# numericalEFT/MCIntegration.jl

Hardware: AMD Instinct MI355X
Metric: Msamples/sec (whole node), 16-D Gaussian :vegas (higher is better)
Workload: dtype f64

## Files before the change

### mcintegration.jl_amd/_lib.py

```python
import ctypes as C
import os

_PKG = os.path.dirname(os.path.abspath(__file__))
_SO = os.path.join(_PKG, "lib", "libmci_hip.so")

MCI_OK = 0
ERR_NAMES = {1: "INVALID", 2: "HIP", 3: "COMPILE", 4: "NORMALIZATION", 5: "HISTOGRAM", 6: "COMM", 7: "NO_DEVICE"}
CONTINUOUS, DISCRETE, FERMIK = 0, 1, 2
VEGAS, VEGASMC, MCMC = 0, 1, 2
ABI_VERSION = 5
SOLVERS = {"vegas": VEGAS, "vegasmc": VEGASMC, "mcmc": MCMC, VEGAS: VEGAS, VEGASMC: VEGASMC, MCMC: MCMC}

c_double_p = C.POINTER(C.c_double)
c_int32_p = C.POINTER(C.c_int32)


class MCIError(RuntimeError):
    def __init__(self, code, msg):
        super().__init__("[MCI_ERR_%s] %s" % (ERR_NAMES.get(code, code), msg))
        self.code = code


class LeafDesc(C.Structure):
    _fields_ = [("kind", C.c_int32), ("pool", C.c_int32), ("lower", C.c_double), ("upper", C.c_double),
                ("npoints", C.c_int32), ("alpha", C.c_double), ("adapt", C.c_int32), ("init", c_double_p)]


class ProblemDesc(C.Structure):
    _fields_ = [("nleaf", C.c_int32), ("leaves", C.POINTER(LeafDesc)), ("npool", C.c_int32),
                ("nintegrand", C.c_int32), ("dof", c_int32_p), ("obs_nbin", c_int32_p), ("obs_bin_draw", c_int32_p),
                ("neighbor_offsets", c_int32_p), ("neighbor_list", c_int32_p), ("ncomp", C.c_int32)]


class IntegrateArgs(C.Structure):
    _fields_ = [("solver", C.c_int32), ("neval", C.c_int64), ("niter", C.c_int32), ("block", C.c_int64),
                ("ignore", C.c_int32), ("adapt", C.c_int32), ("gamma", C.c_double), ("measurefreq", C.c_int64),
                ("seed", C.c_uint64), ("nchain", C.c_int64), ("first_iteration", C.c_int32),
                ("thermal_ratio", C.c_double), ("reweight_goal", c_double_p)]


HOST_INTEGRAND_FN = C.CFUNCTYPE(C.c_int, c_double_p, c_double_p, C.c_int64, C.c_int32, C.c_int32, C.c_void_p)
HOST_INTEGRAND_IDX_FN = C.CFUNCTYPE(C.c_int, C.POINTER(C.c_int32), c_double_p, c_double_p, C.c_int64, C.c_int32, C.c_int32, C.c_void_p)
HOST_MEASURE_FN = C.CFUNCTYPE(C.c_int, c_double_p, c_double_p, C.c_int64, C.c_int64, C.c_int32, C.c_int32, C.c_int64, c_double_p, C.c_int32, C.c_void_p)
HOST_MEASURE_IDX_FN = C.CFUNCTYPE(C.c_int, C.POINTER(C.c_int32), c_double_p, c_double_p, C.c_int64, C.c_int64, C.c_int32, C.c_int32, C.c_int64, c_double_p,
                                  C.c_int32, C.c_void_p)


class ResultC(C.Structure):
    _fields_ = [("niter", C.c_int32), ("nobs", C.c_int32), ("iter_mean", c_double_p), ("iter_std", c_double_p),
                ("mean", c_double_p), ("stdev", c_double_p), ("chi2", c_double_p), ("neval", C.c_int64),
                ("seconds", C.c_double), ("visited", c_double_p), ("correlated", C.c_int32), ("warmup", C.c_int32)]


_VP = C.c_void_p
SIGNATURES = [
    ("mci_ctx_create", C.c_int, [C.c_int32, C.POINTER(_VP)]),
    ("mci_ctx_destroy", C.c_int, [_VP]),
    ("mci_last_error", C.c_char_p, []),
    ("mci_device_count", C.c_int, [c_int32_p]),
    ("mci_ctx_stream", _VP, [_VP]),
    ("mci_comm_unique_id", C.c_int, [_VP]),
    ("mci_comm_init", C.c_int, [_VP, C.c_int32, C.c_int32, _VP]),
    ("mci_comm_rank", C.c_int, [_VP, c_int32_p, c_int32_p]),
    ("mci_comm_sum", C.c_int, [_VP, c_double_p, C.c_int32]),
    ("mci_problem_create", C.c_int, [_VP, C.POINTER(ProblemDesc), C.POINTER(_VP)]),
    ("mci_problem_destroy", C.c_int, [_VP]),
    ("mci_set_integrand_source", C.c_int, [_VP, C.c_char_p, c_double_p, C.c_int32]),
    ("mci_set_integrand_host", C.c_int, [_VP, _VP, _VP]),
    ("mci_set_integrand_host_indexed", C.c_int, [_VP, _VP, _VP]),
    ("mci_set_measure_source", C.c_int, [_VP, C.c_char_p]),
    ("mci_set_measure_host", C.c_int, [_VP, _VP, _VP]),
    ("mci_set_measure_host_indexed", C.c_int, [_VP, _VP, _VP]),
    ("mci_compile", C.c_int, [_VP]),
    ("mci_compile_solver", C.c_int, [_VP, C.c_int32]),
    ("mci_kernel_code_object", C.c_int, [_VP, C.c_int32, C.c_char_p, C.c_int32]),
    ("mci_check_status", C.c_int, [_VP]),
    ("mci_set_launch", C.c_int, [_VP, C.c_int32, C.c_int32]),
    ("mci_problem_info", C.c_int, [_VP, c_int32_p, c_int32_p, C.POINTER(C.c_int64), c_int32_p, C.POINTER(C.c_int64)]),
    ("mci_get_histogram_copies", C.c_int, [_VP, c_int32_p]),
    ("mci_set_kernel_timing", C.c_int, [_VP, C.c_int32]),
    ("mci_iteration_run", C.c_int, [_VP, C.c_int32, C.c_int64, C.c_int64, C.c_int64, C.c_int32, C.c_uint64, C.c_int64, C.c_int64, C.c_double]),
    ("mci_iteration_reduce", C.c_int, [_VP]),
    ("mci_iteration_finish", C.c_int, [_VP, C.c_int32, C.c_int64, C.c_int32, C.c_double, c_double_p, c_double_p]),
    ("mci_integrate", C.c_int, [_VP, C.POINTER(IntegrateArgs), C.POINTER(ResultC)]),
    ("mci_get_iteration_log", C.c_int, [_VP, C.c_int32, c_double_p]),
    ("mci_reserve_iteration_log", C.c_int, [_VP, C.c_int32]),
    ("mci_get_packed", C.c_int, [_VP, c_double_p, C.c_int64]),
    ("mci_set_packed", C.c_int, [_VP, c_double_p, C.c_int64]),
    ("mci_packed_device_ptr", _VP, [_VP]),
    ("mci_get_grid", C.c_int, [_VP, C.c_int32, c_double_p, C.c_int32]),
    ("mci_set_grid", C.c_int, [_VP, C.c_int32, c_double_p, C.c_int32]),
    ("mci_get_distribution", C.c_int, [_VP, C.c_int32, c_double_p, c_double_p, C.c_int32]),
    ("mci_set_distribution", C.c_int, [_VP, C.c_int32, c_double_p, C.c_int32]),
    ("mci_get_reweight", C.c_int, [_VP, c_double_p, C.c_int32]),
    ("mci_set_reweight", C.c_int, [_VP, c_double_p, C.c_int32]),
    ("mci_set_reweight_goal", C.c_int, [_VP, c_double_p, C.c_int32]),
    ("mci_get_acceptance", C.c_int, [_VP, c_double_p, c_double_p, C.c_int32]),
    ("mci_save_state", C.c_int, [_VP, C.c_char_p]),
    ("mci_load_state", C.c_int, [_VP, C.c_char_p]),
    ("mci_set_train_walk", C.c_int, [_VP, C.c_int32]),
    ("mci_set_rng_bits", C.c_int, [_VP, C.c_int32]),
    ("mci_set_rng_rounds", C.c_int, [_VP, C.c_int32]),
    ("mci_set_deterministic", C.c_int, [_VP, C.c_int32]),
    ("mci_set_chain_carry", C.c_int, [_VP, C.c_int32]),
    ("mci_set_iteration_counted", C.c_int, [_VP, C.c_int32]),
    ("mci_set_persistent", C.c_int, [_VP, C.c_int32]),
    ("mci_last_integrate_persistent", C.c_int, [_VP, C.POINTER(C.c_int32)]),
    ("mci_last_chain_launch", C.c_int, [_VP, C.POINTER(C.c_int64), c_int32_p]),
    ("mci_set_stratification", C.c_int, [_VP, C.c_int32, c_int32_p, C.c_double, C.c_int64]),
    ("mci_set_stratification_off", C.c_int, [_VP]),
    ("mci_get_stratification", C.c_int, [_VP, c_int32_p, C.POINTER(C.c_int64), c_double_p]),
    ("mci_get_strat_counts", C.c_int, [_VP, C.POINTER(C.c_int64), C.c_int64]),
    ("mci_strat_plan", C.c_int, [C.c_int64, C.c_int32, C.c_int64, c_int32_p]),
    ("mci_set_chain_speculation", C.c_int, [_VP, C.c_int32, C.c_double, C.c_int32]),
    ("mci_last_chain_speculation", C.c_int, [_VP, c_int32_p, c_int32_p]),
    ("mci_chain_speculation_status", C.c_int, [_VP, C.c_int32, c_int32_p]),
    ("mci_last_integrate_discarded", C.c_int, [_VP, C.POINTER(C.c_int64), c_int32_p]),
    ("mci_speculation_tree", C.c_int, [C.c_int32, C.c_double, C.c_int32, c_int32_p, c_int32_p, c_int32_p, C.POINTER(C.c_uint64), C.POINTER(C.c_uint64)]),
    ("mci_compile_chain_speculation", C.c_int, [_VP, C.c_int32]),
    ("mci_train", C.c_int, [_VP]),
    ("mci_sample_dump", C.c_int, [_VP, C.c_int32, C.c_uint64, C.c_int64, C.c_int64, C.c_int64, c_double_p, c_double_p, c_double_p]),
    ("mci_kernel_times_ms", C.c_int, [_VP, C.POINTER(C.c_float), C.c_int32, c_int32_p, c_int32_p, c_int32_p]),
    ("mci_kernel_clocks", C.c_int, [_VP, c_double_p, C.c_int32, c_int32_p]),
    ("mci_comm_times_ms", C.c_int, [_VP, C.POINTER(C.c_float), C.c_int32, c_int32_p]),
    ("mci_comm_collectives", C.c_int, [_VP, C.POINTER(C.c_int64), C.POINTER(C.c_int64)]),
    ("mci_reduce_size", C.c_int, [_VP, C.POINTER(C.c_int64)]),
    ("mci_external_reduce_done", C.c_int, [_VP]),
    ("mci_standardize_block", None, [C.c_int64, C.c_int64, C.c_int64, C.POINTER(C.c_int64), C.POINTER(C.c_int64)]),
    ("mci_chain_burnin", C.c_double, [C.c_int64, C.c_int64, C.c_int32]),
    ("mci_mcmc_burnin", C.c_int64, [C.c_int64, C.c_int64, C.c_int32, C.c_int32, C.c_int32, C.c_double]),
    ("mci_mcmc_auto_chains", C.c_int64, [C.c_int64, C.c_int64, C.c_int32, C.c_int32, C.c_int32, C.c_int64, C.c_int64, C.c_int32]),
    ("mci_get_hold_histogram", C.c_int, [_VP, C.POINTER(C.c_uint64)]),
    ("mci_mcmc_launch_valid", C.c_int, [_VP, c_int32_p, c_int32_p, C.POINTER(C.c_int64), C.POINTER(C.c_int64)]),
    ("mci_iteration_discard", C.c_int, [_VP]),
    ("mci_get_block_means", C.c_int, [_VP, C.c_int32, c_double_p, C.POINTER(C.c_int64), c_int32_p]),
    ("mci_reset_block_log", C.c_int, [_VP]),
    ("mci_lineage_sums", None, [c_double_p, C.c_int64, C.c_int64, C.c_int64, c_double_p, C.c_int64, C.c_int64, c_double_p, c_double_p]),
    ("mci_maxdof", None, [c_int32_p, C.c_int32, C.c_int32, c_int32_p]),
    ("mci_mean_std", None, [c_double_p, c_double_p, C.c_int64, C.c_int64, c_double_p, c_double_p]),
    ("mci_average", None, [c_double_p, c_double_p, C.c_int64, C.c_int64, C.c_int64, c_double_p, c_double_p, c_double_p]),
    ("mci_do_reweight", None, [c_double_p, c_double_p, C.c_int64, C.c_double, c_double_p]),
    ("mci_version", C.c_char_p, []),
    ("mci_abi_version", C.c_int32, []),
]
DEBUG_SIGNATURES = [
    ("mci_debug_persist_words", C.c_int, [_VP, C.POINTER(C.c_uint64), C.c_int32]),
    ("mci_debug_walk_counts", C.c_int, [_VP, C.POINTER(C.c_int64)]),
    ("mci_debug_plant_wrong_decision", C.c_int, [_VP, C.c_int32]),
    ("mci_debug_persist_spin_ticks", C.c_int, [_VP, C.c_uint64]),
    ("mci_debug_override", C.c_int, [C.c_char_p, C.c_int64, C.c_int32]),
    ("mci_debug_compiler_id", C.c_int, [C.c_char_p, C.c_char_p, C.c_int32]),
    ("mci_debug_split_chunks", C.c_int, [_VP, C.POINTER(C.c_int64), C.POINTER(C.c_int64)]),
    ("mci_debug_strat_dump", C.c_int, [_VP, C.c_int64, c_double_p, c_double_p, C.POINTER(C.c_int64), c_double_p, c_double_p]),
    ("mci_debug_mcmc_policy", C.c_int, [C.c_int64, C.c_int64, C.c_int64, C.c_int64]),
]

_lib = None


def library_path():
    return _SO


def use_rocm_compiler(rocm=None):
    root = rocm or os.environ.get("ROCM_PATH") or "/opt/rocm"
    mapped = set()
    try:
        with open("/proc/self/maps") as fh:
            for line in fh:
                path = line.split(None, 5)[-1].strip() if line.count(" ") >= 5 else ""
                if "amd_comgr" in path or "hiprtc" in path:
                    mapped.add(os.path.realpath(path))
    except OSError:
        pass

    def installed(names):
        for name in names:
            path = os.path.join(root, "lib", name)
            if os.path.exists(path):
                return path
        return None
    comgr, hiprtc = installed(("libamd_comgr.so.3", "libamd_comgr.so.2", "libamd_comgr.so")), installed(("libhiprtc.so.7", "libhiprtc.so"))
    have_comgr = [p for p in mapped if "amd_comgr" in p]
    if have_comgr and (comgr is None or os.path.realpath(comgr) not in have_comgr):
        return False
    done = False
    for path in (comgr, hiprtc):
        if path is not None:
            C.CDLL(path, mode=C.RTLD_GLOBAL)
            done = True
    return done


def compiler_id():
    buf = C.create_string_buffer(1024)
    lib().mci_debug_compiler_id(None, buf, len(buf))
    return buf.value.decode()


def lib():
    global _lib
    if _lib is None:
        if not os.path.exists(_SO):
            raise ImportError("%s is missing: run `python __graft_entry__.py` (hipcc --offload-arch=gfx950) first; "
                              "the MI355X engine has no Python/CPU fallback" % _SO)
        L = C.CDLL(_SO, mode=C.RTLD_GLOBAL)
        for name, res, args in SIGNATURES + DEBUG_SIGNATURES:
            fn = getattr(L, name)
            fn.restype = res
            fn.argtypes = args
        if L.mci_abi_version() != ABI_VERSION:
            raise ImportError("%s has ABI %d, this package was written against ABI %d: rebuild with `python __graft_entry__.py`" % (_SO, L.mci_abi_version(), ABI_VERSION))
        _lib = L
    return _lib


def check(rc):
    if rc != MCI_OK:
        raise MCIError(rc, lib().mci_last_error().decode(errors="replace"))
```

### mcintegration.jl_amd/csrc/mci_debug.h

```cpp
#ifndef MCI_DEBUG_H
#define MCI_DEBUG_H
#include "../../include/mci.h"
#ifdef __cplusplus
extern "C" {
#endif
int mci_debug_persist_words(mci_problem *prob, unsigned long long *out, int32_t n);
int mci_debug_walk_counts(mci_problem *prob, int64_t *out);
int mci_debug_plant_wrong_decision(mci_problem *prob, int32_t on);
int mci_debug_persist_spin_ticks(mci_problem *prob, unsigned long long ticks);
int mci_debug_override(const char *key, int64_t value, int32_t on);
int mci_debug_split_chunks(const mci_problem *prob, int64_t *chunks, int64_t *bytes);
int mci_debug_strat_dump(mci_problem *prob, int64_t n, double *x, double *y, int64_t *h, double *jac, double *w);
int mci_debug_compiler_id(const char *set, char *out, int32_t n);
int mci_debug_mcmc_policy(int64_t pilot_steps, int64_t grow, int64_t carry_holds, int64_t carry_half_floors);
#ifdef __cplusplus
}
#endif
#endif
```

### mcintegration.jl_amd/csrc/mci_host_integrate.h

```cpp
namespace {
int64_t persist_lds(const mci_problem *p, int *map_off) {
    const int N = p->leaves.empty() ? 1 : p->leaves[0].nbin;
    const int64_t a = (p->lds_bytes + 7) / 8, b = (int64_t)mci::train_lds_doubles(N) + N + 256;
    const int64_t off = ((a > b ? a : b) + 1) & ~(int64_t)1;
    if (map_off) *map_off = (int)off;
    return (off + (N + 2) + 4) * 8;
}
bool persist_layout(const mci_problem *p) {
    const auto &s = p->shape;
    if (p->deterministic || s.table_mode != 0 || s.ntile != 1 || s.host_integrand || s.host_measure || s.nbin <= 0 || s.ec_doubles > 0) return false;
    if (s.nleaf != 1 || p->leaves.size() != 1 || p->leaves[0].kind != 0) return false;
    return persist_lds(p, nullptr) <= 64 * 1024;
}
bool persist_plan(const mci_problem *p, const mci_integrate_args *a, int64_t nevalperblock, int64_t nblocks, int *wpb_out) {
    const auto &s = p->shape;
    if (p->persistent == 0 || p->persist_failed) return false;
    if (a->solver != MCI_VEGAS || a->measurefreq != 1 || a->niter < 1) return false;
    if (p->ctx->nranks != 1) return false;
    if (!persist_layout(p)) return false;
    if (p->wg_per_block > 0 || p->kernel_timing > 0 || p->train_serial >= 1) return false;
    const int64_t work = nevalperblock * nblocks * s.ndraw;
    if (p->persistent < 0 && (work >= ((int64_t)1 << 19) || s.ndraw > 7)) return false;
    const int T = p->threads;
    int64_t target = work < ((int64_t)1 << 19) ? 64 : 128;
// ... 45 lines not shown
    g_orphans.push_back(j);
}
static int compile_persist(mci_problem *p, bool background) {
    if (p->persist_compiled) return MCI_OK;
    Candidate local, *c = &local;
    if (p->persist_job) {
        if (!p->persist_job->done.load(std::memory_order_acquire)) {
            if (background) return MCI_OK;
            p->persist_job->th.join();
        }
        if (p->persist_job->th.joinable()) p->persist_job->th.join();
        local = std::move(p->persist_job->c);
        delete p->persist_job;
        p->persist_job = nullptr;
    } else {
        mcijit::ProblemShape sh = p->shape;
        sh.hcopy = 1;
        sh.det = 0;
        c->src = mcijit::generate_source(sh, MCI_VEGAS, mcijit::kUnitVegasPersist, p->leaves[0].alpha);
        c->threads = p->threads;
        c->rc = mcijit::compile(c->src, c->threads, c->code, c->log, c->cached, &c->path, mcijit::kHdrTrain, background);
        if (c->rc == -1) {
            {
                static const int kPersistAfterCalls = 256;
                static std::mutex mu;
                static std::map<uint64_t, int> asked;
                std::lock_guard<std::mutex> g(mu);
                if (++asked[mcijit::fnv1a(c->src)] < kPersistAfterCalls) return MCI_OK;
            }
            p->persist_job = new mci_problem::PersistJob;
            p->persist_job->c = std::move(local);
            mci_problem::PersistJob *j = p->persist_job;
            j->th = std::thread([j] {
                j->c.rc = mcijit::compile(j->c.src, j->c.threads, j->c.code, j->c.log, j->c.cached, &j->c.path, mcijit::kHdrTrain);
                j->done.store(true, std::memory_order_release);
            });
            return MCI_OK;
        }
    }
    if (c->rc) {
        p->persist_failed = true;
        return fail(MCI_ERR_COMPILE, "integrand failed to compile for gfx950:\n%s", c->log.c_str());
    }
    if (mcijit::max_static_lds_bytes(c->code) != 0 || mcijit::kernel_scratch_bytes(c->code, "mci_vegas_persist") != 0) {
        p->persist_failed = true;
        return fail(MCI_ERR_COMPILE, "the persistent :vegas kernel came out with static LDS or scratch");
    }
    p->persist_code_object = c->path;
    p->persist_threads = c->threads;
    if (p->ctx->offline) {
        p->persist_compiled = true;
        return MCI_OK;
    }
    HIPCHK(hipSetDevice(p->ctx->device));
    if (hipModuleLoadData(&p->module_persist, c->code.data()) != hipSuccess) {
        p->persist_failed = true;
        if (c->cached) unlink(c->path.c_str());
        return fail(MCI_ERR_HIP, "hipModuleLoadData failed for the persistent :vegas code object");
    }
    HIPCHK(hipModuleGetFunction(&p->f_persist, p->module_persist, "mci_vegas_persist"));
    if (!p->d_persist) {
        HIPCHK(hipMalloc((void **)&p->d_persist, kPersistWords * sizeof(unsigned long long)));
        HIPCHK(hipMemsetAsync(p->d_persist, 0, kPersistWords * sizeof(unsigned long long), p->ctx->stream));
        p->persist_arrive = p->persist_done = 0;
    }
    p->persist_compiled = true;
    return MCI_OK;
}

static int persist_launch(mci_problem *p, const mci_integrate_args *ia, int64_t nevalperblock, int64_t lo, int64_t hi, int wpb) {
    const auto &s = p->shape;
    const int64_t nblocks = hi - lo, nrows = nblocks * wpb;
    int rc;
    if ((rc = flush_merge(p))) return rc;
    HIPCHK(hipSetDevice(p->ctx->device));
    if ((rc = ensure_capacity(p, 2 * nrows, nblocks))) return rc;
    if ((rc = grow_iteration_log(p, (int64_t)p->log_row + ia->niter))) return rc;
    const int T = p->persist_threads;
    mci::BatchArgs a{};
    a.edges = p->d_edges;
    a.dacc = p->d_dacc;
    a.ddist = p->d_ddist;
    a.reweight = p->d_reweight;
    a.ud = p->d_ud;
    a.part_cols = p->d_part_cols;
    a.part_hist = p->d_part_hist;
    a.ghist = p->d_ghist;
    a.seed = ia->seed;
    a.iteration = (mci::u32)ia->first_iteration;
    a.neval_per_block = nevalperblock;
    a.block_lo = lo;
    a.wg_per_block = wpb;
    a.measurefreq = 1;
    a.nchain = 1;
    a.hist_atomic = 1;
    a.status = p->d_status;
    a.tile_stride = nblocks * nevalperblock;
    a.nrows = nrows;
    mci::PersistArgs f{};
    mci::MergeArgs &m = f.m;
    m.part_cols = p->d_part_cols;
    m.ncols = s.ncols;
    m.nobs = s.nobs;
    m.ni = s.ni;
    m.nblocks = (int)nblocks;
    m.wg_per_block = wpb;
    m.stage1 = p->d_stage1;
    m.ngroup = (int)mci_problem::kGroups;
    m.ghist = p->d_ghist;
    m.use_ghist = 1;
    m.nbin = s.nbin;
    m.packed = p->d_packed;
    m.status = p->d_status;
    m.scratch = p->d_scratch;
    m.part_pa = nullptr;
    m.npa = p->npa;
    m.nrows = (int)nrows;
    mci::TrainArgs &t = f.t;
    t.leaves = p->d_leaves;
    t.nleaf = s.nleaf;
    t.packed = p->d_packed;
    t.nstat = p->nstat;
    t.edges = p->d_edges;
    t.dacc = p->d_dacc;
    t.ddist = p->d_ddist;
    t.iter_log_row = p->d_iterlog + (size_t)p->log_row * p->nstat;
    t.reweight = p->d_reweight;
    t.goal = nullptr;
    t.nd = s.ni + 1;
    t.do_reweight = 0;
    t.gamma = ia->gamma;
    t.do_train = ia->adapt ? 1 : 0;
    t.serial_walk = 0;
    t.status = p->d_status;
    t.maxn = p->leaves[0].nbin;
    f.niter = ia->niter;
    const int64_t lds = persist_lds(p, &f.map_off);
    f.ctr = p->d_persist;
    if (p->persist_arrive > (1ull << 39)) {
        HIPCHK(hipMemsetAsync(p->d_persist, 0, 3 * sizeof(unsigned long long), p->ctx->stream));
        p->persist_arrive = p->persist_done = 0;
    }
    f.arrive0 = p->persist_arrive;
    f.done0 = p->persist_done;
    f.spin_ticks = p->persist_spin_ticks;
    void *args[] = {&a, &f};
    if (!p->d_edges_backup) HIPCHK(hipMalloc((void **)&p->d_edges_backup, (p->h_edges.size() ? p->h_edges.size() : 1) * sizeof(double)));
    if (p->h_edges.size()) HIPCHK(hipMemcpyAsync(p->d_edges_backup, p->d_edges, p->h_edges.size() * sizeof(double), hipMemcpyDeviceToDevice, p->ctx->stream));
    HIPCHK(hipModuleLaunchKernel(p->f_persist, (unsigned)nrows + 1, 1, 1, (unsigned)T, 1, 1, (unsigned)lds, p->ctx->stream, args, nullptr));
    p->persist_arrive += (unsigned long long)(ia->niter + 1) * (unsigned long long)nrows;
    p->persist_done += (unsigned long long)ia->niter;
    p->launch.time_this_launch = false;
    p->merge_pending = false;
    p->merge = m;
    p->merge.part_cols = p->d_part_cols + (size_t)((ia->niter - 1) & 1) * (size_t)nrows * s.ncols;
    p->launch.last_samples = nblocks * nevalperblock;
    p->launch.last_wg = (int)nrows;
    p->launch.last_threads = T;
    p->launch.last_nblocks = (int)nblocks;
    p->log_row += ia->niter;
    return MCI_OK;
}

static int comm_sum_host(mci_problem *p, double *v, int n) {
    if (!p->ctx->comm) return MCI_OK;
    double *d = nullptr;
    HIPCHK(hipMalloc((void **)&d, (size_t)n * sizeof(double)));
    hipStream_t st = p->ctx->stream;
    hipError_t e = hipMemcpyAsync(d, v, (size_t)n * sizeof(double), hipMemcpyHostToDevice, st);
    int r = e == hipSuccess ? g_rccl.AllReduce(d, d, (size_t)n, kNcclFloat64, kNcclSum, p->ctx->comm, st) : 0;
    p->ctx->collectives += 1;
    p->ctx->last_count = n;
    if (e == hipSuccess && !r) e = hipMemcpyAsync(v, d, (size_t)n * sizeof(double), hipMemcpyDeviceToHost, st);
    if (e == hipSuccess && !r) e = hipStreamSynchronize(st);
    (void)hipFree(d);
    if (r) return fail(MCI_ERR_COMM, "ncclAllReduce (lineage sums): %s", g_rccl.GetErrorString ? g_rccl.GetErrorString(r) : "?");
    if (e != hipSuccess) return fail(MCI_ERR_HIP, "lineage sums: %s", hipGetErrorString(e));
    return MCI_OK;
}

int mci_integrate(mci_problem *p, const mci_integrate_args *a, mci_result *res) {
    if (!p || !a || !res) return fail(MCI_ERR_INVALID, "NULL argument");
    if (p->ctx->offline) return fail(MCI_ERR_NO_DEVICE, "offline context: no device to run on");
    const auto &s = p->shape;
    if (res->niter < a->niter || res->nobs != s.nobs) return fail(MCI_ERR_INVALID, "result buffers too small");
    if (!(a->neval > a->block)) return fail(MCI_ERR_INVALID, "neval=%lld should be larger than nblock = %lld", (long long)a->neval, (long long)a->block);
    int64_t nevalperblock, block;
    mci_standardize_block(a->neval, a->block, p->ctx->nranks, &nevalperblock, &block);
    const int64_t per = block / p->ctx->nranks;
    const int64_t lo = per * p->ctx->rank, hi = lo + per;
    if (a->solver != MCI_VEGAS && a->solver != MCI_VEGASMC && a->solver != MCI_MCMC) return fail(MCI_ERR_INVALID, "Solver %d is not supported!", a->solver);
    int wpb_persist = 0, rc = 0;
    const bool strat = p->strat.on;
    if (strat) {
        if (a->solver != MCI_VEGAS) return fail(MCI_ERR_INVALID, "stratification works with solver = :vegas only (mci_set_stratification_off first)");
        if (a->measurefreq != 1) return fail(MCI_ERR_INVALID, "stratification: measurefreq = %lld is refused (every sample is measured)", (long long)a->measurefreq);
        strat_call_start(p);
    }
    bool persist = !strat && persist_plan(p, a, nevalperblock, hi - lo, &wpb_persist);
    if (persist) (void)compile_persist(p, p->persistent < 0);
    persist = persist && p->persist_compiled;
    if (!persist && !strat && (rc = compile_solver(p, kslot(a->solver, a->measurefreq)))) return rc;
    if ((rc = mci_set_reweight_goal(p, a->reweight_goal, a->reweight_goal ? p->ni + 1 : 0))) return rc;
    const int ignore = a->ignore >= 0 ? a->ignore : (a->adapt ? 1 : 0);
    const size_t nlog = (size_t)a->niter * p->nstat;
    if (nlog + 1 > p->cap_hlog) {
        size_t ncap = p->cap_hlog ? p->cap_hlog : (size_t)64 * p->nstat + 1;
        while (ncap < nlog + 1) ncap *= 2;
        if (p->h_log) (void)hipHostFree(p->h_log);
        p->h_log = nullptr;
        p->cap_hlog = 0;
        HIPCHK(hipHostMalloc((void **)&p->h_log, ncap * sizeof(double), hipHostMallocDefault));
        p->cap_hlog = ncap;
    }
    int64_t blk_row0 = -1;
    if (a->solver != MCI_VEGAS) {
        if ((rc = flush_merge(p))) return rc;
        p->launch.blk_rows = 0;
        p->launch.blk_carried = 0;
        p->launch.blk_stride = (hi - lo) * s.nobs;
        p->launch.blk_lo = lo;
        blk_row0 = 0;
        if ((rc = grow_block_log(p, a->niter))) return rc;
    }
    HIPCHK(hipStreamSynchronize(p->ctx->stream));
    const int row0 = p->log_row;
    auto t0 = std::chrono::steady_clock::now();
    double *h = p->h_log;
    int *hstatus = reinterpret_cast<int *>(p->h_log + nlog);
    int res_warmup = 0;
    p->last_discarded_neval = 0;
    p->last_discarded_launches = 0;
    for (int attempt = 0;; ++attempt) {
        p->last_persistent = persist;
        if (persist && (rc = persist_launch(p, a, nevalperblock, lo, hi, wpb_persist))) return rc;
        for (int it = 0; it < a->niter && !persist; ++it) {
            for (int attempt = 0;; ++attempt) {
                const int32_t iter = a->first_iteration + it + kRepeatStride * attempt;
                p->launch_counted = it >= ignore;
                if ((rc = mci_iteration_run(p, a->solver, nevalperblock, lo, hi, iter, a->seed, a->measurefreq, a->nchain, a->thermal_ratio))) return rc;
                if ((rc = mci_iteration_reduce(p))) return rc;
                if ((rc = mci_iteration_finish(p, a->solver, block, a->adapt, a->gamma, nullptr, nullptr))) return rc;
                if (a->solver != MCI_MCMC || a->nchain > 0 || p->launch.mcmc_warm || (it == 0 && ignore >= 1) || attempt >= kMaxRepeats ||
                    a->first_iteration + it >= kRepeatStride || p->launch.last_nchain <= 1 || !p->launch.hold_inflight)
                    break;
                int32_t valid = 0;
                if ((rc = mci_mcmc_launch_valid(p, &valid, nullptr, nullptr, nullptr))) return rc;
                if (valid) break;
                if ((rc = mci_iteration_discard(p))) return rc;
                res_warmup += 1;
                p->last_discarded_neval += nevalperblock * (hi - lo);
                p->last_discarded_launches += 1;
            }
        }
        p->launch_counted = false;
        HIPCHK(hipMemcpyAsync(h, p->d_iterlog + (size_t)row0 * p->nstat, nlog * sizeof(double), hipMemcpyDeviceToHost, p->ctx->stream));
        HIPCHK(hipMemcpyAsync(hstatus, p->d_status, sizeof(int), hipMemcpyDeviceToHost, p->ctx->stream));
        HIPCHK(hipStreamSynchronize(p->ctx->stream));
        if (persist && attempt == 0 && (*hstatus & mci::ST_PERSIST_STALL)) {
            if (p->d_edges_backup && p->h_edges.size())
                HIPCHK(hipMemcpyAsync(p->d_edges, p->d_edges_backup, p->h_edges.size() * sizeof(double), hipMemcpyDeviceToDevice, p->ctx->stream));
            if ((rc = persist_recover(p))) return rc;
            p->log_row = row0;
            persist = false;
            if ((rc = compile_solver(p, kslot(a->solver, a->measurefreq)))) return rc;
            continue;
        }
        break;
    }
    if (*hstatus && (rc = check_status(p))) return rc;
    auto t1 = std::chrono::steady_clock::now();
    res->seconds = std::chrono::duration<double>(t1 - t0).count();
    res->neval = 0;
    for (int it = 0; it < a->niter; ++it) {
        const double *row = h + (size_t)it * p->nstat;
        if (strat) strat_mean_std(row, s.nobs, res->iter_mean + (size_t)it * s.nobs, res->iter_std + (size_t)it * s.nobs);
        else
        mci_mean_std(row, row + s.nobs, s.nobs, block, res->iter_mean + (size_t)it * s.nobs, res->iter_std + (size_t)it * s.nobs);
        res->neval += (int64_t)row[2 * s.nobs + 1];
        if (res->visited && it == a->niter - 1) memcpy(res->visited, row + 2 * s.nobs + 2, (size_t)(s.ni + 1) * sizeof(double));
    }
    for (int o = 0; o < s.nobs; ++o)
        mci_average(res->iter_mean + o, res->iter_std + o, s.nobs, ignore + 1, a->niter, &res->mean[o], &res->stdev[o], &res->chi2[o]);
    res->correlated = 0;
    res->warmup = res_warmup;
    if (a->solver != MCI_VEGAS && blk_row0 >= 0 && p->launch.blk_rows - blk_row0 == a->niter && p->launch.blk_carried > 0 && a->niter > ignore + 1) {
        const int64_t nb = hi - lo;
        std::vector<double> bm((size_t)a->niter * nb * s.nobs), sums(2 * (size_t)s.nobs);
        HIPCHK(hipMemcpyAsync(bm.data(), p->d_blocklog + (size_t)blk_row0 * p->launch.blk_stride, bm.size() * sizeof(double), hipMemcpyDeviceToHost, p->ctx->stream));
        HIPCHK(hipStreamSynchronize(p->ctx->stream));
        mci_lineage_sums(bm.data(), a->niter, nb, s.nobs, res->iter_std, ignore + 1, a->niter, sums.data(), sums.data() + s.nobs);
        if ((rc = comm_sum_host(p, sums.data(), (int)sums.size()))) return rc;
        std::vector<double> lm(s.nobs), le(s.nobs);
        mci_mean_std(sums.data(), sums.data() + s.nobs, s.nobs, block, lm.data(), le.data());
        for (int o = 0; o < s.nobs; ++o) res->stdev[o] = le[o] > 0.0 ? le[o] : res->stdev[o];
        res->correlated = 1;
    }
    return MCI_OK;
}
```

### mcintegration.jl_amd/csrc/mci_host_iteration.h

```cpp
int mci_iteration_run(mci_problem *p, int32_t solver, int64_t nevalperblock, int64_t block_lo, int64_t block_hi,
                      int32_t iteration, uint64_t seed, int64_t measurefreq, int64_t nchain, double thermal_ratio) {
    if (p->ctx->offline) return fail(MCI_ERR_NO_DEVICE, "offline context: no device to run on");
    if (solver != MCI_VEGAS && solver != MCI_VEGASMC && solver != MCI_MCMC) return fail(MCI_ERR_INVALID, "Solver %d is not supported!", solver);
    const bool auto_chains = nchain <= 0;
    if (measurefreq <= 0) return fail(MCI_ERR_INVALID, "measurefreq must be positive");
    const int64_t nblocks = block_hi - block_lo;
    if (nblocks < 1 || nevalperblock < 1) return fail(MCI_ERR_INVALID, "empty iteration");
    if (p->has_fermik && solver != MCI_MCMC) return fail(MCI_ERR_INVALID, "FermiK variables work with solver=:mcmc only");
    if (p->strat.on) {
        if (solver != MCI_VEGAS) return fail(MCI_ERR_INVALID, "stratification works with solver = :vegas only (mci_set_stratification_off first)");
        return strat_run(p, nevalperblock, block_lo, block_hi, iteration, seed, measurefreq);
    }
    const int kern = kslot(solver, measurefreq);
    int rc = (solver == MCI_VEGAS || p->deterministic || p->shape.host_integrand || p->spec_lanes == 1) ? compile_solver(p, kern) : MCI_OK;
    if (rc) return rc;
    if (solver == MCI_VEGAS && p->shape.host_integrand && (rc = ensure_dump(p))) return rc;
    if ((rc = flush_merge(p))) return rc;
    HIPCHK(hipSetDevice(p->ctx->device));
    const auto &s = p->shape;
    int T = solver_threads(p, solver);
    if (solver == MCI_VEGAS && p->vegas_wide && !p->threads_vegas && p->wg_per_block <= 0 && nblocks * nevalperblock < ((int64_t)1 << 22) &&
        nblocks * nevalperblock * p->shape.ndraw >= ((int64_t)1 << 19))
        T = 512;
    int64_t units = nevalperblock;
// ... 424 lines not shown
            p->d_hstep = nullptr;
            p->cap_hstep = 0;
            HIPCHK(hipMalloc(&p->d_hstep, (size_t)nc * ((3 * nd + nw + 4) * sizeof(double) + (2 * nd + 7) * sizeof(int)) + 16));
            p->cap_hstep = nc;
        }
        if (nc > p->cap_hidx) {
            if (p->h_hidx) (void)hipHostFree(p->h_hidx);
            p->h_hidx = nullptr;
            p->cap_hidx = 0;
            HIPCHK(hipHostMalloc((void **)&p->h_hidx, (size_t)(nc + 1) * sizeof(int32_t), hipHostMallocDefault));
            p->cap_hidx = nc;
        }
        {
            double *dp = (double *)p->d_hstep;
            a.hs.cx = dp; dp += (size_t)nd * nc;
            a.hs.cprob = dp; dp += (size_t)nd * nc;
            a.hs.pprob = dp; dp += (size_t)nd * nc;
            a.hs.cw = dp; dp += (size_t)nw * nc;
            a.hs.cprobability = dp; dp += nc;
            a.hs.pprop = dp; dp += nc;
            a.hs.puacc = dp; dp += nc;
            a.hs.cwabs = dp; dp += nc;
            int *ip = (int *)dp;
            a.hs.cbin = ip; ip += (size_t)nd * nc;
            a.hs.pbin = ip; ip += (size_t)nd * nc;
            a.hs.pvi = ip; ip += nc;
            a.hs.ccurr = ip; ip += nc;
            a.hs.cit = ip; ip += nc;
            a.hs.ctr = ip; ip += nc;
            a.hs.pnew = ip; ip += nc;
            a.hs.put = ip; ip += nc;
            a.hs.hidx = ip; ip += nc;
            a.hs.done = ip;
        }
        a.hs.hx = p->d_hx;
        a.hs.nc = nc;
        a.hs.steps = steps;
        HIPCHK(hipMemsetAsync(p->d_part_cols, 0, (size_t)nrows * s.ncols * sizeof(double), st));
        if (hist_lds && s.nbin > 0) HIPCHK(hipMemsetAsync(p->d_part_hist, 0, (size_t)nrows * s.nbin * sizeof(double), st));
        HIPCHK(hipMemsetAsync(p->d_part_pa, 0, (size_t)nrows * 2 * p->npa * sizeof(double), st));
        HIPCHK(hipMemsetAsync(a.hs.done, 0, sizeof(int), st));
        if (solver == MCI_VEGASMC) {
            for (int64_t ne = 0; ne <= steps + 1; ++ne) {
                a.hs.ne = ne;
                HIPCHK(hipModuleLaunchKernel(f, (unsigned)nwg, 1, 1, (unsigned)T, 1, 1, (unsigned)solver_lds(p, solver), st, args, nullptr));
                if (ne > steps) break;
                HIPCHK(hipMemcpyAsync(p->h_hx, p->d_hx, (size_t)nc * nd * sizeof(double), hipMemcpyDeviceToHost, st));
                HIPCHK(hipStreamSynchronize(st));
                if ((rc = eval_host_integrand(p, nullptr, p->h_hx, p->h_hw, nc))) return rc;
                HIPCHK(hipMemcpyAsync(p->d_hw, p->h_hw, (size_t)nc * nw * sizeof(double), hipMemcpyHostToDevice, st));
            }
        } else {
            const int64_t limit = steps + nburn + 2 + 10000;
            for (int64_t ne = 0;; ++ne) {
                a.hs.ne = ne;
                HIPCHK(hipModuleLaunchKernel(f, (unsigned)nwg, 1, 1, (unsigned)T, 1, 1, (unsigned)solver_lds(p, solver), st, args, nullptr));
                HIPCHK(hipMemcpyAsync(p->h_hidx, a.hs.hidx, (size_t)(nc + 1) * sizeof(int32_t), hipMemcpyDeviceToHost, st));
                HIPCHK(hipMemcpyAsync(p->h_hx, p->d_hx, (size_t)nc * nd * sizeof(double), hipMemcpyDeviceToHost, st));
                HIPCHK(hipStreamSynchronize(st));
                if (p->h_hidx[nc] >= nc) break;
                if (ne > limit) return fail(MCI_ERR_INVALID, "host-closure :mcmc chains did not finish (%d of %lld)", (int)p->h_hidx[nc], (long long)nc);
                if ((rc = eval_host_integrand(p, p->h_hidx, p->h_hx, p->h_hw, nc))) return rc;
                HIPCHK(hipMemcpyAsync(p->d_hw, p->h_hw, (size_t)nc * s.ncomp * sizeof(double), hipMemcpyHostToDevice, st));
            }
        }
    } else
    for (int64_t c = 0; c < nchunks; ++c) {
        if (nchunks > 1) {
            a.chunk_lo = c * chunk_len;
            a.chunk_hi = a.chunk_lo + chunk_len < nevalperblock ? a.chunk_lo + chunk_len : nevalperblock;
            a.accum = c > 0 ? 1 : 0;
        }
        HIPCHK(hipModuleLaunchKernel(f, (unsigned)nwg, 1, 1, (unsigned)T_launch, 1, 1, (unsigned)solver_lds(p, solver), st, args, nullptr));
        if (split && c + 1 < nchunks)
            HIPCHK(hipModuleLaunchKernel(p->f_tiles[kern == kSlotVegasAny ? 1 : 0], (unsigned)(((hist_rows + 7) / 8) * 8 * (s.ntile - (s.split_all ? 0 : 1))), 1, 1, (unsigned)T, 1, 1, (unsigned)p->lds_bytes, st, args, nullptr));
    }
    if (solver == MCI_MCMC) p->launch.hold_measured = a.hold_hist != nullptr;
    if (a.hold_hist && auto_chains && (rc = hold_publish(p, nevalperblock / nchain, solver != MCI_VEGAS && p->launch.last_carried))) return rc;
    if (split)
        HIPCHK(hipModuleLaunchKernel(p->f_tiles[kern == kSlotVegasAny ? 1 : 0], (unsigned)(((hist_rows + 7) / 8) * 8 * (s.ntile - (s.split_all ? 0 : 1))), 1, 1, (unsigned)T, 1, 1, (unsigned)p->lds_bytes, st, args, nullptr));
    if (p->launch.time_this_launch) HIPCHK(hipEventRecord(p->evs[2 * slot + 1], st));
    p->launch.ev_valid[slot] = p->launch.time_this_launch;
    p->launch.clock_valid[slot] = a.clock_out != nullptr && !split && s.ntile == 1;
    p->launch.launches += 1;
    if (s.host_measure) {
        const int64_t n = nblocks * hm_n;
        const int nw = s.ni * s.ncomp, nc = s.ncomp;
        std::vector<double> obs((size_t)nblocks * s.nobs, 0.0);
        if (n > 0 && !p->in_self_check) {
            HIPCHK(hipMemcpyAsync(p->h_mx, p->d_mx, (size_t)n * s.ndraw * sizeof(double), hipMemcpyDeviceToHost, st));
            HIPCHK(hipMemcpyAsync(p->h_mrelw, p->d_mrelw, (size_t)n * hm_rows * sizeof(double), hipMemcpyDeviceToHost, st));
            if (solver == MCI_MCMC) HIPCHK(hipMemcpyAsync(p->h_midx, p->d_midx, (size_t)n * sizeof(int32_t), hipMemcpyDeviceToHost, st));
            HIPCHK(hipStreamSynchronize(st));
            const double *relw = p->h_mrelw;
            if (solver == MCI_MCMC && p->hmeas_fn) {
                p->h_mtmp.assign((size_t)n * nw, 0.0);
                for (int64_t i = 0; i < n; ++i)
                    if (p->h_midx[i] >= 0)
                        for (int q = 0; q < nc; ++q) p->h_mtmp[(size_t)(p->h_midx[i] * nc + q) * n + i] = p->h_mrelw[(size_t)q * n + i];
                relw = p->h_mtmp.data();
            }
            if (solver != MCI_MCMC && p->hmeas_idx_fn) p->h_mitmp.resize((size_t)hm_n);
            const bool squeeze = solver == MCI_VEGAS && measurefreq > 1;
            const int64_t keep = squeeze ? nevalperblock / measurefreq : hm_n;
            std::vector<double> sx, sw;
            if (squeeze) {
                sx.resize((size_t)(keep > 0 ? keep : 1) * s.ndraw);
                sw.resize((size_t)(keep > 0 ? keep : 1) * nw);
            }
            for (int64_t b = 0; b < nblocks; ++b) {
                const int64_t off = b * hm_n;
                double *ob = obs.data() + (size_t)b * s.nobs;
                int hrc = 0;
                if (squeeze) {
                    for (int k = 0; k < s.ndraw; ++k)
                        for (int64_t j = 0; j < keep; ++j) sx[(size_t)k * keep + j] = p->h_mx[(size_t)k * n + off + (j + 1) * measurefreq - 1];
                    for (int q = 0; q < nw; ++q)
                        for (int64_t j = 0; j < keep; ++j) sw[(size_t)q * keep + j] = relw[(size_t)q * n + off + (j + 1) * measurefreq - 1];
                    if (p->hmeas_fn) hrc = p->hmeas_fn(sx.data(), sw.data(), keep, keep, s.ndraw, nw, block_lo + b, ob, s.nobs, p->hmeas_user);
                    else {
                        p->h_mitmp.resize((size_t)(keep > 0 ? keep : 1));
                        for (int j = 0; j < s.ni && !hrc; ++j) {
                            std::fill(p->h_mitmp.begin(), p->h_mitmp.end(), (int32_t)j);
                            hrc = p->hmeas_idx_fn(p->h_mitmp.data(), sx.data(), sw.data() + (size_t)j * nc * keep, keep, keep, s.ndraw, nc, block_lo + b, ob,
                                                  s.nobs, p->hmeas_user);
                        }
                    }
                } else if (p->hmeas_fn) {
                    hrc = p->hmeas_fn(p->h_mx + off, relw + off, hm_n, n, s.ndraw, nw, block_lo + b, ob, s.nobs, p->hmeas_user);
                } else if (solver == MCI_MCMC) {
                    hrc = p->hmeas_idx_fn(p->h_midx + off, p->h_mx + off, relw + off, hm_n, n, s.ndraw, nc, block_lo + b, ob, s.nobs, p->hmeas_user);
                } else {
                    for (int j = 0; j < s.ni && !hrc; ++j) {
                        std::fill(p->h_mitmp.begin(), p->h_mitmp.end(), (int32_t)j);
                        hrc = p->hmeas_idx_fn(p->h_mitmp.data(), p->h_mx + off, relw + (size_t)j * nc * n + off, hm_n, n, s.ndraw, nc, block_lo + b, ob,
                                              s.nobs, p->hmeas_user);
                    }
                }
                if (hrc) return fail(MCI_ERR_INVALID, "the host measure failed (%d)", hrc);
            }
        }
        HIPCHK(hipMemcpyAsync(p->d_mobs, obs.data(), obs.size() * sizeof(double), hipMemcpyHostToDevice, st));
        hipLaunchKernelGGL(mci::k_add_host_obs, dim3((unsigned)((nblocks * s.nobs + 255) / 256)), dim3(256), 0, st, p->d_mobs, (int)nblocks, s.nobs, s.ncols, wpb,
                           p->d_part_cols);
        HIPCHK(hipGetLastError());
        HIPCHK(hipStreamSynchronize(st));
    }
    p->launch.last_samples = nblocks * nevalperblock;
    p->launch.last_wg = (int)nwg;
    p->launch.last_threads = T_launch;
    p->launch.last_nblocks = (int)nblocks;
    if (solver != MCI_VEGAS) p->launch.last_nchain = nchain;
    const int nb256 = (s.nbin + 255) / 256;
    if (hist_lds && s.nbin > 0 && !atomic_flush)
        hipLaunchKernelGGL(mci::k_hist_stage1, dim3(nb256, mci_problem::kGroups), dim3(256), 0, st, p->d_part_hist, (int)hist_rows, s.nbin,
                           (int)mci_problem::kGroups, p->d_stage1);
    HIPCHK(hipGetLastError());
    mci::MergeArgs &m = p->merge;
    m.part_cols = p->d_part_cols;
    m.ncols = s.ncols;
    m.nobs = s.nobs;
    m.ni = s.ni;
    m.nblocks = (int)nblocks;
    m.wg_per_block = wpb;
    m.stage1 = p->d_stage1;
    m.ngroup = (int)mci_problem::kGroups;
    m.ghist = p->d_ghist;
    m.use_ghist = (hist_lds && !atomic_flush) ? 0 : atomic_flush ? ghist_buffers : 1;
    m.nbin = s.nbin;
    m.packed = p->d_packed;
    m.status = p->d_status;
    m.scratch = p->d_scratch;
    m.part_pa = solver != MCI_VEGAS ? p->d_part_pa : nullptr;
    m.npa = p->npa;
    m.nrows = (int)nrows;
    m.block_means = nullptr;
    m.hold = a.hold_hist;
    if (solver != MCI_VEGAS && !p->in_self_check) {
        const int64_t stride = nblocks * s.nobs;
        if (stride != p->launch.blk_stride || block_lo != p->launch.blk_lo) {
            p->launch.blk_rows = 0;
            p->launch.blk_carried = 0;
            p->launch.blk_stride = stride;
            p->launch.blk_lo = block_lo;
        }
        if ((rc = grow_block_log(p, p->launch.blk_rows + 1))) return rc;
        m.block_means = p->d_blocklog + (size_t)p->launch.blk_rows * stride;
        p->launch.blk_rows += 1;
        p->launch.blk_carried += p->launch.last_carried ? 1 : 0;
    }
    p->merge_pending = true;
    return MCI_OK;
}

static int flush_merge(mci_problem *p) {
    if (!p->merge_pending) return MCI_OK;
    p->merge_pending = false;
    HIPCHK(hipSetDevice(p->ctx->device));
    const int nb256 = (p->shape.nbin + 255) / 256;
    hipLaunchKernelGGL(mci::k_finalize, dim3(nb256 + 1 + (2 * p->npa + 3) / 4), dim3(256), 0, p->ctx->stream, p->merge);
    HIPCHK(hipGetLastError());
    return MCI_OK;
}

int mci_iteration_reduce(mci_problem *p) {
    if (p->ctx->offline) return fail(MCI_ERR_NO_DEVICE, "offline context");
    if (!p->ctx->comm) return MCI_OK;
    int rc = flush_merge(p);
    if (rc) return rc;
    const bool timed = p->launch.time_this_launch;
    const int slot = (int)(p->reduces % mci_problem::kCevRing);
    if (timed) {
        if (p->cevs.empty()) {
            p->cevs.resize(2 * mci_problem::kCevRing);
            for (auto &e : p->cevs) HIPCHK(hipEventCreate(&e));
        }
        HIPCHK(hipEventRecord(p->cevs[2 * slot], p->ctx->stream));
    }
    const size_t count = (size_t)p->packed_n + (p->launch.hold_deferred ? 64 : 0);
    int r = g_rccl.AllReduce(p->d_packed, p->d_packed, count, kNcclFloat64, kNcclSum, p->ctx->comm, p->ctx->stream);
    if (r) return fail(MCI_ERR_COMM, "ncclAllReduce: %s", g_rccl.GetErrorString ? g_rccl.GetErrorString(r) : "?");
    p->ctx->collectives += 1;
    p->ctx->last_count = (long long)count;
    if (p->launch.hold_deferred && (rc = hold_publish_reduced(p))) return rc;
    if (timed) HIPCHK(hipEventRecord(p->cevs[2 * slot + 1], p->ctx->stream));
    p->cev_valid[slot] = timed;
    p->reduces += 1;
    return MCI_OK;
}

int mci_comm_collectives(const mci_ctx *c, int64_t *calls, int64_t *last_count) {
    if (!c) return fail(MCI_ERR_INVALID, "NULL argument");
    if (calls) *calls = c->collectives;
    if (last_count) *last_count = c->last_count;
    return MCI_OK;
}

int mci_external_reduce_done(mci_problem *p) {
    if (!p) return fail(MCI_ERR_INVALID, "NULL argument");
    if (p->ctx->offline) return fail(MCI_ERR_NO_DEVICE, "offline context");
    if (!p->launch.hold_ext_pending) return MCI_OK;
    p->launch.hold_ext_pending = false;
    HIPCHK(hipSetDevice(p->ctx->device));
    return hold_publish_reduced(p);
}

int mci_reduce_size(const mci_problem *p, int64_t *n) {
    if (!p || !n) return fail(MCI_ERR_INVALID, "NULL argument");
    *n = p->packed_n + 64;
    return MCI_OK;
}

int mci_comm_times_ms(mci_problem *p, float *ms, int32_t n, int32_t *got) {
    if (!p || !ms || !got) return fail(MCI_ERR_INVALID, "NULL argument");
    if (p->ctx->offline) return fail(MCI_ERR_NO_DEVICE, "offline context");
    HIPCHK(hipStreamSynchronize(p->ctx->stream));
    int64_t have = p->reduces < mci_problem::kCevRing ? p->reduces : mci_problem::kCevRing;
    if (have > n) have = n;
    int32_t k = 0;
    for (int64_t i = 0; i < have; ++i) {
        const int slot = (int)((p->reduces - have + i) % mci_problem::kCevRing);
        if (!p->cev_valid[slot]) continue;
        float t = 0.f;
        HIPCHK(hipEventElapsedTime(&t, p->cevs[2 * slot], p->cevs[2 * slot + 1]));
        ms[k++] = t;
    }
    *got = k;
    return MCI_OK;
}

static int launch_train(mci_problem *p, int do_train, int do_reweight, double gamma, double *log_row) {
    const auto &s = p->shape;
    int maxn = 1;
    for (auto &L : p->leaves) maxn = L.nbin > maxn ? L.nbin : maxn;
    mci::TrainArgs a{};
    a.leaves = p->d_leaves;
    a.nleaf = s.nleaf;
    a.packed = p->d_packed;
    a.nstat = p->nstat;
    a.edges = p->d_edges;
    a.dacc = p->d_dacc;
    a.ddist = p->d_ddist;
    a.iter_log_row = log_row;
    a.reweight = p->d_reweight;
    a.goal = p->h_goal.empty() ? nullptr : p->d_goal;
    a.nd = s.ni + 1;
    a.do_reweight = do_reweight;
    a.gamma = gamma;
    a.do_train = do_train;
    if (do_train) p->ntrain += 1;
    a.serial_walk = p->train_serial >= 0 ? p->train_serial : (p->launch.last_samples == 0 || p->launch.last_samples >= mci_problem::kSerialWalkSamples) ? 1 : 0;
    if (p->debug_wrong_decision && a.serial_walk == 1) a.serial_walk = 3;
    a.status = p->d_status;
    a.maxn = maxn;
    a.spare = (size_t)(mci::train_lds_doubles(maxn) + mci::train_spare_doubles(maxn)) * sizeof(double) <= (size_t)kTrainLdsMax ? 1 : 0;
    const size_t sm = (size_t)(mci::train_lds_doubles(maxn) + (a.spare ? mci::train_spare_doubles(maxn) : maxn)) * sizeof(double);
    const unsigned tt = maxn > 256 ? 512u : 256u;
    if (sm > 64 * 1024 && !p->train_lds_raised) {
        HIPCHK(hipFuncSetAttribute((const void *)mci::k_train, hipFuncAttributeMaxDynamicSharedMemorySize, (int)kTrainLdsMax));
        HIPCHK(hipFuncSetAttribute((const void *)mci::k_finish, hipFuncAttributeMaxDynamicSharedMemorySize, (int)kTrainLdsMax));
        p->train_lds_raised = true;
    }
    if (p->merge_pending) {
        p->merge_pending = false;
        hipLaunchKernelGGL(mci::k_finish, dim3(s.nleaf + 1 + (2 * p->npa + 3) / 4), dim3(tt), sm, p->ctx->stream, p->merge, a);
    } else {
        hipLaunchKernelGGL(mci::k_train, dim3(s.nleaf + 1), dim3(tt), sm, p->ctx->stream, a);
    }
    HIPCHK(hipGetLastError());
    return MCI_OK;
}

static int grow_iteration_log(mci_problem *p, int64_t need) {
    if (need <= p->cap_iter) return MCI_OK;
    int64_t ncap = p->cap_iter ? p->cap_iter : 64;
    while (ncap < need) ncap *= 2;
    double *n = nullptr;
    HIPCHK(hipMalloc((void **)&n, (size_t)ncap * p->nstat * sizeof(double)));
    if (p->d_iterlog) {
        HIPCHK(hipMemcpyAsync(n, p->d_iterlog, (size_t)p->cap_iter * p->nstat * sizeof(double), hipMemcpyDeviceToDevice, p->ctx->stream));
        HIPCHK(hipStreamSynchronize(p->ctx->stream));
        (void)hipFree(p->d_iterlog);
    }
    p->d_iterlog = n;
    p->cap_iter = ncap;
    return MCI_OK;
}

int mci_reserve_iteration_log(mci_problem *p, int32_t rows) {
    if (!p || rows < 0) return fail(MCI_ERR_INVALID, "bad argument");
    if (p->ctx->offline) return fail(MCI_ERR_NO_DEVICE, "offline context");
    HIPCHK(hipSetDevice(p->ctx->device));
    return grow_iteration_log(p, (int64_t)p->log_row + rows);
}

int mci_iteration_finish(mci_problem *p, int32_t solver, int64_t block_total, int32_t adapt, double gamma, double *mean, double *std) {
    if (p->ctx->offline) return fail(MCI_ERR_NO_DEVICE, "offline context");
    HIPCHK(hipSetDevice(p->ctx->device));
    const auto &s = p->shape;
    if (int grc = grow_iteration_log(p, (int64_t)p->log_row + 1)) return grc;
    double *row = p->d_iterlog + (size_t)p->log_row * p->nstat;
    const bool strat = p->strat.last_run;
    int rc = launch_train(p, adapt ? 1 : 0, (solver == MCI_VEGASMC || solver == MCI_MCMC) ? 1 : 0, gamma, row);
    if (rc) return rc;
    if (strat && (rc = strat_finish(p, row, adapt))) return rc;
    p->log_row += 1;
    if (mean || std) {
        std::vector<double> h(p->nstat);
        HIPCHK(hipMemcpyAsync(h.data(), row, (size_t)p->nstat * sizeof(double), hipMemcpyDeviceToHost, p->ctx->stream));
        if ((rc = check_status(p))) return rc;
        std::vector<double> m(s.nobs), e(s.nobs);
        if (strat) strat_mean_std(h.data(), s.nobs, m.data(), e.data());
        else
        mci_mean_std(h.data(), h.data() + s.nobs, s.nobs, block_total, m.data(), e.data());
        if (mean) memcpy(mean, m.data(), s.nobs * sizeof(double));
        if (std) memcpy(std, e.data(), s.nobs * sizeof(double));
    }
    return MCI_OK;
}

int mci_train(mci_problem *p) {
    if (p->ctx->offline) return fail(MCI_ERR_NO_DEVICE, "offline context");
    int rc = flush_merge(p);
    if (rc) return rc;
    rc = launch_train(p, 1, 0, 1.0, nullptr);
    if (rc) return rc;
    return check_status(p);
}
```

### mcintegration.jl_amd/csrc/mci_host_jit.h

```cpp
enum { kSlotVegasAny = 3, kSlotDump = 4, kSlotVegasmcSpec = 5, kSlotMcmcSpec = 6 };
static int kslot(int solver, int64_t measurefreq) { return solver == MCI_VEGAS && measurefreq != 1 ? kSlotVegasAny : solver; }
static int slot_solver(int slot) { return slot == kSlotVegasAny ? MCI_VEGAS : slot == kSlotVegasmcSpec ? MCI_VEGASMC : slot == kSlotMcmcSpec ? MCI_MCMC : slot; }

namespace {
struct Candidate {
    std::string src;
    int threads = 256;
    std::vector<char> code;
    std::string log, path;
    bool cached = false;
    int rc = 0;
    long vgprs() const { return mcijit::kernel_vgprs(code, "mci_vegas_batch"); }
    long scratch() const { return mcijit::kernel_scratch_bytes(code, "mci_vegas_batch"); }
};
void compile_all(std::vector<Candidate *> &cs) {
    std::vector<std::thread> th;
    for (size_t i = 1; i < cs.size(); ++i)
        th.emplace_back([c = cs[i]] { c->rc = mcijit::compile(c->src, c->threads, c->code, c->log, c->cached, &c->path); });
    if (!cs.empty()) cs[0]->rc = mcijit::compile(cs[0]->src, cs[0]->threads, cs[0]->code, cs[0]->log, cs[0]->cached, &cs[0]->path);
    for (auto &t : th) t.join();
}
}

static int load_slot(mci_problem *p, int slot, Candidate &c, int64_t lds) {
// ... 397 lines not shown
    int maxacc = 0;
    spec_build(lanes, accept, max_accepts, tab, &maxacc);
    for (int i = 0; i < lanes; ++i) {
        if (depth) depth[i] = tab[(size_t)i].depth;
        if (anc) anc[i] = tab[(size_t)i].anc;
        if (nacc) nacc[i] = tab[(size_t)i].nacc;
        if (needacc) needacc[i] = tab[(size_t)i].needacc;
        if (needrej) needrej[i] = tab[(size_t)i].needrej;
    }
    return MCI_OK;
}

int mci_compile_chain_speculation(mci_problem *p, int32_t solver) {
    if (!p) return fail(MCI_ERR_INVALID, "NULL argument");
    if (solver != MCI_VEGASMC && solver != MCI_MCMC) return fail(MCI_ERR_INVALID, "several lanes per chain: solver MCI_VEGASMC or MCI_MCMC");
    if (p->shape.host_integrand) return fail(MCI_ERR_INVALID, "a host integrand keeps one lane per chain");
    return compile_spec(p, solver);
}

int mci_compile(mci_problem *p) { return compile_solver(p, MCI_VEGAS); }

int mci_kernel_code_object(mci_problem *p, int32_t solver, char *buf, int32_t n) {
    if (!p || !buf || n < 1) return fail(MCI_ERR_INVALID, "NULL argument");
    if (solver == MCI_VEGAS_PERSISTENT) {
        if (!p->persist_compiled) return fail(MCI_ERR_INVALID, "the persistent :vegas kernel has not been compiled yet");
        snprintf(buf, (size_t)n, "%s", p->persist_code_object.c_str());
        return MCI_OK;
    }
    if (solver == MCI_VEGASMC_LANES || solver == MCI_MCMC_LANES) {
        const int sl = solver == MCI_VEGASMC_LANES ? kSlotVegasmcSpec : kSlotMcmcSpec;
        if (!p->compiled[sl]) return fail(MCI_ERR_INVALID, "the several-lanes-per-chain kernel has not been compiled yet");
        snprintf(buf, (size_t)n, "%s", p->code_object[sl].c_str());
        return MCI_OK;
    }
    if (solver == MCI_VEGAS_STRAT) {
        if (!p->strat.compiled) return fail(MCI_ERR_INVALID, "the stratified :vegas kernel has not been compiled yet");
        snprintf(buf, (size_t)n, "%s", p->strat.code_object.c_str());
        return MCI_OK;
    }
    if (solver < 0 || solver > 2) return fail(MCI_ERR_INVALID, "Solver %d is not supported!", solver);
    const int slot = (solver == MCI_VEGAS && !p->compiled[solver] && p->compiled[kSlotVegasAny]) ? kSlotVegasAny : solver;
    if (!p->compiled[slot]) return fail(MCI_ERR_INVALID, "solver %d has not been compiled yet", solver);
    snprintf(buf, (size_t)n, "%s", p->code_object[slot].c_str());
    return MCI_OK;
}

int mci_set_rng_bits(mci_problem *p, int32_t bits) {
    if (!p) return fail(MCI_ERR_INVALID, "NULL argument");
    if (bits != 52 && bits != 32) return fail(MCI_ERR_INVALID, "rng bits must be 52 (default: the resolution of rand(Float64)) or 32");
    if (p->shape.rng_bits != bits) {
        p->shape.rng_bits = bits;
        drop_modules(p);
    }
    return MCI_OK;
}

int mci_set_rng_rounds(mci_problem *p, int32_t rounds) {
    if (!p) return fail(MCI_ERR_INVALID, "NULL argument");
    if (rounds != 10 && rounds != 7) return fail(MCI_ERR_INVALID, "Philox4x32 rounds must be 10 (default) or 7 (the fewest that pass BigCrush)");
    if (p->shape.rng_rounds != rounds) {
        p->shape.rng_rounds = rounds;
        drop_modules(p);
    }
    return MCI_OK;
}

int mci_set_train_walk(mci_problem *p, int32_t mode) {
    if (!p) return fail(MCI_ERR_INVALID, "NULL argument");
    if (mode < -1 || mode > 2) return fail(MCI_ERR_INVALID, "train walk mode must be -1 (automatic), 0 (prefix scan), 1 (serial recurrence) or 2 (serial recurrence, general form only)");
    p->train_serial = mode;
    return MCI_OK;
}

int mci_debug_plant_wrong_decision(mci_problem *p, int32_t on) {
    if (!p) return fail(MCI_ERR_INVALID, "NULL argument");
    p->debug_wrong_decision = on != 0;
    return MCI_OK;
}

int mci_debug_override(const char *key, int64_t value, int32_t on) {
    Override *o = override_slot(key);
    if (!o) return fail(MCI_ERR_INVALID, "no such override: %s", key ? key : "(null)");
    o->on = on != 0;
    o->v = value;
    return MCI_OK;
}

int mci_debug_split_chunks(const mci_problem *p, int64_t *chunks, int64_t *bytes) {
    if (!p) return fail(MCI_ERR_INVALID, "NULL argument");
    if (chunks) *chunks = p->launch.last_split_chunks;
    if (bytes) *bytes = p->launch.last_split_bytes;
    return MCI_OK;
}

int mci_debug_compiler_id(const char *set, char *out, int32_t n) {
    if (set) mcijit::compiler_id_override() = set;
    if (out && n > 0) snprintf(out, (size_t)n, "%s", mcijit::compiler_id().c_str());
    return MCI_OK;
}

int mci_debug_mcmc_policy(int64_t pilot_steps, int64_t grow, int64_t carry_holds, int64_t carry_half_floors) {
    if (pilot_steps > 0) mci_problem::kMcmcPilotSteps = pilot_steps;
    if (grow > 0) mci_problem::kMcmcGrow = grow;
    if (carry_holds > 0) mci_problem::kMcmcCarryHolds = carry_holds;
    if (carry_half_floors > 0) mci_problem::kMcmcCarryHalfFloors = carry_half_floors;
    return MCI_OK;
}

int mci_debug_persist_spin_ticks(mci_problem *p, unsigned long long ticks) {
    if (!p || ticks == 0) return fail(MCI_ERR_INVALID, "bad argument");
    p->persist_spin_ticks = ticks;
    return MCI_OK;
}

int mci_set_deterministic(mci_problem *p, int32_t on) {
    if (!p) return fail(MCI_ERR_INVALID, "NULL argument");
    const bool want = on != 0;
    if (want != p->deterministic) {
        p->deterministic = want;
        p->shape.det = want ? 1 : 0;
        drop_modules(p);
    }
    return MCI_OK;
}

int mci_set_chain_carry(mci_problem *p, int32_t mode) {
    if (!p) return fail(MCI_ERR_INVALID, "NULL argument");
    if (mode < -1 || mode > 1) return fail(MCI_ERR_INVALID, "chain carry mode must be -1 (automatic) or 1 (many-chain launches of :vegasmc and :mcmc continue the chains of the iteration before) or 0 (every launch starts its chains afresh)");
    p->chain_carry = mode;
    if (mode == 0) p->launch.chain_valid = false;
    return MCI_OK;
}

int mci_set_iteration_counted(mci_problem *p, int32_t counted) {
    if (!p) return fail(MCI_ERR_INVALID, "NULL argument");
    p->launch_counted = counted != 0;
    return MCI_OK;
}

int mci_set_persistent(mci_problem *p, int32_t mode) {
    if (!p) return fail(MCI_ERR_INVALID, "NULL argument");
    if (mode < -1 || mode > 1) return fail(MCI_ERR_INVALID, "persistent mode must be -1 (automatic: launch-bound :vegas calls), 0 (one launch chain per iteration) or 1 (whenever the layout allows)");
    p->persistent = mode;
    return MCI_OK;
}

int mci_debug_persist_words(mci_problem *p, unsigned long long *out, int32_t n) {
    if (!p || !out || !p->d_persist) return fail(MCI_ERR_INVALID, "no persistent launch yet");
    HIPCHK(hipStreamSynchronize(p->ctx->stream));
    HIPCHK(hipMemcpy(out, p->d_persist, (size_t)(n < (int)kPersistWords ? n : (int)kPersistWords) * sizeof(unsigned long long), hipMemcpyDeviceToHost));
    return MCI_OK;
}

int mci_debug_walk_counts(mci_problem *p, int64_t *out) {
    if (!p || !out || !p->d_status) return fail(MCI_ERR_INVALID, "NULL argument");
    int h[2] = {0, 0};
    HIPCHK(hipStreamSynchronize(p->ctx->stream));
    HIPCHK(hipMemcpy(h, p->d_status + 1, sizeof(h), hipMemcpyDeviceToHost));
    out[0] = h[0];
    out[1] = h[1];
    return MCI_OK;
}

int mci_last_integrate_persistent(const mci_problem *p, int32_t *persistent) {
    if (!p || !persistent) return fail(MCI_ERR_INVALID, "NULL argument");
    *persistent = p->last_persistent ? 1 : 0;
    return MCI_OK;
}

int mci_last_chain_launch(const mci_problem *p, int64_t *nchain, int32_t *carried) {
    if (!p) return fail(MCI_ERR_INVALID, "NULL argument");
    if (nchain) *nchain = p->launch.last_nchain;
    if (carried) *carried = p->launch.last_carried ? 1 : 0;
    return MCI_OK;
}

int mci_check_status(mci_problem *p) {
    if (!p) return fail(MCI_ERR_INVALID, "NULL argument");
    if (p->ctx->offline) return fail(MCI_ERR_NO_DEVICE, "offline context");
    return check_status(p);
}
static int compile_persist(mci_problem *p, bool background);
static bool persist_layout_ok(const mci_problem *p);
static int compile_strat(mci_problem *p);
int mci_compile_solver(mci_problem *p, int32_t solver) {
    if (solver == MCI_VEGAS_PERSISTENT) {
        if (!persist_layout_ok(p)) return fail(MCI_ERR_INVALID, "this layout has no persistent :vegas kernel (mci_set_persistent)");
        return compile_persist(p, false);
    }
    if (solver == MCI_VEGASMC_LANES || solver == MCI_MCMC_LANES) return mci_compile_chain_speculation(p, solver == MCI_VEGASMC_LANES ? MCI_VEGASMC : MCI_MCMC);
    if (solver == MCI_VEGAS_STRAT) {
        if (!p->strat.on) return fail(MCI_ERR_INVALID, "the problem is not stratified (mci_set_stratification)");
        return compile_strat(p);
    }
    if (solver < 0 || solver > 2) return fail(MCI_ERR_INVALID, "Solver %d is not supported!", solver);
    return compile_solver(p, solver);
}

int mci_get_histogram_copies(const mci_problem *p, int32_t *copies) {
    if (!p || !copies) return fail(MCI_ERR_INVALID, "NULL argument");
    *copies = (p->compiled[MCI_VEGAS] || p->compiled[kSlotVegasAny]) ? p->shape.hcopy : planned_hcopy(p, nullptr);
    return MCI_OK;
}

int mci_problem_info(const mci_problem *p, int32_t *ndraw, int32_t *nobs, int64_t *packed_size, int32_t *table_mode, int64_t *lds_bytes) {
    if (ndraw) *ndraw = p->shape.ndraw;
    if (nobs) *nobs = p->shape.nobs;
    if (packed_size) *packed_size = p->packed_n;
    if (table_mode) *table_mode = p->shape.table_mode;
    if (lds_bytes) *lds_bytes = p->lds_bytes;
    return MCI_OK;
}
```

### mcintegration.jl_amd/csrc/mci_host_problem.h

```cpp
int mci_problem_create(mci_ctx *ctx, const mci_problem_desc *d, mci_problem **out) {
    if (!ctx || !d || !out) return fail(MCI_ERR_INVALID, "NULL argument");
    if (d->nleaf < 1 || d->npool < 1 || d->nintegrand < 1) return fail(MCI_ERR_INVALID, "At least one integrand is required.");
    if (d->nintegrand > 31) return fail(MCI_ERR_INVALID, "at most 31 integrands are supported");
    mci_problem *p = new mci_problem();
    p->ctx = ctx;
    p->npool = d->npool;
    p->ni = d->nintegrand;
    const int Nd = p->ni + 1;
    p->dof.assign((size_t)Nd * p->npool, 0);
    for (int i = 0; i < p->ni * p->npool; ++i) {
        if (d->dof[i] < 0) { delete p; return fail(MCI_ERR_INVALID, "dof must be non-negative"); }
        p->dof[i] = d->dof[i];
    }
    p->maxdof.assign(p->npool, 0);
    mci_maxdof(p->dof.data(), Nd, p->npool, p->maxdof.data());
    p->pool_leaf0.assign(p->npool, -1);
    p->pool_nleaf.assign(p->npool, 0);
    auto &s = p->shape;
    int eoff = 0, aoff = 0, doff = 0, boff = 0;
    for (int l = 0; l < d->nleaf; ++l) {
        const mci_leaf_desc &ld = d->leaves[l];
        if (ld.pool < 0 || ld.pool >= p->npool) { delete p; return fail(MCI_ERR_INVALID, "leaf %d: pool out of range", l); }
        if (p->pool_leaf0[ld.pool] < 0) p->pool_leaf0[ld.pool] = l;
        else if (p->pool_leaf0[ld.pool] + p->pool_nleaf[ld.pool] != l) { delete p; return fail(MCI_ERR_INVALID, "leaves of pool %d are not contiguous", ld.pool); }
// ... 154 lines not shown
    for (auto &L : p->leaves) {
        s.leaf_kind.push_back(L.kind);
        s.leaf_nbin.push_back(L.nbin);
        s.leaf_eoff.push_back(L.eoff);
        s.leaf_doff.push_back(L.doff);
        s.leaf_boff.push_back(L.boff);
        s.leaf_adapt.push_back(L.adapt);
        s.leaf_lower.push_back(L.kind == MCI_CONTINUOUS ? 0.0 : L.lower);
        s.leaf_upper.push_back(L.kind == MCI_CONTINUOUS ? 0.0 : L.upper);
    }
    {
        int npair = 0;
        for (auto &L : p->leaves) {
            s.leaf_poff.push_back(npair);
            if (L.kind == MCI_CONTINUOUS) npair += 2 * L.nbin;
        }
        s.npair = npair;
        const int64_t fixed = (int64_t)(s.ndacc + s.nddist + s.nobs + 16 * s.ncols + 2 * p->npa) * 8;
        const int64_t e1 = (int64_t)s.nedge * 8, e2 = (int64_t)npair * 8, hb = (int64_t)s.nbin * 8;
        const int64_t lim0 = 80 * 1024, lim1 = 160 * 1024 - 1024;
        int mode = 3, pair = 0;
        if (fixed + e2 + hb <= lim0) { mode = 0; pair = 1; }
        else if (fixed + e1 + hb <= lim0) { mode = 0; pair = 0; }
        else if (fixed + e2 + hb <= lim1) { mode = 0; pair = 1; }
        else if (fixed + e1 + hb <= lim1) { mode = 0; pair = 0; }
        if (g_over.table_mode.on) {
            const int m = (int)g_over.table_mode.v;
            if (m == 1 && fixed + e1 <= lim1) { mode = 1; pair = (fixed + e2 <= lim1) ? 1 : 0; }
            if (m == 2) { mode = 2; pair = 0; }
            if (m == 3) { mode = 3; pair = 0; }
        }
        if (g_over.train_walk.on) p->train_serial = g_over.train_walk.v == 2 ? 2 : g_over.train_walk.v != 0 ? 1 : 0;
        s.leaf_tile.assign(p->leaves.size(), 0);
        s.tile_boff.assign(1, 0);
        s.tile_nbin.assign(1, s.nbin);
        if (mode == 3) {
            int64_t budget = (lim1 - fixed) / 8;
            if (g_over.hist_tile_bins.on) budget = g_over.hist_tile_bins.v;
            s.tile_boff.clear();
            s.tile_nbin.clear();
            int64_t fill = budget;
            {
                int64_t ntile_min = 1, acc = 0;
                for (const Leaf &L : p->leaves) {
                    if (acc + L.nbin > budget) { ntile_min += 1; acc = 0; }
                    acc += L.nbin;
                }
                const int64_t even = ((int64_t)s.nbin + ntile_min - 1) / ntile_min;
                int64_t mx = 0;
                for (const Leaf &L : p->leaves) mx = L.nbin > mx ? L.nbin : mx;
                fill = even + mx - 1 < budget ? even + mx - 1 : budget;
                if (g_over.hist_tile_bins.on) fill = budget;
            }
            int cur = -1;
            for (size_t l = 0; l < p->leaves.size(); ++l) {
                const Leaf &L = p->leaves[l];
                if (L.nbin > budget) { delete p; return fail(MCI_ERR_INVALID, "leaf %zu: %d bins do not fit the LDS histogram", l, L.nbin); }
                if (cur < 0 || s.tile_nbin[cur] + L.nbin > fill) {
                    s.tile_boff.push_back(L.boff);
                    s.tile_nbin.push_back(0);
                    cur += 1;
                }
                s.leaf_tile[l] = cur;
                s.tile_nbin[cur] += L.nbin;
            }
        }
        s.ntile = (int)s.tile_nbin.size();
        s.split_all = (s.ntile > 1 && !(g_over.no_split_all.on && g_over.no_split_all.v != 0)) ? 1 : 0;
        s.leaf_ecoff.assign(p->leaves.size(), -1);
        s.ec_doubles = 0;
        if (s.split_all) {
            int64_t budget = (lim1 - fixed) / 8;
            for (size_t l = 0; l < p->leaves.size(); ++l) {
                const Leaf &L = p->leaves[l];
                if (L.kind != MCI_CONTINUOUS || s.ec_doubles + L.nbin + 1 > budget) continue;
                s.leaf_ecoff[l] = s.ec_doubles;
                s.ec_doubles += L.nbin + 1;
            }
        }
        p->lds_bytes_k1 = fixed + (int64_t)s.ec_doubles * 8;
        p->ntdraw = 0;
        int tdraw_maxbin = 2;
        if (s.ntile > 1)
            for (int k = 0; k < s.ndraw; ++k) {
                const Leaf &L = p->leaves[s.draw_leaf[k]];
                if (L.adapt && s.cover_mask[k] && s.leaf_tile[s.draw_leaf[k]] >= (s.split_all ? 0 : 1)) {
                    p->ntdraw += 1;
                    if (L.nbin > 65536) { delete p; return fail(MCI_ERR_INVALID, "leaf %d: more than 65536 bins with tiled histograms", s.draw_leaf[k]); }
                    if (s.leaf_nbin[s.draw_leaf[k]] > tdraw_maxbin) tdraw_maxbin = s.leaf_nbin[s.draw_leaf[k]];
                }
            }
        {
            int bits = 1;
            while ((1 << bits) < tdraw_maxbin) ++bits;
            p->tdraw_words = (p->ntdraw * bits + 31) / 32;
        }
        s.htile = 0;
        for (int v : s.tile_nbin) s.htile = v > s.htile ? v : s.htile;
        s.table_mode = mode;
        s.pair_table = pair;
        const bool hist_lds = (mode == 0 || mode == 3);
        p->lds_bytes = fixed + (mode <= 1 ? (pair ? e2 : e1) : 0) + (hist_lds ? (int64_t)s.htile * 8 : 0);
        s.hcopy = 1;
        {
            int hc = 1;
            const int64_t one = (int64_t)s.htile * 8;
            int nadd = 0;
            for (int k = 0; k < s.ndraw; ++k) nadd += (p->leaves[s.draw_leaf[k]].adapt && s.cover_mask[k]) ? 1 : 0;
            if (mode == 0 && s.ntile == 1 && p->lds_bytes <= lim0 && nadd >= 4)
                while (hc < 8 && p->lds_bytes + one * (2 * hc - 1) <= lim0) hc *= 2;
            if (g_over.hist_copies.on) {
                hc = (int)g_over.hist_copies.v;
                while (hc > 1 && (!hist_lds || s.ntile != 1 || (hc & (hc - 1)) || p->lds_bytes + one * (hc - 1) > lim1)) hc >>= 1;
                if (hc < 1) hc = 1;
            }
            s.hcopy = p->hcopy_auto = p->hcopy_rule = hc;
        }
        const int64_t hcopy_bytes = (int64_t)s.htile * 8 * (s.hcopy - 1);
        if (mode == 3 && s.ntile == 1) {
            const int64_t budget = (lim1 - p->lds_bytes - hcopy_bytes) / 8;
            for (size_t l = 0; l < p->leaves.size(); ++l) {
                const Leaf &L = p->leaves[l];
                if (L.kind != MCI_CONTINUOUS || s.ec_doubles + L.nbin + 1 > budget) continue;
                s.leaf_ecoff[l] = s.ec_doubles;
                s.ec_doubles += L.nbin + 1;
            }
            p->lds_bytes_k1 = p->lds_bytes + (int64_t)s.ec_doubles * 8;
        }
        s.l1_phase = (mode == 3 && s.split_all) ? 1 : 0;
        if (g_over.l1_phase.on) s.l1_phase = (mode >= 2 && g_over.l1_phase.v > 0) ? 1 : 0;
        if (p->lds_bytes > lim0) p->threads = 512;
        if (p->lds_bytes > lim0) {
            p->vegas_plan_a = true;
            p->threads_vegas = 1024;
        }
        if (s.hcopy > 1 && !p->vegas_plan_a) {
            p->hcopy_plan = true;
            p->threads_vegas = 512;
        }
    }
    p->nstat = 2 * s.nobs + 2 + Nd;
    p->packed_n = p->nstat + s.nbin + 2 * p->npa;
    p->h_reweight.assign(Nd, 1.0 / Nd);
    s.body = "w[0] = 1.0;";
    if (!ctx->offline) {
        HIPCHK(hipSetDevice(ctx->device));
        int rc = upload(p);
        if (rc) { delete p; return rc; }
        HIPCHK(hipMalloc((void **)&p->d_packed, (size_t)(p->packed_n + 64) * sizeof(double)));
        HIPCHK(hipMemset(p->d_packed, 0, (size_t)(p->packed_n + 64) * sizeof(double)));
        HIPCHK(hipMalloc((void **)&p->d_ghist, 3 * (size_t)(s.nbin ? s.nbin : 1) * sizeof(double)));
        HIPCHK(hipMemset(p->d_ghist, 0, 3 * (size_t)(s.nbin ? s.nbin : 1) * sizeof(double)));
        HIPCHK(hipMalloc((void **)&p->d_stage1, (size_t)mci_problem::kGroups * (s.nbin ? s.nbin : 1) * sizeof(double)));
        HIPCHK(hipMalloc((void **)&p->d_status, 4 * sizeof(int)));
        HIPCHK(hipMemset(p->d_status, 0, 4 * sizeof(int)));
        std::vector<mci::LeafDev> ld;
        for (auto &L : p->leaves) ld.push_back({L.kind, L.nbin, L.eoff, L.doff, L.boff, L.adapt, L.alpha});
        HIPCHK(hipMalloc((void **)&p->d_leaves, ld.size() * sizeof(mci::LeafDev)));
        HIPCHK(hipMemcpy(p->d_leaves, ld.data(), ld.size() * sizeof(mci::LeafDev), hipMemcpyHostToDevice));
        p->evs.resize(2 * mci_problem::kEvRing);
        for (auto &e : p->evs) HIPCHK(hipEventCreate(&e));
    }
    *out = p;
    return MCI_OK;
}

static void strat_free_buffers(mci_problem *p);
int mci_problem_destroy(mci_problem *p) {
    if (!p) return MCI_OK;
    if (!p->ctx->offline) {
        (void)hipStreamSynchronize(p->ctx->stream);
        for (void *q : {(void *)p->d_edges, (void *)p->d_dacc, (void *)p->d_ddist, (void *)p->d_reweight, (void *)p->d_ud,
                        (void *)p->d_part_cols, (void *)p->d_part_hist, (void *)p->d_ghist, (void *)p->d_stage1,
                        (void *)p->d_packed, (void *)p->d_scratch, (void *)p->d_iterlog, (void *)p->d_dump,
                        (void *)p->d_status, (void *)p->d_leaves})
            if (q) (void)hipFree(q);
        for (int k = 0; k < mci_problem::kSlots; ++k)
            if (p->module[k]) (void)hipModuleUnload(p->module[k]);
        if (p->module_persist) (void)hipModuleUnload(p->module_persist);
        if (p->strat.module) (void)hipModuleUnload(p->strat.module);
        strat_free_buffers(p);
        if (p->d_persist) (void)hipFree(p->d_persist);
    }
    persist_job_drop(p);
    if (!p->ctx->offline) {
        if (p->d_goal) (void)hipFree(p->d_goal);
        if (p->d_part_pa) (void)hipFree(p->d_part_pa);
        if (p->d_hold) (void)hipFree(p->d_hold);
        for (int b = 0; b < 2; ++b) {
            if (p->d_chain_x[b]) (void)hipFree(p->d_chain_x[b]);
            if (p->d_chain_curr[b]) (void)hipFree(p->d_chain_curr[b]);
        }
        if (p->d_reweight_used) (void)hipFree(p->d_reweight_used);
        if (p->d_carry_W) (void)hipFree(p->d_carry_W);
        if (p->d_carry_src) (void)hipFree(p->d_carry_src);
        if (p->d_spec_tab) (void)hipFree(p->d_spec_tab);
        for (int b = 0; b < 2; ++b)
            if (p->d_chain_P[b]) (void)hipFree(p->d_chain_P[b]);
        if (p->d_carry_w) (void)hipFree(p->d_carry_w);
        if (p->d_clocks) (void)hipFree(p->d_clocks);
        if (p->d_edges_backup) (void)hipFree(p->d_edges_backup);
        if (p->h_hold) (void)hipHostFree(p->h_hold);
        if (p->h_hold_d) (void)hipHostFree(p->h_hold_d);
        if (p->h_log) (void)hipHostFree(p->h_log);
        if (p->hold_ev) (void)hipEventDestroy(p->hold_ev);
        if (p->d_blocklog) (void)hipFree(p->d_blocklog);
        for (auto &e : p->cevs) (void)hipEventDestroy(e);
        if (p->d_hx) (void)hipFree(p->d_hx);
        if (p->d_hstep) (void)hipFree(p->d_hstep);
        if (p->h_hidx) (void)hipHostFree(p->h_hidx);
        if (p->d_hw) (void)hipFree(p->d_hw);
        if (p->h_hx) (void)hipHostFree(p->h_hx);
        if (p->h_hw) (void)hipHostFree(p->h_hw);
        tile_release(p);
        if (p->d_mx) (void)hipFree(p->d_mx);
        if (p->d_mrelw) (void)hipFree(p->d_mrelw);
        if (p->d_mobs) (void)hipFree(p->d_mobs);
        if (p->h_mx) (void)hipHostFree(p->h_mx);
        if (p->h_mrelw) (void)hipHostFree(p->h_mrelw);
        if (p->d_midx) (void)hipFree(p->d_midx);
        if (p->h_midx) (void)hipHostFree(p->h_midx);
        for (auto &e : p->evs) (void)hipEventDestroy(e);
    }
    delete p;
    return MCI_OK;
}

int mci_set_integrand_source(mci_problem *p, const char *body, const double *ud, int32_t nud) {
    if (!p || !body) return fail(MCI_ERR_INVALID, "NULL argument");
    p->shape.body = body;
    p->shape.host_integrand = 0;
    p->host_fn = nullptr;
    p->h_ud.assign(ud, ud + (nud > 0 ? nud : 0));
    drop_modules(p);
    if (!p->ctx->offline) {
        if (p->d_ud) (void)hipFree(p->d_ud);
        p->d_ud = nullptr;
        HIPCHK(hipMalloc((void **)&p->d_ud, (p->h_ud.size() ? p->h_ud.size() : 1) * sizeof(double)));
        if (p->h_ud.size()) HIPCHK(hipMemcpy(p->d_ud, p->h_ud.data(), p->h_ud.size() * sizeof(double), hipMemcpyHostToDevice));
    }
    return MCI_OK;
}

int mci_set_integrand_host(mci_problem *p, mci_host_integrand_fn fn, void *user) {
    if (!p || !fn) return fail(MCI_ERR_INVALID, "NULL argument");
    p->host_fn = fn;
    p->host_user = user;
    p->host_idx_fn = nullptr;
    p->shape.host_integrand = 1;
    p->shape.body = "";
    p->h_ud.clear();
    drop_modules(p);
    if (!p->ctx->offline && !p->d_ud) HIPCHK(hipMalloc((void **)&p->d_ud, sizeof(double)));
    return MCI_OK;
}

int mci_set_integrand_host_indexed(mci_problem *p, mci_host_integrand_idx_fn fn, void *user) {
    if (!p || !fn) return fail(MCI_ERR_INVALID, "NULL argument");
    p->host_idx_fn = fn;
    p->host_fn = nullptr;
    p->host_user = user;
    p->shape.host_integrand = 1;
    p->shape.body = "";
    p->h_ud.clear();
    drop_modules(p);
    if (!p->ctx->offline && !p->d_ud) HIPCHK(hipMalloc((void **)&p->d_ud, sizeof(double)));
    return MCI_OK;
}

static int eval_host_integrand(mci_problem *p, const int32_t *idx, const double *x, double *w, int64_t n) {
    const auto &s = p->shape;
    const int nw = s.ni * s.ncomp, nc = s.ncomp;
    int hrc = 0;
    if (!idx) {
        memset(w, 0, (size_t)n * nw * sizeof(double));
        if (p->host_fn) hrc = p->host_fn(x, w, n, s.ndraw, nw, p->host_user);
        else {
            std::vector<int32_t> which((size_t)n);
            for (int j = 0; j < s.ni && !hrc; ++j) {
                std::fill(which.begin(), which.end(), j);
                hrc = p->host_idx_fn(which.data(), x, w + (size_t)j * nc * n, n, s.ndraw, nc, p->host_user);
            }
        }
    } else if (p->host_idx_fn) {
        memset(w, 0, (size_t)n * nc * sizeof(double));
        hrc = p->host_idx_fn(idx, x, w, n, s.ndraw, nc, p->host_user);
    } else {
        p->h_tmp.assign((size_t)n * nw, 0.0);
        hrc = p->host_fn(x, p->h_tmp.data(), n, s.ndraw, nw, p->host_user);
        for (int q = 0; q < nc; ++q)
            for (int64_t i = 0; i < n; ++i) w[(size_t)q * n + i] = idx[i] >= 0 ? p->h_tmp[((size_t)idx[i] * nc + q) * n + i] : 0.0;
    }
    if (hrc) return fail(MCI_ERR_INVALID, "the host integrand failed (%d)", hrc);
    return MCI_OK;
}

int mci_set_measure_source(mci_problem *p, const char *body) {
    if (!p) return fail(MCI_ERR_INVALID, "NULL argument");
    p->shape.measure_body = body ? body : "";
    p->shape.host_measure = 0;
    p->hmeas_fn = nullptr;
    p->hmeas_idx_fn = nullptr;
    drop_modules(p);
    return MCI_OK;
}

int mci_set_measure_host(mci_problem *p, mci_host_measure_fn fn, void *user) {
    if (!p) return fail(MCI_ERR_INVALID, "NULL argument");
    p->hmeas_fn = fn;
    p->hmeas_idx_fn = nullptr;
    p->hmeas_user = user;
    p->shape.host_measure = fn ? 1 : 0;
    if (fn) p->shape.measure_body = "";
    drop_modules(p);
    return MCI_OK;
}

int mci_set_measure_host_indexed(mci_problem *p, mci_host_measure_idx_fn fn, void *user) {
    if (!p) return fail(MCI_ERR_INVALID, "NULL argument");
    p->hmeas_idx_fn = fn;
    p->hmeas_fn = nullptr;
    p->hmeas_user = user;
    p->shape.host_measure = fn ? 1 : 0;
    if (fn) p->shape.measure_body = "";
    drop_modules(p);
    return MCI_OK;
}

int mci_set_launch(mci_problem *p, int32_t threads, int32_t wg_per_block) {
    if (threads > 0) {
        if (threads % 64 || threads > 1024) return fail(MCI_ERR_INVALID, "threads per workgroup must be a multiple of 64, <= 1024");
        p->threads_explicit = true;
        if (threads != p->threads || p->threads_vegas) {
            p->threads = threads;
            p->vegas_plan_a = false;
// ... 43 lines not shown
```

### mcintegration.jl_amd/csrc/mci_host_strat.h

```cpp
static_assert(mci::kStratMaxCols == mci::kStratReduceCols, "k_strat_reduce keeps the columns the sample kernel writes");
static int flush_merge(mci_problem *p);

static const int64_t kStratSamplesPerCube = 8;

int mci_strat_plan(int64_t neval, int32_t ndim, int64_t max_nhcube, int32_t *nstrat) {
    if (!nstrat || ndim < 1) return fail(MCI_ERR_INVALID, "stratification: ndim must be positive");
    if (max_nhcube < 1) return fail(MCI_ERR_INVALID, "stratification: max_nhcube must be positive");
    const int64_t per = neval / kStratSamplesPerCube, cap = per < max_nhcube ? per : max_nhcube;
    if (cap < 1) return fail(MCI_ERR_INVALID, "stratification: neval = %lld is too small for %lld samples per hypercube", (long long)neval,
                             (long long)kStratSamplesPerCube);
    auto power_le = [cap](int64_t v, int n) {
        int64_t r = 1;
        for (int i = 0; i < n; ++i) {
            if (r > cap / v) return cap + 1;
            r *= v;
        }
        return r;
    };
    int64_t s = (int64_t)floor(pow((double)cap, 1.0 / ndim));
    if (s < 1) s = 1;
    while (s > 1 && power_le(s, ndim) > cap) --s;
    while (power_le(s + 1, ndim) <= cap) ++s;
    int64_t ncube = power_le(s, ndim);
    for (int d = 0; d < ndim; ++d) nstrat[d] = (int32_t)s;
// ... 214 lines not shown
    if ((rc = compile_strat(p))) return rc;
    HIPCHK(hipSetDevice(p->ctx->device));
    const int64_t N = (block_hi - block_lo) * nevalperblock;
    if ((rc = strat_prepare(p, N))) return rc;
    const int T = 256, NW = s.ni * s.ncomp;
    const int64_t base = p->deterministic ? det_lds(p, T) : p->lds_bytes;
    int trips = 0;
    int64_t lds = 0;
    for (int64_t lim : {(int64_t)64 * 1024, (int64_t)159 * 1024}) {
        for (int k = 8; k >= 1 && !trips; k >>= 1) {
            const int nloc = k * T / 2 + 1;
            const int64_t need = base + (int64_t)((nloc + 1) + nloc * 2 * NW + T + T * 2 * NW) * 8;
            if (need <= lim) {
                trips = k;
                lds = need;
            }
        }
        if (trips) break;
    }
    if (!trips) return fail(MCI_ERR_INVALID, "stratification: the tables and the chunk's hypercubes do not fit one CU's LDS");
    const int64_t S = (int64_t)trips * T, nchunk = (N + S - 1) / S;
    const int64_t nblocks = block_hi - block_lo;
    int64_t nwg = nchunk < 2048 ? nchunk : 2048;
    const int64_t mblocks = nwg >= nblocks ? nblocks : 1;
    nwg -= nwg % mblocks;
    if ((rc = ensure_capacity(p, nwg, 1))) return rc;
    if (nchunk > st.cap_chunk) {
        for (void *q : {(void *)st.d_part, (void *)st.d_rec_s, (void *)st.d_rec_h})
            if (q) (void)hipFree(q);
        st.d_part = st.d_rec_s = nullptr;
        st.d_rec_h = nullptr;
        st.cap_chunk = 0;
        HIPCHK(hipMalloc((void **)&st.d_part, (size_t)nchunk * 2 * NW * sizeof(double)));
        HIPCHK(hipMalloc((void **)&st.d_rec_s, (size_t)nchunk * 2 * 2 * NW * sizeof(double)));
        HIPCHK(hipMalloc((void **)&st.d_rec_h, (size_t)nchunk * 2 * sizeof(long long)));
        st.cap_chunk = nchunk;
    }
    if (!st.d_stat) HIPCHK(hipMalloc((void **)&st.d_stat, 2 * mci::kStratMaxCols * sizeof(double)));
    st.ran = true;
    st.last_nchunk = nchunk;

    mci::BatchArgs a{};
    a.edges = p->d_edges;
    a.dacc = p->d_dacc;
    a.ddist = p->d_ddist;
    a.reweight = p->d_reweight;
    a.ud = p->d_ud;
    a.part_cols = p->d_part_cols;
    a.part_hist = p->d_part_hist;
    a.ghist = p->d_ghist;
    a.seed = seed;
    a.iteration = (mci::u32)iteration;
    a.neval_per_block = nevalperblock;
    a.block_lo = block_lo;
    a.wg_per_block = (int)nwg;
    a.measurefreq = 1;
    a.nchain = 1;
    a.status = p->d_status;
    a.hist_atomic = 0;
    a.nrows = nwg;
    mci::StratArgs sa{};
    sa.off = st.d_off;
    sa.dnext = st.d_d;
    sa.part = st.d_part;
    sa.rec_h = st.d_rec_h;
    sa.rec_s = st.d_rec_s;
    sa.ncube = st.ncube;
    sa.nsamp = N;
    sa.chunk = S;
    sa.nchunk = nchunk;
    sa.first_index = block_lo * nevalperblock;
    sa.nloc = (int)(S / 2 + 1);
    sa.beta = st.beta;
    for (int d = 0; d < s.ndraw; ++d) {
        const uint32_t n = (uint32_t)st.nstrat[d];
        int l = 0;
        while (((uint64_t)1 << l) < n) ++l;
        const uint64_t m = (((uint64_t)1 << (31 + l)) + n - 1) / n;
        sa.magic[d] = (uint32_t)(m > 0xFFFFFFFFull ? 0xFFFFFFFFull : m);
        sa.shift[d] = 31 + l;
        sa.nstrat[d] = (int)n;
        sa.inv[d] = 1.0 / (double)n;
        if (n == 1) {
            sa.magic[d] = 0x80000000u;
            sa.shift[d] = 31;
        }
    }
    struct Scratch {
        void *q[5] = {nullptr, nullptr, nullptr, nullptr, nullptr};
        ~Scratch() {
            for (void *v : q)
                if (v) (void)hipFree(v);
        }
    } dump;
    const bool dumping = st.hn > 0;
    if (dumping) {
        if (st.hn != N) return fail(MCI_ERR_INVALID, "mci_debug_strat_dump: %lld samples asked for, the iteration has %lld", (long long)st.hn, (long long)N);
        HIPCHK(hipMalloc(&dump.q[0], (size_t)N * s.ndraw * sizeof(double)));
        HIPCHK(hipMalloc(&dump.q[1], (size_t)N * s.ndraw * sizeof(double)));
        HIPCHK(hipMalloc(&dump.q[2], (size_t)N * sizeof(long long)));
        HIPCHK(hipMalloc(&dump.q[3], (size_t)N * sizeof(double)));
        HIPCHK(hipMalloc(&dump.q[4], (size_t)N * NW * sizeof(double)));
        sa.dump_x = (double *)dump.q[0];
        sa.dump_y = (double *)dump.q[1];
        sa.dump_h = (long long *)dump.q[2];
        sa.dump_jac = (double *)dump.q[3];
        sa.dump_w = (double *)dump.q[4];
    }
    void *args[] = {&a, &sa};
    const int slot = (int)(p->launch.launches % mci_problem::kEvRing);
    p->launch.time_this_launch = p->kernel_timing > 0 || (p->kernel_timing < 0 && N >= ((int64_t)1 << 20));
    if (p->launch.time_this_launch) HIPCHK(hipEventRecord(p->evs[2 * slot], p->ctx->stream));
    HIPCHK(hipModuleLaunchKernel(st.f, (unsigned)nwg, 1, 1, (unsigned)T, 1, 1, (unsigned)lds, p->ctx->stream, args, nullptr));
    if (p->launch.time_this_launch) HIPCHK(hipEventRecord(p->evs[2 * slot + 1], p->ctx->stream));
    p->launch.ev_valid[slot] = p->launch.time_this_launch;
    p->launch.clock_valid[slot] = false;
    p->launch.launches += 1;
    if (dumping) {
        hipStream_t hs = p->ctx->stream;
        HIPCHK(hipMemcpyAsync(st.hx, dump.q[0], (size_t)N * s.ndraw * sizeof(double), hipMemcpyDeviceToHost, hs));
        HIPCHK(hipMemcpyAsync(st.hy, dump.q[1], (size_t)N * s.ndraw * sizeof(double), hipMemcpyDeviceToHost, hs));
        HIPCHK(hipMemcpyAsync(st.hh, dump.q[2], (size_t)N * sizeof(long long), hipMemcpyDeviceToHost, hs));
        HIPCHK(hipMemcpyAsync(st.hjac, dump.q[3], (size_t)N * sizeof(double), hipMemcpyDeviceToHost, hs));
        HIPCHK(hipMemcpyAsync(st.hw, dump.q[4], (size_t)N * NW * sizeof(double), hipMemcpyDeviceToHost, hs));
        HIPCHK(hipStreamSynchronize(hs));
        st.hn = 0;
    }
    const int nb256 = (s.nbin + 255) / 256;
    if (s.nbin > 0)
        hipLaunchKernelGGL(mci::k_hist_stage1, dim3(nb256, mci_problem::kGroups), dim3(256), 0, p->ctx->stream, p->d_part_hist, (int)nwg, s.nbin,
                           (int)mci_problem::kGroups, p->d_stage1);
    HIPCHK(hipGetLastError());
    mci::MergeArgs &m = p->merge;
    m.part_cols = p->d_part_cols;
    m.ncols = s.ncols;
    m.nobs = s.nobs;
    m.ni = s.ni;
    m.nblocks = (int)mblocks;
    m.wg_per_block = (int)(nwg / mblocks);
    m.stage1 = p->d_stage1;
    m.ngroup = (int)mci_problem::kGroups;
    m.ghist = p->d_ghist;
    m.use_ghist = 0;
    m.nbin = s.nbin;
    m.packed = p->d_packed;
    m.status = p->d_status;
    m.scratch = p->d_scratch;
    m.part_pa = nullptr;
    m.npa = p->npa;
    m.nrows = (int)nwg;
    m.block_means = nullptr;
    m.hold = nullptr;
    p->merge_pending = true;
    p->launch.last_samples = N;
    p->launch.last_wg = (int)nwg;
    p->launch.last_threads = T;
    p->launch.last_nblocks = (int)mblocks;
    st.last_run = true;
    return MCI_OK;
}

static int strat_finish(mci_problem *p, double *row, int32_t adapt) {
    auto &st = p->strat;
    st.last_run = false;
    mci::StratReduceArgs r{};
    r.off = st.d_off;
    r.part = st.d_part;
    r.rec_h = st.d_rec_h;
    r.rec_s = st.d_rec_s;
    r.ncube = st.ncube;
    r.nchunk = st.last_nchunk;
    r.nw = p->shape.ni * p->shape.ncomp;
    r.beta = st.beta;
    r.dnext = st.d_d;
    r.out = st.d_stat;
    r.log_row = row;
    hipLaunchKernelGGL(mci::k_strat_reduce, dim3(1), dim3(mci::kStratReduceThreads), 0, p->ctx->stream, r);
    HIPCHK(hipGetLastError());
    st.alloc_pending = adapt != 0;
    return MCI_OK;
}

static void strat_mean_std(const double *row, int nobs, double *mean, double *std) {
    for (int o = 0; o < nobs; ++o) {
        mean[o] = row[o];
        std[o] = row[nobs + o] > 0.0 ? sqrt(row[nobs + o]) : 0.0;
    }
}
```

### mcintegration.jl_amd/csrc/mci_host_types.h

```cpp
namespace {

struct Id128 { char b[128]; };
struct Rccl {
    void *h = nullptr;
    int (*GetUniqueId)(void *) = nullptr;
    int (*CommInitRank)(void **, int, Id128 , int) = nullptr;
    int (*AllReduce)(const void *, void *, size_t, int, int, void *, hipStream_t) = nullptr;
    int (*CommDestroy)(void *) = nullptr;
    const char *(*GetErrorString)(int) = nullptr;
};
Rccl g_rccl;
const int kNcclFloat64 = 8, kNcclSum = 0;

int find_loaded_rccl(struct dl_phdr_info *info, size_t, void *out) {
    const char *n = info->dlpi_name;
    if (n && strstr(n, "librccl.so")) {
        *(std::string *)out = n;
        return 1;
    }
    return 0;
}

int rccl_load() {
    if (g_rccl.h) return MCI_OK;
    void *h = nullptr;
    std::string loaded;
    dl_iterate_phdr(find_loaded_rccl, &loaded);
    if (!loaded.empty()) h = dlopen(loaded.c_str(), RTLD_NOW | RTLD_GLOBAL);
    if (!h) h = dlopen("librccl.so", RTLD_NOW | RTLD_GLOBAL);
    if (!h) h = dlopen("librccl.so.1", RTLD_NOW | RTLD_GLOBAL);
    if (!h) return fail(MCI_ERR_COMM, "cannot load librccl.so: %s", dlerror());
    g_rccl.GetUniqueId = (int (*)(void *))dlsym(h, "ncclGetUniqueId");
    g_rccl.CommInitRank = (int (*)(void **, int, Id128, int))dlsym(h, "ncclCommInitRank");
    g_rccl.AllReduce = (int (*)(const void *, void *, size_t, int, int, void *, hipStream_t))dlsym(h, "ncclAllReduce");
    g_rccl.CommDestroy = (int (*)(void *))dlsym(h, "ncclCommDestroy");
    g_rccl.GetErrorString = (const char *(*)(int))dlsym(h, "ncclGetErrorString");
    if (!g_rccl.GetUniqueId || !g_rccl.CommInitRank || !g_rccl.AllReduce || !g_rccl.CommDestroy)
        return fail(MCI_ERR_COMM, "librccl.so lacks the nccl* entry points");
    g_rccl.h = h;
    return MCI_OK;
}

}

struct mci_ctx {
    int device = -1;
    bool offline = false;
    hipStream_t stream = nullptr;
    void *comm = nullptr;
    int rank = 0, nranks = 1;
    long long collectives = 0, last_count = 0;
    std::mutex spare_mu;
    void *spare = nullptr;
    size_t spare_bytes = 0;
};

namespace {
const int64_t kTrainLdsMax = 160 * 1024 - 4096;
const int kMaxLeafBins = 4400;
struct Leaf {
    int kind, pool, npts, nbin, adapt, eoff, doff, boff;
    double lower, upper, alpha;
    int width = 1;
};
}

struct mci_problem {
    mci_ctx *ctx = nullptr;
    std::vector<Leaf> leaves;
    int npool = 0, ni = 0;
    std::vector<int> dof, maxdof, pool_leaf0, pool_nleaf;
    mcijit::ProblemShape shape;
    int nstat = 0;
    int64_t packed_n = 0;
    int64_t lds_bytes = 0;
    int64_t lds_bytes_k1 = 0;
    std::vector<double> h_edges, h_dacc, h_ddist, h_reweight, h_ud;
    double *d_edges = nullptr, *d_dacc = nullptr, *d_ddist = nullptr, *d_reweight = nullptr, *d_ud = nullptr;
    double *d_part_cols = nullptr, *d_part_hist = nullptr, *d_ghist = nullptr, *d_stage1 = nullptr, *d_packed = nullptr;
    double *d_scratch = nullptr, *d_iterlog = nullptr, *d_dump = nullptr;
    int *d_status = nullptr;
    mci::LeafDev *d_leaves = nullptr;
    int64_t cap_wg = 0, cap_blocks = 0, cap_iter = 0, cap_dump = 0;
    static const int kSlots = 7;
    hipModule_t module[kSlots] = {};
    hipFunction_t f_solver[kSlots] = {}, f_dump = nullptr;
    bool compiled[kSlots] = {};
    std::string code_object[kSlots];
    int spec_lanes = -1, spec_maxacc = -1;
    double spec_accept = 0.0;
    mci::SpecNode *d_spec_tab = nullptr;
    int spec_tab_lanes = 0, spec_tab_limit = -2, spec_tab_maxacc = 0;
    int spec_ntree = 0, spec_first = 0;
    float spec_accepts[8] = {};
    double spec_tab_accept = -1.0;
    int spec_state[2] = {0, 0};
    bool spec_need_check[2] = {false, false};
    bool in_self_check = false;
    int64_t last_discarded_neval = 0;
    int32_t last_discarded_launches = 0;
    static const int64_t kSpecFill = 65536;
    bool vegas_planned = false, vegas_keys = false;
    std::vector<double> h_goal;
    double *d_goal = nullptr;
    int npa = 0;
    double *d_part_pa = nullptr;
    int64_t cap_pa = 0;
    unsigned long long *d_hold = nullptr;
    double *d_tile_w = nullptr;
    uint32_t *d_tile_bins = nullptr;
    size_t tile_bytes = 0;
    int64_t cap_tile = 0;
    int ntdraw = 0;
    int tdraw_words = 0;
    hipFunction_t f_tiles[2] = {nullptr, nullptr};
    mci::MergeArgs merge{};
    bool merge_pending = false;
    bool has_fermik = false;
    mci_host_integrand_fn host_fn = nullptr;
    mci_host_integrand_idx_fn host_idx_fn = nullptr;
    int32_t *h_hidx = nullptr;
    int64_t cap_hidx = 0;
    std::vector<double> h_tmp;
    void *host_user = nullptr;
    double *d_hx = nullptr, *d_hw = nullptr, *h_hx = nullptr, *h_hw = nullptr;
    int64_t cap_host = 0;
    void *d_hstep = nullptr;
    int64_t cap_hstep = 0;
    mci_host_measure_fn hmeas_fn = nullptr;
    mci_host_measure_idx_fn hmeas_idx_fn = nullptr;
    void *hmeas_user = nullptr;
    double *d_mx = nullptr, *d_mrelw = nullptr, *h_mx = nullptr, *h_mrelw = nullptr, *d_mobs = nullptr;
    int32_t *d_midx = nullptr, *h_midx = nullptr;
    int64_t cap_hmeas = 0, cap_mobs = 0;
    std::vector<double> h_mtmp;
    std::vector<int32_t> h_mitmp;
    int threads = 256, wg_per_block = 0;
    bool threads_explicit = false;
    bool vegas_wide = false;
    int threads_vegas = 0;
    bool vegas_plan_a = false;
    int kernel_timing = -1;
    int hcopy_auto = 1, hcopy_rule = 1;
    bool deterministic = false;
    int threads_det[3] = {0, 0, 0};
    bool hcopy_plan = false;
    int train_serial = -1;
    bool debug_wrong_decision = false;
    static const int64_t kSerialWalkSamples = (int64_t)1 << 26;
    bool train_lds_raised = false;
    std::vector<hipEvent_t> cevs;
    bool cev_valid[64] = {};
    int64_t reduces = 0;
    static const int kCevRing = 64;
    unsigned long long *h_hold = nullptr;
    double *h_hold_d = nullptr;
    hipEvent_t hold_ev = nullptr;
    double *d_blocklog = nullptr;
    int64_t cap_blocklog = 0;
    double *d_chain_x[2] = {nullptr, nullptr};
    double *d_chain_P[2] = {nullptr, nullptr};
    double *d_carry_w = nullptr;
    int64_t cap_carry_w = 0;
    hipFunction_t f_carryw[2] = {nullptr, nullptr};
    int *d_chain_curr[2] = {nullptr, nullptr};
    int64_t chain_cap[2] = {0, 0};
    int chain_carry = -1;
    int64_t ntrain = 0;
    bool launch_counted = false;
    double *d_reweight_used = nullptr, *d_carry_W = nullptr;
    int *d_carry_src = nullptr;
    int64_t cap_carry_src = 0, cap_carry_W = 0;
    unsigned long long *d_clocks = nullptr;
    std::vector<hipEvent_t> evs;
    static const int kEvRing = 512;
    int log_row = 0;
    double *h_log = nullptr;
    size_t cap_hlog = 0;
    hipModule_t module_persist = nullptr;
    hipFunction_t f_persist = nullptr;
    bool persist_compiled = false, persist_failed = false;
    std::string persist_code_object;
    int persist_threads = 256;
    struct PersistJob;
    PersistJob *persist_job = nullptr;
    unsigned long long *d_persist = nullptr;
    double *d_edges_backup = nullptr;
    unsigned long long persist_arrive = 0, persist_done = 0;
    unsigned long long persist_spin_ticks = 200000000ull;
    int persistent = -1;
    bool last_persistent = false;
    static const int kGroups = mci::kMergeGroups;
    static const int64_t kChainFill = 131072;
    static int64_t kMcmcPilotSteps, kMcmcGrow;
    static int64_t kMcmcCarryHolds, kMcmcCarryHalfFloors;
    struct LaunchState {
        int last_wg = 0, last_threads = 0, last_nblocks = 0;
        int64_t last_samples = 0;
        int64_t last_nchain = 0;
        int last_spec_lanes = 1, last_spec_maxacc = 0;
        bool last_carried = false;
        int64_t last_split_chunks = 0, last_split_bytes = 0;
        int64_t launches = 0;
        bool time_this_launch = true;
        bool ev_valid[kEvRing] = {};
        bool clock_valid[kEvRing] = {};
        int chain_cur = 0;
        bool chain_valid = false;
        int chain_solver = -1, chain_iteration = -1;
        int64_t chain_lo = 0, chain_hi = 0, chain_nchain = 0;
        int64_t chain_ntrain = 0;
        int64_t blk_rows = 0, blk_stride = 0, blk_lo = -1;
        int blk_carried = 0;
        int64_t hold_max = 0;
        int64_t hold_len = 0;
        int64_t hold_prev = 0;
        bool hold_valid = false;
        bool hold_measured = false;
        bool mcmc_warm = false;
        bool hold_inflight = false;
        bool hold_from_packed = false;
        bool hold_deferred = false;
        bool hold_ext_pending = false;
        int64_t hold_launches = 0;
        int64_t hold_len_inflight = 0;
        bool hold_carried_inflight = false;
    } launch;
    static_assert(std::is_trivially_copyable<LaunchState>::value, "the launch record holds values only");
    struct Strat {
        bool on = false;
        std::vector<int> want;
        double beta = 0.75;
        int64_t max_nhcube = (int64_t)1 << 24;
        std::vector<int> nstrat;
        int64_t ncube = 0, nsamp = 0;
        long long *d_off = nullptr;
        bool ran = false;
        bool alloc_valid = false;
        bool alloc_pending = false;
        double *d_d = nullptr;
        double *d_tsum = nullptr;
        int64_t cap_cube = 0;
        double *d_part = nullptr, *d_rec_s = nullptr, *d_stat = nullptr;
        long long *d_rec_h = nullptr;
        int64_t cap_chunk = 0, last_nchunk = 0;
        bool last_run = false;
        bool compiled = false;
        int compiled_det = -1;
        hipModule_t module = nullptr;
        hipFunction_t f = nullptr;
        std::string code_object;
        double *hx = nullptr, *hy = nullptr, *hjac = nullptr, *hw = nullptr;
        long long *hh = nullptr;
        int64_t hn = 0;
    } strat;
};

static const int kRepeatStride = 16384, kMaxRepeats = 7;

int64_t mci_problem::kMcmcPilotSteps = 4096;
int64_t mci_problem::kMcmcGrow = 2;
int64_t mci_problem::kMcmcCarryHolds = 4;
int64_t mci_problem::kMcmcCarryHalfFloors = 2;

namespace {
struct Override { bool on = false; int64_t v = 0; };
struct Overrides { Override table_mode, hist_tile_bins, no_split_all, l1_phase, train_walk, hist_copies, fresh_floors, fresh_burnin_pct, spec_self_check, split_chunk; } g_over;
Override *override_slot(const char *key) {
    if (!key) return nullptr;
    if (!strcmp(key, "table_mode")) return &g_over.table_mode;
    if (!strcmp(key, "hist_tile_bins")) return &g_over.hist_tile_bins;
    if (!strcmp(key, "no_split_all")) return &g_over.no_split_all;
    if (!strcmp(key, "l1_phase")) return &g_over.l1_phase;
    if (!strcmp(key, "train_walk")) return &g_over.train_walk;
    if (!strcmp(key, "hist_copies")) return &g_over.hist_copies;
    if (!strcmp(key, "fresh_floors")) return &g_over.fresh_floors;
    if (!strcmp(key, "fresh_burnin_pct")) return &g_over.fresh_burnin_pct;
    if (!strcmp(key, "spec_self_check")) return &g_over.spec_self_check;
    if (!strcmp(key, "split_chunk")) return &g_over.split_chunk;
    return nullptr;
}
}

static void persist_job_drop(mci_problem *p);
namespace { void persist_orphans_join(); }
static const size_t kPersistWords = 8 + 3 * 8 * 8 + 16;

namespace {

int tile_alloc(mci_problem *p, size_t bytes) {
    mci_ctx *c = p->ctx;
    void *base = nullptr;
    {
        std::lock_guard<std::mutex> g(c->spare_mu);
        if (c->spare && c->spare_bytes >= bytes && c->spare_bytes <= 2 * bytes + ((size_t)64 << 20)) {
            base = c->spare;
            p->tile_bytes = c->spare_bytes;
            c->spare = nullptr;
            c->spare_bytes = 0;
        }
    }
    if (!base) {
        HIPCHK(hipMalloc(&base, bytes));
        p->tile_bytes = bytes;
    }
    p->d_tile_w = (double *)base;
    return MCI_OK;
}
void tile_release(mci_problem *p) {
    if (!p->d_tile_w) return;
    mci_ctx *c = p->ctx;
    void *drop = p->d_tile_w;
    {
        std::lock_guard<std::mutex> g(c->spare_mu);
        if (p->tile_bytes > c->spare_bytes) {
            drop = c->spare;
            c->spare = p->d_tile_w;
            c->spare_bytes = p->tile_bytes;
        }
    }
    if (drop) (void)hipFree(drop);
    p->d_tile_w = nullptr;
    p->d_tile_bins = nullptr;
    p->tile_bytes = 0;
    p->cap_tile = 0;
}

int upload(mci_problem *p) {
    if (p->ctx->offline) return MCI_OK;
    auto up = [&](double *&d, const std::vector<double> &h) -> int {
        size_t n = h.size() ? h.size() : 1;
        if (!d) HIPCHK(hipMalloc((void **)&d, n * sizeof(double)));
        if (h.size()) HIPCHK(hipMemcpyAsync(d, h.data(), h.size() * sizeof(double), hipMemcpyHostToDevice, p->ctx->stream));
        return MCI_OK;
    };
    int rc;
    if ((rc = up(p->d_edges, p->h_edges))) return rc;
    if ((rc = up(p->d_dacc, p->h_dacc))) return rc;
    if ((rc = up(p->d_ddist, p->h_ddist))) return rc;
    if ((rc = up(p->d_reweight, p->h_reweight))) return rc;
    HIPCHK(hipStreamSynchronize(p->ctx->stream));
    return MCI_OK;
}

int ensure_capacity(mci_problem *p, int64_t nwg, int64_t nblocks) {
    const auto &s = p->shape;
    if (nwg > p->cap_wg) {
        if (p->d_part_cols) (void)hipFree(p->d_part_cols);
        if (p->d_part_hist) (void)hipFree(p->d_part_hist);
        p->d_part_cols = p->d_part_hist = nullptr;
        HIPCHK(hipMalloc((void **)&p->d_part_cols, (size_t)nwg * s.ncols * sizeof(double)));
        if (s.table_mode == 0 || s.table_mode == 3) HIPCHK(hipMalloc((void **)&p->d_part_hist, (size_t)nwg * (s.nbin ? s.nbin : 1) * sizeof(double)));
        p->cap_wg = nwg;
    }
    if (nblocks > p->cap_blocks) {
        if (p->d_scratch) (void)hipFree(p->d_scratch);
        p->d_scratch = nullptr;
        HIPCHK(hipMalloc((void **)&p->d_scratch, (size_t)nblocks * s.ncols * sizeof(double)));
        p->cap_blocks = nblocks;
    }
    return MCI_OK;
}

int check_status(mci_problem *p) {
    int st = 0;
    HIPCHK(hipMemcpyAsync(&st, p->d_status, sizeof(int), hipMemcpyDeviceToHost, p->ctx->stream));
    HIPCHK(hipStreamSynchronize(p->ctx->stream));
    if (!st) return MCI_OK;
    HIPCHK(hipMemsetAsync(p->d_status, 0, sizeof(int), p->ctx->stream));
    if (st & mci::ST_PERSIST_STALL) {
        HIPCHK(hipMemsetAsync(p->d_persist, 0, 3 * sizeof(unsigned long long), p->ctx->stream));
        HIPCHK(hipMemsetAsync(p->d_ghist, 0, 3 * (size_t)(p->shape.nbin ? p->shape.nbin : 1) * sizeof(double), p->ctx->stream));
        p->persist_arrive = p->persist_done = 0;
        p->persist_failed = true;
        return fail(MCI_ERR_HIP, "the persistent :vegas launch stalled (is the device shared with other long-running kernels?); "
                                 "the iterations of this call are void -- later calls launch per iteration (mci_set_persistent(prob, 0))");
    }
    if (st & mci::ST_MCMC_INIT) return fail(MCI_ERR_INVALID, "Cannot find the variables that makes the integrand nonzero!");
    if (st & mci::ST_NORMALIZATION) return fail(MCI_ERR_NORMALIZATION, "Block normalization is not positively defined!");
    if (st & mci::ST_HIST_NONFINITE) return fail(MCI_ERR_HISTOGRAM, "histogram should be all finite");
    if (st & mci::ST_HIST_NONPOSITIVE) return fail(MCI_ERR_HISTOGRAM, "histogram should be all positive and non-zero");
    return fail(MCI_ERR_HISTOGRAM, "distribution is not all finite");
}

int persist_recover(mci_problem *p) {
    hipStream_t st = p->ctx->stream;
    HIPCHK(hipMemsetAsync(p->d_status, 0, sizeof(int), st));
    HIPCHK(hipMemsetAsync(p->d_persist, 0, 3 * sizeof(unsigned long long), st));
    HIPCHK(hipMemsetAsync(p->d_ghist, 0, 3 * (size_t)(p->shape.nbin ? p->shape.nbin : 1) * sizeof(double), st));
    p->persist_arrive = p->persist_done = 0;
    p->persist_failed = true;
    p->merge_pending = false;
    return MCI_OK;
}

int hold_publish(mci_problem *p, int64_t chain_len, bool carried) {
    hipStream_t st = p->ctx->stream;
    if (!p->h_hold) {
        HIPCHK(hipHostMalloc((void **)&p->h_hold, 64 * sizeof(unsigned long long), hipHostMallocDefault));
        HIPCHK(hipHostMalloc((void **)&p->h_hold_d, 64 * sizeof(double), hipHostMallocDefault));
        HIPCHK(hipEventCreateWithFlags(&p->hold_ev, hipEventDisableTiming));
    }
    p->launch.hold_len_inflight = chain_len;
    p->launch.hold_carried_inflight = carried;
    p->launch.hold_launches += 1;
    if (p->ctx->comm) {
        p->launch.hold_deferred = true;
        return MCI_OK;
    }
    if (p->launch.hold_inflight) HIPCHK(hipEventSynchronize(p->hold_ev));
    HIPCHK(hipMemcpyAsync(p->h_hold, p->d_hold, 64 * sizeof(unsigned long long), hipMemcpyDeviceToHost, st));
    HIPCHK(hipEventRecord(p->hold_ev, st));
    p->launch.hold_inflight = true;
    p->launch.hold_from_packed = false;
    p->launch.hold_ext_pending = true;
    return MCI_OK;
}

int hold_publish_reduced(mci_problem *p) {
    hipStream_t st = p->ctx->stream;
    HIPCHK(hipMemcpyAsync(p->h_hold_d, p->d_packed + p->packed_n, 64 * sizeof(double), hipMemcpyDeviceToHost, st));
    HIPCHK(hipEventRecord(p->hold_ev, st));
    p->launch.hold_inflight = true;
    p->launch.hold_from_packed = true;
    p->launch.hold_deferred = false;
    return MCI_OK;
}

int hold_consume(mci_problem *p) {
    if (!p->launch.hold_inflight) return MCI_OK;
    HIPCHK(hipEventSynchronize(p->hold_ev));
    p->launch.hold_inflight = false;
    int top = -1;
    for (int b = 0; b < 64; ++b)
        if (p->launch.hold_from_packed ? p->h_hold_d[b] > 0.5 : p->h_hold[b] != 0ull) top = b;
    if (top >= 0) {
        p->launch.hold_prev = p->launch.mcmc_warm ? p->launch.hold_max : 0;
        p->launch.hold_max = (int64_t)1 << top;
        p->launch.hold_len = p->launch.hold_len_inflight;
        p->launch.hold_valid = p->launch.hold_len >= (p->launch.hold_carried_inflight ? mci_problem::kMcmcCarryHolds : 16) * p->launch.hold_max;
        if (p->launch.hold_valid) p->launch.mcmc_warm = true;
    }
    return MCI_OK;
}

void drop_modules(mci_problem *p) {
    p->vegas_planned = p->vegas_keys = p->vegas_wide = false;
    p->f_dump = nullptr;
    for (int k = 0; k < mci_problem::kSlots; ++k) {
        p->compiled[k] = false;
        if (p->module[k]) {
            (void)hipModuleUnload(p->module[k]);
            p->module[k] = nullptr;
        }
    }
    p->persist_compiled = p->persist_failed = false;
    persist_job_drop(p);
    p->f_persist = nullptr;
    if (p->module_persist) {
        (void)hipModuleUnload(p->module_persist);
        p->module_persist = nullptr;
    }
    p->strat.compiled = false;
    p->strat.f = nullptr;
    if (p->strat.module) {
        (void)hipModuleUnload(p->strat.module);
        p->strat.module = nullptr;
    }
}

}

static int flush_merge(mci_problem *p);
static int comm_sum_host(mci_problem *p, double *v, int n);

static int grow_block_log(mci_problem *p, int64_t rows) {
    const int64_t need = rows * p->launch.blk_stride;
    if (need <= p->cap_blocklog) return MCI_OK;
    int64_t ncap = p->cap_blocklog ? p->cap_blocklog : 4096;
    while (ncap < need) ncap *= 2;
    double *n = nullptr;
    HIPCHK(hipMalloc((void **)&n, (size_t)ncap * sizeof(double)));
    if (p->d_blocklog) {
        HIPCHK(hipMemcpyAsync(n, p->d_blocklog, (size_t)p->cap_blocklog * sizeof(double), hipMemcpyDeviceToDevice, p->ctx->stream));
        HIPCHK(hipStreamSynchronize(p->ctx->stream));
        (void)hipFree(p->d_blocklog);
    }
    p->d_blocklog = n;
    p->cap_blocklog = ncap;
    return MCI_OK;
}
```

### mcintegration.jl_amd/csrc/mci_static_kernels.h

```cpp
#pragma once
#include <hip/hip_runtime.h>

#include "mci_train.h"

namespace mci {

__global__ void __launch_bounds__(256) k_hist_stage1(const double *__restrict__ part_hist, int nwg, int nbin, int ngroup,
                                                     double *__restrict__ out) {
    const int bin = blockIdx.x * 256 + threadIdx.x;
    const int g = blockIdx.y;
    if (bin >= nbin) return;
    const int per = (nwg + ngroup - 1) / ngroup;
    const int w0 = g * per, w1 = min(nwg, w0 + per);
    double s0 = 0.0, s1 = 0.0, s2 = 0.0, s3 = 0.0;
    int w = w0;
    for (; w + 3 < w1; w += 4) {
        s0 += part_hist[(size_t)(w + 0) * nbin + bin];
        s1 += part_hist[(size_t)(w + 1) * nbin + bin];
        s2 += part_hist[(size_t)(w + 2) * nbin + bin];
        s3 += part_hist[(size_t)(w + 3) * nbin + bin];
    }
    for (; w < w1; ++w) s0 += part_hist[(size_t)w * nbin + bin];
    out[(size_t)g * nbin + bin] = (s0 + s1) + (s2 + s3);
}

__global__ void __launch_bounds__(256) k_add_host_obs(const double *__restrict__ obs, int nblocks, int nobs, int ncols, int wg_per_block,
                                                      double *__restrict__ part_cols) {
    const int i = blockIdx.x * 256 + threadIdx.x;
    if (i >= nblocks * nobs) return;
    const int b = i / nobs, o = i % nobs;
    part_cols[(size_t)b * wg_per_block * ncols + o] += obs[i];
}

__global__ void __launch_bounds__(256) k_finalize(MergeArgs m) {
    const int nhb = (m.nbin + 255) / 256;
    const int hoff = 2 * m.nobs + 2 + m.ni + 1;
    if ((int)blockIdx.x < nhb) {
        const int bin = blockIdx.x * 256 + threadIdx.x;
        if (bin < m.nbin) m.packed[hoff + bin] = merge_hist_bin(m, bin);
        return;
    }
    if ((int)blockIdx.x > nhb) {
        merge_pa(m, (int)blockIdx.x - nhb - 1);
        return;
    }
    merge_stats(m);
}

struct ResampleArgs {
    const int *curr_old;
    long long n_old, n_new;
    int nd;
    const double *rw_now, *rw_used;
    int *src;
    double *W;
    const double *w_chain;
};
__global__ void __launch_bounds__(256) k_resample_chains(ResampleArgs a) {
    constexpr int kLdsW = 8192;
    __shared__ double sW[kLdsW];
    __shared__ long long part[256];
    const int tid = threadIdx.x, T = 256;
    const int *co = a.curr_old + (size_t)blockIdx.x * a.n_old;
    double *W = a.W + (size_t)blockIdx.x * a.n_old;
    int *src = a.src + (size_t)blockIdx.x * a.n_new;
    const long long per = (a.n_old + T - 1) / T, j0 = tid * per < a.n_old ? tid * per : a.n_old, j1 = j0 + per < a.n_old ? j0 + per : a.n_old;
    constexpr int kNd = 16;
    if (a.w_chain) {
        __shared__ double dpart[256];
        const double *wc = a.w_chain + (size_t)blockIdx.x * a.n_old;
        double mine = 0.0;
        for (long long j = j0; j < j1; ++j) mine += wc[j];
        dpart[tid] = mine;
        __syncthreads();
        double below = 0.0;
        for (int t = 0; t < tid; ++t) below += dpart[t];
        double run = 0.0;
        for (long long j = j0; j < j1; ++j) {
            run += wc[j];
            const double v = below + run;
            W[j] = v;
            if (a.n_old <= kLdsW) sW[j] = v;
        }
    } else
    if (a.nd <= kNd) {
        long long cnt[kNd];
        double w[kNd];
#pragma unroll
        for (int i = 0; i < kNd; ++i) {
            cnt[i] = 0;
            w[i] = i < a.nd ? a.rw_now[i] / a.rw_used[i] : 0.0;
        }
        for (long long j = j0; j < j1; ++j) {
            const int c = co[j];
#pragma unroll
            for (int i = 0; i < kNd; ++i) cnt[i] += c == i ? 1 : 0;
        }
        for (int i = 0; i < a.nd; ++i) {
            long long mine = 0;
#pragma unroll
            for (int q = 0; q < kNd; ++q) mine = q == i ? cnt[q] : mine;
            __syncthreads();
            part[tid] = mine;
            __syncthreads();
            long long below = 0;
            for (int t = 0; t < tid; ++t) below += part[t];
#pragma unroll
            for (int q = 0; q < kNd; ++q) cnt[q] = q == i ? below : cnt[q];
        }
        for (long long j = j0; j < j1; ++j) {
            const int c = co[j];
            double acc = 0.0;
#pragma unroll
            for (int i = 0; i < kNd; ++i) {
                cnt[i] += c == i ? 1 : 0;
                if (i < a.nd) {
                    const double term = w[i] * (double)cnt[i];
                    acc = i == 0 ? term : acc + term;
                }
            }
            W[j] = acc;
            if (a.n_old <= kLdsW) sW[j] = acc;
        }
    } else
    for (int i = 0; i < a.nd; ++i) {
        const double w = a.rw_now[i] / a.rw_used[i];
        long long mine = 0;
        for (long long j = j0; j < j1; ++j) mine += co[j] == i ? 1 : 0;
        __syncthreads();
        part[tid] = mine;
        __syncthreads();
        long long cnt = 0;
        for (int t = 0; t < tid; ++t) cnt += part[t];
        for (long long j = j0; j < j1; ++j) {
            cnt += co[j] == i ? 1 : 0;
            const double term = w * (double)cnt;
            W[j] = i == 0 ? term : W[j] + term;
        }
    }
    __threadfence_block();
    __syncthreads();
    const bool in_lds = (a.w_chain != nullptr || a.nd <= kNd) && a.n_old <= kLdsW;
    const double step = W[a.n_old - 1] / (double)a.n_new;
    if (!(W[a.n_old - 1] > 0.0)) {
        for (long long c = tid; c < a.n_new; c += T) src[c] = (int)(c % a.n_old);
        return;
    }
    for (long long c = tid; c < a.n_new; c += T) {
        const double target = ((double)c + 0.6180339887498949) * step;
        long long lo = 0, hi = a.n_old - 1;
        while (lo < hi) {
            const long long mid = (lo + hi) >> 1;
            if ((in_lds ? sW[mid] : W[mid]) > target) hi = mid;
            else lo = mid + 1;
        }
        src[c] = (int)lo;
    }
}

__global__ void __launch_bounds__(512) k_train(TrainArgs a) {
    extern __shared__ __attribute__((aligned(16))) double sm[];
    __shared__ double ps[256];
    __shared__ int bad;
    __shared__ double ssum;
    if ((int)blockIdx.x == a.nleaf) {
        iteration_bookkeeping(a);
        return;
    }
    if (!a.do_train) return;
    const LeafDev L = a.leaves[blockIdx.x];
    if (!L.adapt) return;
    double *h = a.packed + a.nstat + L.boff;
    train_leaf(L, h, h, sm, ps, bad, ssum, a.edges, a.dacc, a.ddist, a.serial_walk, a.status, false, nullptr, false, a.spare ? sm + train_lds_doubles(a.maxn) : nullptr);
}

__global__ void __launch_bounds__(512) k_finish(MergeArgs m, TrainArgs a) {
    extern __shared__ __attribute__((aligned(16))) double sm[];
    __shared__ double ps[256];
    __shared__ int bad;
    __shared__ double ssum;
    const int tid = threadIdx.x, T = blockDim.x;
    if ((int)blockIdx.x == a.nleaf) {
        merge_stats(m);
        __syncthreads();
        iteration_bookkeeping(a);
        return;
    }
    if ((int)blockIdx.x > a.nleaf) {
        merge_pa(m, (int)blockIdx.x - a.nleaf - 1);
        return;
    }
    const LeafDev L = a.leaves[blockIdx.x];
    double *hl = sm + train_lds_doubles(a.maxn);
    double *hp = a.packed + a.nstat + L.boff;
    const bool train = a.do_train && L.adapt;
    if (train) train_stage_grid(L, sm, a.edges);
    for (int i = tid; i < L.nbin; i += T) {
        const double v = merge_hist_bin(m, L.boff + i);
        hl[i] = v;
        hp[i] = v;
    }
    __syncthreads();
    if (!train) return;
    train_leaf(L, hl, hp, sm, ps, bad, ssum, a.edges, a.dacc, a.ddist, a.serial_walk, a.status, true, nullptr, false, a.spare ? hl : nullptr);
}

struct StratAllocArgs {
    const double *d;
    long long *off;
    double *tsum;
    long long ncube, nsamp;
    int ntile;
    int uniform;
};
__device__ inline void strat_stretch(const StratAllocArgs &a, long long &lo, long long &hi) {
    const long long tl = (a.ncube + a.ntile - 1) / a.ntile, t0 = (long long)blockIdx.x * tl, t1 = t0 + tl < a.ncube ? t0 + tl : a.ncube;
    const long long per = (t1 - t0 + 255) / 256;
    lo = t0 + (long long)threadIdx.x * per;
    if (lo > t1) lo = t1;
    hi = lo + per < t1 ? lo + per : t1;
}
__global__ void __launch_bounds__(256) k_strat_alloc(StratAllocArgs a, int phase) {
    __shared__ double part[256];
    const int tid = threadIdx.x;
    const long long M = a.nsamp - 2 * a.ncube;
    if (phase == 1) {
        if (tid != 0) return;
        double base = 0.0;
        for (int g = 0; g < a.ntile; ++g) {
            a.tsum[a.ntile + g] = base;
            base += a.tsum[g];
        }
        a.tsum[2 * a.ntile] = base;
        a.tsum[2 * a.ntile + 1] = (a.uniform || !(base > 0.0) || !isfinite(base)) ? 1.0 : 0.0;
        return;
    }
    long long lo, hi;
    strat_stretch(a, lo, hi);
    double mine = 0.0;
    if (!(phase == 2 && a.tsum[2 * a.ntile + 1] != 0.0))
        for (long long h = lo; h < hi; ++h) mine += a.d[h];
    part[tid] = mine;
    __syncthreads();
    if (phase == 0) {
        if (tid == 0) {
            double s = 0.0;
            for (int t = 0; t < 256; ++t) s += part[t];
            a.tsum[blockIdx.x] = s;
        }
        return;
    }
    if (blockIdx.x == 0 && tid == 0) a.off[0] = 0;
    if (a.tsum[2 * a.ntile + 1] != 0.0) {
        for (long long h = lo; h < hi; ++h) {
            double C = (double)M * (double)(h + 1) / (double)a.ncube;
            if (h == a.ncube - 1 || C > (double)M) C = (double)M;
            a.off[h + 1] = 2 * (h + 1) + (long long)floor(C);
        }
        return;
    }
    double sbase = 0.0;
    for (int t = 0; t < tid; ++t) sbase += part[t];
    const double tbase = a.tsum[a.ntile + blockIdx.x], total = a.tsum[2 * a.ntile];
    double run = 0.0;
    for (long long h = lo; h < hi; ++h) {
        run += a.d[h];
        double C = (double)M * (tbase + (sbase + run)) / total;
        if (h == a.ncube - 1 || C > (double)M) C = (double)M;
        a.off[h + 1] = 2 * (h + 1) + (long long)floor(C);
    }
}

enum { kStratReduceCols = 8, kStratReduceThreads = 1024 };
struct StratReduceArgs {
    const long long *off;
    const double *part;
    const long long *rec_h;
    const double *rec_s;
    long long ncube, nchunk;
    int nw;
    double beta;
    double *dnext;
    double *out;
    double *log_row;
};
__global__ void __launch_bounds__(kStratReduceThreads) k_strat_reduce(StratReduceArgs a) {
    __shared__ double red[kStratReduceThreads];
    const int tid = threadIdx.x, T = blockDim.x, nw = a.nw;
    double acc[2 * kStratReduceCols];
    for (int q = 0; q < 2 * kStratReduceCols; ++q) acc[q] = 0.0;
    const double V = 1.0 / (double)a.ncube;
    const long long per = (a.nchunk + T - 1) / T;
    long long c0 = (long long)tid * per;
    if (c0 > a.nchunk) c0 = a.nchunk;
    const long long c1 = c0 + per < a.nchunk ? c0 + per : a.nchunk;
    for (long long c = c0; c < c1; ++c) {
        for (int q = 0; q < 2 * nw; ++q) acc[q] += a.part[c * 2 * nw + q];
        for (int rr = 0; rr < 2; ++rr) {
            const long long h = a.rec_h[2 * c + rr];
            if (h < 0) continue;
            if (rr == 0 && c > 0) {
                const long long ph = a.rec_h[2 * c - 1] >= 0 ? a.rec_h[2 * c - 1] : a.rec_h[2 * c - 2];
                if (ph == h) continue;
            }
            double S[2 * kStratReduceCols];
            for (int q = 0; q < 2 * nw; ++q) S[q] = a.rec_s[(2 * c + rr) * 2 * nw + q];
            for (long long d = c + 1; d < a.nchunk && a.rec_h[2 * d] == h; ++d)
                for (int q = 0; q < 2 * nw; ++q) S[q] += a.rec_s[(2 * d) * 2 * nw + q];
            const double n = (double)(a.off[h + 1] - a.off[h]);
            double ssum = 0.0;
            for (int q = 0; q < nw; ++q) {
                double v2 = (S[nw + q] - S[q] * S[q] / n) / (n - 1.0);
                v2 = v2 > 0.0 ? v2 : 0.0;
                acc[q] += V / n * S[q];
                acc[nw + q] += V * V * v2 / n;
                ssum += v2;
            }
            a.dnext[h] = pow(ssum, 0.5 * a.beta);
        }
    }
    for (int q = 0; q < 2 * nw; ++q) {
        red[tid] = acc[q];
        __syncthreads();
        for (int s = T / 2; s > 0; s >>= 1) {
            if (tid < s) red[tid] += red[tid + s];
            __syncthreads();
        }
        if (tid == 0) {
            a.out[q] = red[0];
            if (a.log_row) a.log_row[q] = red[0];
        }
        __syncthreads();
    }
}

}
```

### mcintegration.jl_amd/csrc/mci_train.h

```cpp
#pragma once
#include "mci_device.h"

namespace mci {


struct LeafDev {
    int kind;
    int nbin;
    int eoff;
    int doff;
    int boff;
    int adapt;
    double alpha;
};


enum { kMergeGroups = 32 };

struct MergeArgs {
    const double *part_cols;
    int ncols, nobs, ni, nblocks, wg_per_block;
    const double *stage1;
    int ngroup;
    double *ghist;
// ... 145 lines not shown
#pragma unroll
        for (int k = 0; k < 32; ++k) s += t[k];
    }
    for (; i + 112 < n; i += 128) {
        double t[8];
#pragma unroll
        for (int k = 0; k < 8; ++k) t[k] = v[i + 16 * k];
#pragma unroll
        for (int k = 0; k < 8; ++k) s += t[k];
    }
    for (; i < n; i += 16) s += v[i];
    s += dpp_read<0x108, 0xf>(s);
    s += dpp_read<0x104, 0xf>(s);
    s += dpp_read<0x102, 0xf>(s);
    s += dpp_read<0x101, 0xf>(s);
    return __shfl(s, 0, 16);
}

#ifdef MCI_TRAIN_SHORT_SUMS
template <int DEPTH = 3> __device__ inline double sum_julia(const double *v, int n) { return sum16(v, n); }
#else
template <int DEPTH = 3> __device__ inline double sum_julia(const double *v, int n) {
    if constexpr (DEPTH == 0) return sum16(v, n);
    else {
        if (n <= 1024) return sum16(v, n);
        const int h = ((n - 1) >> 1) + 1;
        return sum_julia<DEPTH - 1>(v, h) + sum_julia<DEPTH - 1>(v + h, n - h);
    }
}
#endif

__device__ inline double rescale_pow(double b, double alpha) {
    if (alpha == 2.0) return b * b;
    if (alpha == 1.0) return b;
    if (alpha == 3.0) return b * b * b;
    return pow(b, alpha);
}

struct TrainArgs {
    const LeafDev *leaves;
    int nleaf;
    double *packed;
    int nstat;
    double *edges, *dacc, *ddist;
    double *iter_log_row;
    double *reweight;
    const double *goal;
    int nd, do_reweight;
    double gamma;
    int do_train, serial_walk;
    int *status;
    int maxn;
    int spare;
};

#ifndef MCI_TRAIN_SCAN_ONLY
#define MCI_WALK_BIN(K, OFF, DN)                                                                                                       \
    "ds_write_b64 %4, %0 offset:" OFF "\n\tv_cmp_ge_f64 vcc, %0, %3\n\tv_add_f64 %1, %0, -%3\n\tv_cmp_ge_f64_e64 %2, %1, %3\n\t"          \
    "v_add_f64 %0, %0, " DN "\n\ts_cbranch_vccz .Lwd" K "_%=\n\tv_add_f64 %0, %1, " DN "\n\ts_cmp_lg_u64 %2, 0\n\t"                      \
    "s_cbranch_scc1 .Lwr" K "_%=\n.Lwd" K "_%=:\n\t"
#define MCI_WALK_MORE(K, DN)                                                                                                           \
    ".Lwr" K "_%=:\n\tv_add_f64 %1, %1, -%3\n\tv_cmp_ge_f64 vcc, %1, %3\n\ts_cbranch_vccnz .Lwr" K "_%=\n\tv_add_f64 %0, %1, " DN "\n\t"   \
    "s_branch .Lwd" K "_%=\n\t"
__device__ __forceinline__ void walk_bins16(double &acc, const double (&v)[16], const double vnext, const double f, const unsigned rec_addr) {
    double a1;
    unsigned long long c2;
    asm volatile(
                 MCI_WALK_BIN("0", "0", "%6")
                 MCI_WALK_BIN("1", "8", "%7")
                 MCI_WALK_BIN("2", "16", "%8")
                 MCI_WALK_BIN("3", "24", "%9")
                 MCI_WALK_BIN("4", "32", "%10")
                 MCI_WALK_BIN("5", "40", "%11")
                 MCI_WALK_BIN("6", "48", "%12")
                 MCI_WALK_BIN("7", "56", "%13")
                 MCI_WALK_BIN("8", "64", "%14")
                 MCI_WALK_BIN("9", "72", "%15")
                 MCI_WALK_BIN("10", "80", "%16")
                 MCI_WALK_BIN("11", "88", "%17")
                 MCI_WALK_BIN("12", "96", "%18")
                 MCI_WALK_BIN("13", "104", "%19")
                 MCI_WALK_BIN("14", "112", "%20")
                 MCI_WALK_BIN("15", "120", "%21")
                 "s_branch .Lwend_%=\n\t"
                 MCI_WALK_MORE("0", "%6")
                 MCI_WALK_MORE("1", "%7")
                 MCI_WALK_MORE("2", "%8")
                 MCI_WALK_MORE("3", "%9")
                 MCI_WALK_MORE("4", "%10")
                 MCI_WALK_MORE("5", "%11")
                 MCI_WALK_MORE("6", "%12")
                 MCI_WALK_MORE("7", "%13")
                 MCI_WALK_MORE("8", "%14")
                 MCI_WALK_MORE("9", "%15")
                 MCI_WALK_MORE("10", "%16")
                 MCI_WALK_MORE("11", "%17")
                 MCI_WALK_MORE("12", "%18")
                 MCI_WALK_MORE("13", "%19")
                 MCI_WALK_MORE("14", "%20")
                 MCI_WALK_MORE("15", "%21")
                 ".Lwend_%=:"
                 : "+v"(acc), "=&v"(a1), "=&s"(c2)
                 : "v"(f), "v"(rec_addr), "v"(v[0]), "v"(v[1]), "v"(v[2]), "v"(v[3]), "v"(v[4]), "v"(v[5]), "v"(v[6]), "v"(v[7]), "v"(v[8]),
                   "v"(v[9]), "v"(v[10]), "v"(v[11]), "v"(v[12]), "v"(v[13]), "v"(v[14]), "v"(v[15]), "v"(vnext)
                 : "vcc", "scc", "memory");
}

#undef MCI_WALK_BIN
#undef MCI_WALK_MORE

template <bool RECORD> __device__ __forceinline__ void walk_slots16(double &acc, const double (&e)[16], double *__restrict__ rec) {
    if (!RECORD) rec[0] = acc;
#pragma unroll
    for (int k = 0; k < 16; ++k) {
        if (RECORD) rec[k] = acc;
        acc = acc + e[k];
    }
}

__device__ __forceinline__ void walk_trip(double &acc, const double (&v)[16], const double vnext, const double f, const unsigned rec_addr) {
    walk_bins16(acc, v, vnext, f, rec_addr);
}
#endif

enum { kTrainQ = 4 };

__device__ inline void train_stage_grid(const LeafDev &L, double *sm, const double *__restrict__ edges) {
    if (L.kind != 0) return;
    const int tid = threadIdx.x, T = blockDim.x, N = L.nbin;
    double *d = sm, *sg = sm + N + kWalkPad;
    const double *g = edges + L.eoff;
    for (int base = 0; base <= N; base += kTrainQ * T) {
        double v[kTrainQ];
#pragma unroll
        for (int q = 0; q < kTrainQ; ++q) {
            const int i = base + q * T + tid;
            v[q] = i <= N ? g[i] : 0.0;
        }
#pragma unroll
        for (int q = 0; q < kTrainQ; ++q) {
            const int i = base + q * T + tid;
            if (i <= N) sg[i] = v[q];
        }
    }
    if (tid < kWalkPad) d[N + tid] = 0.0;
}

__device__ inline void train_leaf(const LeafDev &L, const double *h, double *hclear, double *sm, double *ps, int &bad, double &ssum,
                                  double *__restrict__ edges, double *__restrict__ dacc, double *__restrict__ ddist, int serial_walk,
                                  int *__restrict__ status, bool staged = false, unsigned long long *tt = nullptr, bool checked = false,
                                  double *spare = nullptr) {
#ifdef MCI_PERSIST_TRACE
#define MCI_TT(k) if (tt && threadIdx.x == 0) tt[k] = wall_clock64();
#else
#define MCI_TT(k)
    (void)tt;
#endif
    const int tid = threadIdx.x, T = blockDim.x;
    const int N = L.nbin;
    double *d = sm;
    double *sg = sm + N + kWalkPad;
    double *wa = sg + N + 2;
    MCI_TT(0)
    if (!checked) {
        if (tid == 0) bad = 0;
        __syncthreads();
        for (int i = tid; i < N; i += T) {
            const double v = h[i];
            if (!isfinite(v)) atomicOr(&bad, ST_HIST_NONFINITE);
            else if (!(v > 0.0)) atomicOr(&bad, ST_HIST_NONPOSITIVE);
        }
        __syncthreads();
    }
    if (bad) {
        if (tid == 0) atomicOr(status, bad);
        return;
    }
    if (L.kind == 0) {
        double *g = edges + L.eoff;
        MCI_TT(1)
        if (!staged) train_stage_grid(L, sm, edges);
        double mine = 0.0;
        for (int i = tid; i < N; i += T) {
            double v;
            if (N <= 1) v = h[i];
            else if (i == 0) v = (h[0] * 7.0 + h[1]) / 8.0;
            else if (i == N - 1) v = (h[N - 1] * 7.0 + h[N - 2]) / 8.0;
            else v = (h[i - 1] + h[i] * 6.0 + h[i + 1]) / 8.0;
            d[i] = v;
            mine += v;
        }
        if (!serial_walk) {
            const double w = wave_sum(mine);
            if ((tid & 63) == 0) ps[32 + (tid >> 6)] = w;
        }
        __syncthreads();
        MCI_TT(2)
        if (N > 1) {
            double s;
            if (serial_walk) {
                s = sum_julia(d, N);
                __syncthreads();
            } else {
                s = 0.0;
                for (int w = 0; w < (T >> 6); ++w) s += ps[32 + w];
            }
            MCI_TT(3)
            int anybad = 0;
            auto rescale_q = [&](auto power, auto QC) {
                constexpr int Q = decltype(QC)::value;
                for (int base = 0; base < N; base += Q * T) {
                    double v[Q];
#pragma unroll
                    for (int q = 0; q < Q; ++q) {
                        const int i = base + q * T + tid;
                        v[q] = i < N ? d[i] / s : 1.0;
                    }
#pragma unroll
                    for (int q = 0; q < Q; ++q) {
                        const double r = power(-(1 - v[q]) / log(v[q]));
                        v[q] = (v[q] > 0 && v[q] <= 0.99999999) ? r : v[q];
                    }
#pragma unroll
                    for (int q = 0; q < Q; ++q) {
                        const int i = base + q * T + tid;
                        if (!isfinite(v[q])) anybad = 1;
                        if (i < N) d[i] = v[q];
                    }
                }
            };
            auto rescale_bins = [&](auto power) {
#ifdef MCI_TRAIN_SCAN_ONLY
                rescale_q(power, IC<(MCI_THREADS >= 512 ? 2 : kTrainQ)>{});
#else
                if (2 * T >= N) rescale_q(power, IC<2>{});
                else rescale_q(power, IC<kTrainQ>{});
#endif
            };
            const double alpha = L.alpha;
#if defined(MCI_TRAIN_POWER) && MCI_TRAIN_POWER == 2
            rescale_bins([](double b) { return b * b; });
#elif defined(MCI_TRAIN_POWER) && MCI_TRAIN_POWER == 3
            rescale_bins([](double b) { return b * b * b; });
#elif defined(MCI_TRAIN_POWER) && MCI_TRAIN_POWER == 1
            rescale_bins([](double b) { return b; });
#elif defined(MCI_TRAIN_POWER) && MCI_TRAIN_POWER == 4
            rescale_bins([alpha](double b) { return pow(b, alpha); });
#else
            if (alpha == 2.0) rescale_bins([](double b) { return b * b; });
            else if (alpha == 3.0) rescale_bins([](double b) { return b * b * b; });
            else if (alpha == 1.0) rescale_bins([](double b) { return b; });
            else rescale_bins([alpha](double b) { return pow(b, alpha); });
#endif
            if (anybad) atomicOr(&bad, ST_RESCALE_NONFINITE);
            __syncthreads();
            MCI_TT(4)
            if (bad) {
                if (tid == 0) atomicOr(status, bad);
                return;
            }
        }
        if (!serial_walk) {
            const double total = block_prefix(d, wa, N, ps);
            const double f_ninc = total / (double)N;
            MCI_TT(5)
            auto place_points = [&](auto QC) {
                constexpr int Q = decltype(QC)::value;
                for (int base = 0; base <= N; base += Q * T) {
                    int lo[Q];
                    double target[Q];
#pragma unroll
                    for (int q = 0; q < Q; ++q) {
                        lo[q] = 0;
                        target[q] = (double)(base + q * T + tid) * f_ninc;
                    }
                    for (int len = N; len > 1;) {
                        const int half = len >> 1;
#pragma unroll
                        for (int q = 0; q < Q; ++q) lo[q] += wa[lo[q] + half - 1] < target[q] ? half : 0;
                        len -= half;
                    }
#pragma unroll
                    for (int q = 0; q < Q; ++q) {
                        lo[q] += wa[lo[q]] < target[q] ? 1 : 0;
                        lo[q] = lo[q] > N - 1 ? N - 1 : lo[q];
                    }
                    double vnew[Q];
#pragma unroll
                    for (int q = 0; q < Q; ++q) {
                        const int i = base + q * T + tid, j = lo[q];
                        const double acc_f = wa[j] - target[q];
                        const double v = sg[j + 1] - (acc_f / d[j]) * (sg[j + 1] - sg[j]);
                        vnew[q] = (i == 0 || i >= N) ? sg[i < N ? 0 : N] : v;
                    }
#pragma unroll
                    for (int q = 0; q < Q; ++q) {
                        const int i = base + q * T + tid;
                        if (i <= N) g[i] = vnew[q];
                    }
                }
            };
#ifdef MCI_TRAIN_SCAN_ONLY
            place_points(IC<(MCI_THREADS >= 512 ? 2 : kTrainQ)>{});
#else
            if (2 * T > N) place_points(IC<2>{});
            else place_points(IC<kTrainQ>{});
#endif
            __syncthreads();
            MCI_TT(6)
            if (hclear)
                for (int i = tid; i < N; i += T) hclear[i] = 1.0e-10;
            MCI_TT(7)
            return;
        }
#ifndef MCI_TRAIN_SCAN_ONLY
        const double f_ninc = sum_julia(d, N) / (double)N;
        if (!(f_ninc > 0.0 && isfinite(f_ninc))) {
            if (tid == 0) atomicOr(status, ST_RESCALE_NONFINITE);
            return;
        }
        int *flag = (int *)(ps + 64);
        int *pw = (int *)ps;
        const int lane = tid & 63, wave = tid >> 6;
        const int per = (N + T - 1) / T, b = min(N, tid * per), e = min(N, b + per);
        bool given = spare != nullptr && serial_walk != 2 && N > 1;
        double *es = spare, *rs = spare + 2 * N + kWalkPad, *heads = rs + 2 * N + kWalkPad;
        const double f_inv = 1.0 / f_ninc, f_lo = 0.5 * f_ninc, f_hi = 2.0 * f_ninc;
        auto points = [&](int j) {
            if (j >= N - 1) return 0;
            const double c = floor(wa[j] * f_inv) - (j > 0 ? floor(wa[j - 1] * f_inv) : 0.0);
            if (serial_walk == 3 && j == N / 2) return c > 0.0 ? (int)c + 1 : 1;
            return c > 0.0 ? (int)c : 0;
        };
        auto slots = [&](int j, int c) { return c + ((c >= 1 && d[j + 1] >= f_lo && d[j + 1] <= f_hi) ? 0 : 1); };
        int sbase = 0, nslot = 0;
        if (given) {
            if (tid == 0) *flag = 0;
            block_prefix(d, wa, N, ps);
            int mine = 0;
            for (int j = b; j < e; ++j) mine += slots(j, points(j));
            int x = mine;
#pragma unroll
            for (int off = 1; off < 64; off <<= 1) {
                const int y = __shfl_up(x, off, 64);
                if (lane >= off) x += y;
            }
            if (lane == 63) pw[wave] = x;
            __syncthreads();
            for (int w = 0; w < (T >> 6); ++w) {
                if (w < wave) sbase += pw[w];
                nslot += pw[w];
            }
            sbase += x - mine;
            int sl = sbase;
            for (int j = b; j < e; ++j) {
                const int c = points(j);
                for (int k = 0; k < c - 1; ++k) es[sl++] = -f_ninc;
                if (c >= 1 && slots(j, c) == c) es[sl++] = d[j + 1] - f_ninc;
                else {
                    if (c >= 1) es[sl++] = -f_ninc;
                    es[sl++] = d[j + 1];
                }
            }
            for (int k = nslot + tid; k < nslot + kWalkPad; k += T) es[k] = 0.0;
            __syncthreads();
        }
        int cnt;
        for (;;) {
            if (tid == 0) {
                double va[16], vb[16];
                double acc_f = 0.0 + d[0];
                if (given) {
#pragma unroll
                    for (int k = 0; k < 16; ++k) va[k] = es[k];
                    for (int sb = 0; sb < nslot; sb += 32) {
#pragma unroll
                        for (int k = 0; k < 16; ++k) vb[k] = es[sb + 16 + k];
                        walk_slots16<false>(acc_f, va, heads + (sb >> 4));
#pragma unroll
                        for (int k = 0; k < 16; ++k) va[k] = es[sb + 32 + k];
                        walk_slots16<false>(acc_f, vb, heads + (sb >> 4) + 1);
                    }
                } else {
                    const unsigned rec = (unsigned)(size_t)wa;
#pragma unroll
                    for (int k = 0; k < 16; ++k) va[k] = d[k];
                    for (int jb = 0; jb < N; jb += 32) {
#pragma unroll
                        for (int k = 0; k < 16; ++k) vb[k] = d[jb + 16 + k];
                        walk_trip(acc_f, va, vb[0], f_ninc, rec + 8u * (unsigned)jb);
#pragma unroll
                        for (int k = 0; k < 16; ++k) va[k] = d[jb + 32 + k];
                        walk_trip(acc_f, vb, va[0], f_ninc, rec + 8u * (unsigned)(jb + 16));
                    }
                }
            }
            __syncthreads();
            if (given) {
                for (int t = tid; t * 16 < nslot; t += T) {
                    double ev[16];
#pragma unroll
                    for (int k = 0; k < 16; ++k) ev[k] = es[t * 16 + k];
                    double acc_f = heads[t];
                    walk_slots16<true>(acc_f, ev, rs + t * 16);
                }
                __syncthreads();
            }
            cnt = 0;
            int wrong = 0, sl = sbase;
            for (int j = b; j < e; ++j) {
                int c = 0;
                for (double a = given ? rs[sl] : wa[j]; a >= f_ninc; a -= f_ninc) c += 1;
                cnt += c;
                if (given) {
                    const int cp = points(j);
                    wrong |= (j < N - 1 && c != cp) ? 1 : 0;
                    sl += slots(j, cp);
                }
            }
            if (!given) break;
            if (wrong) atomicOr(flag, 1);
            __syncthreads();
            if (*flag == 0) break;
            given = false;
        }
        if (tid == 0) atomicAdd(status + (given ? 1 : 2), 1);
        {
            int x = cnt;
#pragma unroll
            for (int off = 1; off < 64; off <<= 1) {
                const int y = __shfl_up(x, off, 64);
                if (lane >= off) x += y;
            }
            if (lane == 63) pw[wave] = x;
            __syncthreads();
            int base = 0, total = 0;
            for (int w = 0; w < (T >> 6); ++w) {
                if (w < wave) base += pw[w];
                total += pw[w];
            }
            int i = 1 + base + x - cnt;
            int sl = sbase;
            for (int j = b; j < e; ++j) {
                for (double a = given ? rs[sl] : wa[j]; a >= f_ninc;) {
                    a -= f_ninc;
                    if (i < N) g[i] = sg[j + 1] - (a / d[j]) * (sg[j + 1] - sg[j]);
                    i += 1;
                }
                if (given) sl += slots(j, points(j));
            }
            for (int k = 1 + total + tid; k < N; k += T) g[k] = sg[N];
            if (tid == 0) {
                g[0] = sg[0];
                g[N] = sg[N];
            }
        }
#endif
    }
#ifndef MCI_TRAIN_CONTINUOUS_ONLY
    else {
        double *acc = dacc + L.eoff, *dist = ddist + L.doff;
        const double s = N > 1 ? sum_julia(h, N) : 1.0;
        if (tid == 0) {
            int lbad = 0;
            if (N > 1) {
                for (int i = 0; i < N; ++i) {
                    double v = h[i] / s;
                    if (v > 0 && v <= 0.99999999) v = rescale_pow(-(1 - v) / log(v), L.alpha);
                    if (!isfinite(v)) lbad = ST_RESCALE_NONFINITE;
                    d[i] = v;
                }
            } else {
                d[0] = h[0];
            }
            if (lbad) {
                atomicOr(status, lbad);
            } else {
                double s = 0.0;
                for (int i = 0; i < N; ++i) s += d[i];
                double run = 0.0;
                acc[0] = 0.0;
                for (int i = 0; i < N; ++i) {
                    const double v = d[i] / s;
                    dist[i] = v;
                    run += v;
                    acc[i + 1] = run;
                }
            }
        }
    }
#endif
    __syncthreads();
    if (hclear)
        for (int i = tid; i < N; i += T) hclear[i] = 1.0e-10;
#undef MCI_TT
}

__device__ inline void iteration_bookkeeping(const TrainArgs &a) {
    const int tid = threadIdx.x, T = blockDim.x;
    double *row = a.iter_log_row;
    if (row)
        for (int i = tid; i < a.nstat; i += T) row[i] = a.packed[i];
#ifndef MCI_TRAIN_CONTINUOUS_ONLY
    if (a.do_reweight && tid == 0) do_reweight_dev(a.reweight, a.packed + (a.nstat - a.nd), a.nd, a.gamma, a.goal);
#endif
}

struct PersistArgs {
    MergeArgs m;
    TrainArgs t;
    int niter;
    int map_off;
    u64 *ctr;
    u64 arrive0, done0;
    u64 spin_ticks;
};

enum : u64 { kPersistDoneShift = 40, kPersistArriveMask = (1ull << 40) - 1 };
__device__ __forceinline__ bool persist_wait(const PersistArgs &f, u64 t0, u64 t1, int *verdict) {
    if (threadIdx.x == 0) {
        int ok = 1;
        const u64 start = wall_clock64();
        unsigned n = 0;
        for (;;) {
            const u64 w = __hip_atomic_load(&f.ctr[0], __ATOMIC_RELAXED, __HIP_MEMORY_SCOPE_AGENT);
            if ((w & kPersistArriveMask) >= t0 && (long long)(((w >> kPersistDoneShift) - t1) << kPersistDoneShift) >= 0) break;
            __builtin_amdgcn_s_sleep(1);
            if (((++n & 255u) == 0u || f.spin_ticks < 256ull) &&
                (__hip_atomic_load(&f.ctr[2], __ATOMIC_RELAXED, __HIP_MEMORY_SCOPE_AGENT) != 0ull || wall_clock64() - start > f.spin_ticks)) {
                ok = 0;
                break;
            }
        }
        if (!ok) {
            __hip_atomic_store(&f.ctr[2], 1ull, __ATOMIC_RELAXED, __HIP_MEMORY_SCOPE_AGENT);
            atomicOr(f.m.status, ST_PERSIST_STALL);
        }
        __builtin_amdgcn_fence(__ATOMIC_ACQUIRE, "agent");
        *verdict = ok;
    }
    __syncthreads();
    return *verdict != 0;
}
__device__ __forceinline__ void persist_signal(u64 *ctr, u64 inc) {
    __builtin_amdgcn_s_waitcnt(0x0F70);
    __syncthreads();
    if (threadIdx.x == 0) {
        __builtin_amdgcn_fence(__ATOMIC_RELEASE, "agent");
        __hip_atomic_fetch_add(ctr, inc, __ATOMIC_RELAXED, __HIP_MEMORY_SCOPE_AGENT);
    }
}

template <class Cfg> __device__ __forceinline__ void vegas_persist(const BatchArgs &a0, const PersistArgs &f) {
    static_assert(Cfg::NLEAF == 1 && Cfg::leaf_kind(0) == 0, "the persistent kernel refines ONE Continuous grid (the host checks)");
    extern __shared__ __attribute__((aligned(16))) double smem[];
    const int tid = threadIdx.x, T = blockDim.x;
    constexpr int N = Cfg::leaf_nbin(0);
    double *sm = smem, *hl = sm + train_lds_doubles(N), *ps = hl + N, *gcur = smem + f.map_off, *flags = gcur + N + 2;
    int *verdict = reinterpret_cast<int *>(flags + 2);
    const u64 G = gridDim.x - 1;
    const int wg = (int)blockIdx.x;
    const size_t rows = (size_t)G * f.m.ncols;
#ifdef MCI_PERSIST_TRACE
#define MCI_PT(k)                                                                                                                      \
    if (tid == 0 && it < 8 && (wg == 0 || wg == (int)G - 1 || wg == (int)G)) {                                                          \
        f.ctr[8 + ((wg == 0 ? 0 : wg == (int)G ? 1 : 2) * 8 + it) * 8 + (k)] = wall_clock64();                                          \
        if (wg == 0 && (k) == 0 && (it == 0 || it == 7)) f.ctr[8 + 3 * 8 * 8 + 8 + (it == 0 ? 0 : 1)] = clock64();   \
    }
#else
#define MCI_PT(k)
#endif
    const LeafDev L = f.t.leaves[0];
    const bool train = f.t.do_train && L.adapt;
    if (wg == (int)G) {
        for (int it = 0; it < f.niter; ++it) {
            MCI_PT(0)
            if (!persist_wait(f, f.arrive0 + (u64)(it + 1) * G, f.done0 + (u64)it, verdict)) return;
            MCI_PT(3)
            MergeArgs m = f.m;
            m.part_cols = f.m.part_cols + (size_t)(it & 1) * rows;
            merge_stats(m);
            for (int e = tid; e < 2 * m.npa; e += T)
                m.packed[2 * m.nobs + 2 + m.ni + 1 + m.nbin + e] = (double)(m.nblocks + 1) * (e < m.npa ? 1.0e-8 : 1.0e-10);
            if (it > 0) {
                double *gz = a0.ghist + (size_t)((it + 2) % 3) * Cfg::NBIN + L.boff;
                for (int i = tid; i < N; i += T) gz[i] = 0.0;
            }
            if (it == f.niter - 1) {
                const double *gh = a0.ghist + (size_t)(it % 3) * Cfg::NBIN + L.boff;
                double *hp = f.t.packed + f.t.nstat + L.boff;
                for (int i = tid; i < N; i += T)
                    hp[i] = train ? 1.0e-10 : (double)(m.nblocks + 1) * 1.0e-10 + __hip_atomic_load(&gh[i], __ATOMIC_RELAXED, __HIP_MEMORY_SCOPE_AGENT);
            }
            __syncthreads();
            TrainArgs t = f.t;
            if (t.iter_log_row) t.iter_log_row += (size_t)it * t.nstat;
            iteration_bookkeeping(t);
            __syncthreads();
            MCI_PT(4)
            persist_signal(&f.ctr[0], 1ull << kPersistDoneShift);
            MCI_PT(5)
        }
        if (!persist_wait(f, f.arrive0 + (u64)(f.niter + 1) * G, f.done0, verdict)) return;
        double *gz = a0.ghist + (size_t)((f.niter - 1) % 3) * Cfg::NBIN + L.boff;
        for (int i = tid; i < N; i += T) gz[i] = 0.0;
        return;
    }
    for (int i = tid; i <= N; i += T) gcur[i] = f.t.edges[L.eoff + i];
    for (int it = 0; it < f.niter; ++it) {
        BatchArgs a = a0;
        a.iteration = a0.iteration + (u32)it;
        a.edges = gcur - L.eoff;
        a.part_cols = a0.part_cols + (size_t)(it & 1) * rows;
        a.ghist = a0.ghist + (size_t)(it % 3) * Cfg::NBIN;
        MCI_PT(0)
        if (tid == 0) *reinterpret_cast<int *>(flags) = 0;
        __syncthreads();
        vegas_batch<Cfg, false>(a);
        __syncthreads();
        MCI_PT(1)
        persist_signal(&f.ctr[0], 1ull);
        MCI_PT(2)
        if (!persist_wait(f, f.arrive0 + (u64)(it + 1) * G, f.done0 + (u64)it, verdict)) return;
        MCI_PT(3)
        const double *gh = a.ghist + L.boff;
        int hbad = 0;
        for (int base = 0; base < N; base += kTrainQ * T) {
            double v[kTrainQ];
#pragma unroll
            for (int q = 0; q < kTrainQ; ++q) {
                const int i = base + q * T + tid;
                v[q] = i < N ? __hip_atomic_load(&gh[i], __ATOMIC_RELAXED, __HIP_MEMORY_SCOPE_AGENT) : 0.0;
            }
#pragma unroll
            for (int q = 0; q < kTrainQ; ++q) {
                const int i = base + q * T + tid;
                if (i < N) {
                    const double h = (double)(f.m.nblocks + 1) * 1.0e-10 + v[q];
                    hl[i] = h;
                    if (!isfinite(h)) hbad |= ST_HIST_NONFINITE;
                    else if (!(h > 0.0)) hbad |= ST_HIST_NONPOSITIVE;
                }
            }
        }
        if (hbad) atomicOr(reinterpret_cast<int *>(flags), hbad);
        __syncthreads();
#ifdef MCI_PERSIST_TRACE
// ... 20 lines not shown
```

### mcintegration.jl_amd/engine.py

```python
import atexit
import ctypes as C
import weakref

import numpy as np

from . import _lib
from ._lib import LeafDesc, ProblemDesc, c_double_p, c_int32_p, check, lib
from .integrand import HostIntegrand, HostMeasure, Integrand, Measure
from .variables import ContinuousVar, FermiK

_ctx_cache = {}


def _dp(a):
    return a.ctypes.data_as(c_double_p)


def context(device=0):
    if device not in _ctx_cache:
        p = C.c_void_p()
        check(lib().mci_ctx_create(device, C.byref(p)))
        _ctx_cache[device] = p
    return _ctx_cache[device]

# ... 370 lines not shown
        try:
            self.close()
        except Exception:
            pass

    @staticmethod
    def _kernel_code(solver):
        return {"vegas_persistent": 3, "vegasmc_lanes": 5, "mcmc_lanes": 6, "vegas_strat": 7}.get(solver) or _lib.SOLVERS[solver]

    def compile(self, solver="vegas"):
        check(lib().mci_compile_solver(self.p, self._kernel_code(solver)))

    def code_object(self, solver="vegas"):
        buf = C.create_string_buffer(4096)
        check(lib().mci_kernel_code_object(self.p, self._kernel_code(solver), buf, len(buf)))
        return buf.value.decode()

    def set_kernel_timing(self, mode=-1):
        check(lib().mci_set_kernel_timing(self.p, int(mode)))

    def histogram_copies(self):
        n = C.c_int32()
        check(lib().mci_get_histogram_copies(self.p, C.byref(n)))
        return n.value

    def check_status(self):
        check(lib().mci_check_status(self.p))

    def set_launch(self, threads=0, wg_per_block=-1):
        check(lib().mci_set_launch(self.p, threads, wg_per_block))

    def run(self, solver, nevalperblock, block_lo, block_hi, iteration, seed, measurefreq=1, nchain=0, thermal_ratio=0.1):
        check(lib().mci_iteration_run(self.p, _lib.SOLVERS[solver], int(nevalperblock), int(block_lo), int(block_hi),
                                      int(iteration), int(seed), int(measurefreq), int(nchain), float(thermal_ratio)))

    def reduce(self):
        check(lib().mci_iteration_reduce(self.p))

    def finish(self, solver, block_total, adapt=True, gamma=1.0, want_stats=True):
        if not want_stats:
            check(lib().mci_iteration_finish(self.p, _lib.SOLVERS[solver], int(block_total), 1 if adapt else 0, gamma, None, None))
            return None, None
        m, e = np.empty(self.nobs), np.empty(self.nobs)
        check(lib().mci_iteration_finish(self.p, _lib.SOLVERS[solver], int(block_total), 1 if adapt else 0, gamma, _dp(m), _dp(e)))
        return m, e

    def iteration(self, solver, nevalperblock, block_lo, block_hi, iteration, seed, measurefreq=1, nchain=0, thermal_ratio=0.1):
        self.run(solver, nevalperblock, block_lo, block_hi, iteration, seed, measurefreq, nchain, thermal_ratio)
        return self.get_packed()

    def iteration_log(self, nrows):
        nstat = 2 * self.nobs + 2 + self.config.N + 1
        out = np.empty((nrows, nstat))
        check(lib().mci_get_iteration_log(self.p, int(nrows), _dp(out)))
        return out

    def reserve_iterations(self, rows):
        check(lib().mci_reserve_iteration_log(self.p, int(rows)))

    def get_packed(self, reduce_size=False):
        out = np.empty(self.reduce_size if reduce_size else self.packed_size)
        check(lib().mci_get_packed(self.p, _dp(out), len(out)))
        return out

    @property
    def reduce_size(self):
        return self.packed_size + 64

    def external_reduce_done(self):
        check(lib().mci_external_reduce_done(self.p))

    def comm_collectives(self):
        n, c = C.c_int64(), C.c_int64()
        check(lib().mci_comm_collectives(context(self.device), C.byref(n), C.byref(c)))
        return int(n.value), int(c.value)

    def set_packed(self, a):
        a = np.ascontiguousarray(a, dtype=np.float64)
        check(lib().mci_set_packed(self.p, _dp(a), len(a)))

    def packed_device_ptr(self):
        return lib().mci_packed_device_ptr(self.p)

    def hold_histogram(self):
        out = (C.c_uint64 * 64)()
        check(lib().mci_get_hold_histogram(self.p, out))
        return np.array(list(out), dtype=np.uint64)

    def stream(self):
        return lib().mci_ctx_stream(context(self.device)) or 0

    def save_state(self, path):
        check(lib().mci_save_state(self.p, str(path).encode()))

    def load_state(self, path):
        check(lib().mci_load_state(self.p, str(path).encode()))

    def train(self):
        check(lib().mci_train(self.p))

    def set_rng_rounds(self, rounds):
        check(lib().mci_set_rng_rounds(self.p, int(rounds)))

    def set_rng_bits(self, bits):
        check(lib().mci_set_rng_bits(self.p, int(bits)))

    def set_deterministic(self, on=True):
        check(lib().mci_set_deterministic(self.p, 1 if on else 0))

    def set_chain_carry(self, mode):
        check(lib().mci_set_chain_carry(self.p, {"auto": -1, "off": 0, "on": 1, -1: -1, 0: 0, 1: 1}[mode]))

    def set_iteration_counted(self, counted):
        check(lib().mci_set_iteration_counted(self.p, 1 if counted else 0))

    def set_persistent(self, mode):
        check(lib().mci_set_persistent(self.p, {"auto": -1, "off": 0, "on": 1, -1: -1, 0: 0, 1: 1}[mode]))

    def last_integrate_persistent(self):
        v = C.c_int32()
        check(lib().mci_last_integrate_persistent(self.p, C.byref(v)))
        return bool(v.value)

    def last_chain_launch(self):
        n, c = C.c_int64(), C.c_int32()
        check(lib().mci_last_chain_launch(self.p, C.byref(n), C.byref(c)))
        return int(n.value), bool(c.value)

    def set_chain_speculation(self, lanes=-1, accept=0.0, max_accepts=-1):
        check(lib().mci_set_chain_speculation(self.p, int(lanes), float(accept), int(max_accepts)))

    def last_chain_speculation(self):
        g, m = C.c_int32(), C.c_int32()
        check(lib().mci_last_chain_speculation(self.p, C.byref(g), C.byref(m)))
        return int(g.value), int(m.value)

    def chain_speculation_status(self, solver):
        st = C.c_int32()
        check(lib().mci_chain_speculation_status(self.p, _lib.SOLVERS[solver], C.byref(st)))
        return int(st.value)

    def compile_chain_speculation(self, solver):
        check(lib().mci_compile_chain_speculation(self.p, _lib.SOLVERS[solver]))

    def set_train_walk(self, mode):
        check(lib().mci_debug_plant_wrong_decision(self.p, 1 if mode in ("serial_wrong_decision", 3) else 0))
        check(lib().mci_set_train_walk(self.p, {"auto": -1, "scan": 0, "serial": 1, "serial_general": 2, "serial_wrong_decision": 1, -1: -1, 0: 0, 1: 1, 2: 2, 3: 1}[mode]))

    def walk_counts(self):
        out = (C.c_int64 * 2)()
        check(lib().mci_debug_walk_counts(self.p, out))
        return int(out[0]), int(out[1])

    def split_chunks(self):
        n, b = C.c_int64(), C.c_int64()
        check(lib().mci_debug_split_chunks(self.p, C.byref(n), C.byref(b)))
        return int(n.value), int(b.value)

    def integrate(self, solver, neval, niter=10, block=16, ignore=-1, adapt=True, gamma=1.0, measurefreq=1, seed=1234,
                  nchain=0, first_iteration=0, thermal_ratio=0.1, reweight_goal=None):
        goal = None
        if reweight_goal is not None:
            self._goal = np.ascontiguousarray(reweight_goal, dtype=np.float64)
            goal = _dp(self._goal)
        a = _lib.IntegrateArgs(_lib.SOLVERS[solver], int(neval), int(niter), int(block), int(ignore), 1 if adapt else 0,
                               float(gamma), int(measurefreq), int(seed), int(nchain), int(first_iteration),
                               float(thermal_ratio), goal)
        n = self.nobs
        im, ie = np.zeros((niter, n)), np.zeros((niter, n))
        m, s, c2 = np.zeros(n), np.zeros(n), np.zeros(n)
        vis = np.zeros(self.config.N + 1)
        r = _lib.ResultC(niter, n, _dp(im), _dp(ie), _dp(m), _dp(s), _dp(c2), 0, 0.0, _dp(vis), 0, 0)
        check(lib().mci_integrate(self.p, C.byref(a), C.byref(r)))
        dn, dl = C.c_int64(), C.c_int32()
        check(lib().mci_last_integrate_discarded(self.p, C.byref(dn), C.byref(dl)))
        out = dict(mean=m, stdev=s, chi2=c2, iter_mean=im, iter_std=ie, neval=r.neval, seconds=r.seconds, visited=vis,
                   correlated=bool(r.correlated), block_mean=None, warmup=int(r.warmup), neval_discarded=int(dn.value))
        if _lib.SOLVERS[solver] != _lib.VEGAS and out["correlated"]:
            out["block_mean"] = self.block_means(niter)[0]
        return out

    def mcmc_launch_valid(self):
        v, w, ln, h = C.c_int32(), C.c_int32(), C.c_int64(), C.c_int64()
        check(lib().mci_mcmc_launch_valid(self.p, C.byref(v), C.byref(w), C.byref(ln), C.byref(h)))
        return bool(v.value), bool(w.value), int(ln.value), int(h.value)

    def discard_iteration(self):
        check(lib().mci_iteration_discard(self.p))

    def block_means(self, rows):
        nb, carried = C.c_int64(), C.c_int32()
        check(lib().mci_get_block_means(self.p, 0, None, C.byref(nb), C.byref(carried)))
        out = np.zeros((int(rows), int(nb.value), self.nobs))
        if rows > 0 and out.size:
            check(lib().mci_get_block_means(self.p, int(rows), _dp(out), C.byref(nb), C.byref(carried)))
        return out, int(carried.value)

    def comm_sum(self, v):
        a = np.ascontiguousarray(v, dtype=np.float64).copy()
        check(lib().mci_comm_sum(self.p, _dp(a), a.size))
        return a

    def reset_block_log(self):
        check(lib().mci_reset_block_log(self.p))

    def comm_ranks(self):
        r, n = C.c_int32(), C.c_int32()
        check(lib().mci_comm_rank(context(self.device), C.byref(r), C.byref(n)))
        return int(n.value)

    def set_stratification(self, nstrat=None, beta=0.75, max_nhcube=2 ** 24, on=True):
        if not on:
            check(lib().mci_set_stratification_off(self.p))
            return
        ns = None
        if nstrat is not None:
            self._nstrat = np.ascontiguousarray(nstrat, dtype=np.int32)
            ns = self._nstrat.ctypes.data_as(c_int32_p)
        check(lib().mci_set_stratification(self.p, self.ndraw, ns, float(beta), int(max_nhcube)))

    def stratification(self):
        ns, nc, b = np.zeros(self.ndraw, dtype=np.int32), C.c_int64(), C.c_double()
        check(lib().mci_get_stratification(self.p, ns.ctypes.data_as(c_int32_p), C.byref(nc), C.byref(b)))
        if not ns.any():
            return None
        return dict(nstrat=[int(v) for v in ns], ncube=int(nc.value), beta=float(b.value))

    def strat_counts(self):
        info = self.stratification()
        n = info["ncube"] if info else 0
        out = np.zeros(n, dtype=np.int64)
        check(lib().mci_get_strat_counts(self.p, out.ctypes.data_as(C.POINTER(C.c_int64)), n))
        return out

    def strat_dump_next(self, n):
        d = dict(x=np.zeros((n, self.ndraw)), y=np.zeros((n, self.ndraw)), h=np.zeros(n, dtype=np.int64), jac=np.zeros(n),
                 w=np.zeros((n, self.config.N * self.config.ncomp)))
        self._strat_dump = d
        check(lib().mci_debug_strat_dump(self.p, int(n), _dp(d["x"]), _dp(d["y"]), d["h"].ctypes.data_as(C.POINTER(C.c_int64)),
                                         _dp(d["jac"]), _dp(d["w"])))
        return d

    def sample_dump(self, n, nevalperblock=None, block_index=0, iteration=0, seed=1234):
        nevalperblock = n if nevalperblock is None else nevalperblock
        x, jac, w = np.empty((n, self.ndraw)), np.empty(n), np.empty((n, self.config.N * self.config.ncomp))
        check(lib().mci_sample_dump(self.p, iteration, seed, int(nevalperblock), int(block_index), int(n), _dp(x), _dp(jac), _dp(w)))
        return x, jac, w

    def kernel_times_ms(self, n=512):
        ms = (C.c_float * n)()
        got, wg, th = C.c_int32(), C.c_int32(), C.c_int32()
        check(lib().mci_kernel_times_ms(self.p, ms, n, C.byref(got), C.byref(wg), C.byref(th)))
        return np.array(ms[:got.value], dtype=np.float64), wg.value, th.value

    def kernel_clocks_mhz(self, n=512):
        out = np.empty(n)
        got = C.c_int32()
        check(lib().mci_kernel_clocks(self.p, _dp(out), n, C.byref(got)))
        return out[:got.value].copy()

    def comm_times_ms(self, n=64):
        ms = (C.c_float * n)()
        got = C.c_int32()
        check(lib().mci_comm_times_ms(self.p, ms, n, C.byref(got)))
        return np.array(ms[:got.value], dtype=np.float64)

    def last_kernel_ms(self):
        ms, wg, th = self.kernel_times_ms(1)
        return (float(ms[-1]) if len(ms) else float("nan")), wg, th

    def grid(self, leaf):
        n = self.config.leaves[leaf].ninc
        out = np.empty(n)
        check(lib().mci_get_grid(self.p, leaf, _dp(out), n))
        return out

    def set_grid(self, leaf, grid):
        g = np.ascontiguousarray(grid, dtype=np.float64)
        check(lib().mci_set_grid(self.p, leaf, _dp(g), len(g)))

    def distribution(self, leaf):
        lf = self.config.leaves[leaf]
        k = lf.upper - lf.lower + 1
        d, a = np.empty(k), np.empty(k + 1)
        check(lib().mci_get_distribution(self.p, leaf, _dp(d), _dp(a), k))
        return d, a

    def set_distribution(self, leaf, dist):
        d = np.ascontiguousarray(dist, dtype=np.float64)
        check(lib().mci_set_distribution(self.p, leaf, _dp(d), len(d)))

    def histogram(self, leaf):
        packed = self.get_packed()
        off = 2 * self.nobs + 2 + self.config.N + 1
        for i, lf in enumerate(self.config.leaves):
            nb = (lf.ninc - 1) if isinstance(lf, ContinuousVar) else 1 if isinstance(lf, FermiK) else (lf.upper - lf.lower + 1)
            if i == leaf:
                return packed[off:off + nb]
            off += nb
        raise IndexError(leaf)

    def reweight(self):
        out = np.empty(self.config.N + 1)
        check(lib().mci_get_reweight(self.p, _dp(out), len(out)))
        return out

# ... 25 lines not shown
```

Measured before the change: 74590.

## Fuse histogram stage-1 reduction into finalize/finish kernels via atomic tickets

Removes the separate k_hist_stage1 launch after each iteration. The stage-1 partial histogram reduction now runs as extra workgroups inside the finalize or finish kernel. The last-arriving workgroup for each slice or leaf, detected with an agent-scope atomic ticket counter, then does the merge and training. This saves one kernel launch and its serialization per iteration, at the cost of more workgroups and release/acquire fences. It also adds debug ticket introspection, optional phase timers, and an override that restores the two-launch path.

After: 74610, median of 4. No clear change (+0.0%).

```diff
diff --git a/mcintegration.jl_amd/_lib.py b/mcintegration.jl_amd/_lib.py
--- a/mcintegration.jl_amd/_lib.py
+++ b/mcintegration.jl_amd/_lib.py
@@ -146,6 +146,7 @@
 DEBUG_SIGNATURES = [
     ("mci_debug_persist_words", C.c_int, [_VP, C.POINTER(C.c_uint64), C.c_int32]),
     ("mci_debug_walk_counts", C.c_int, [_VP, C.POINTER(C.c_int64)]),
+    ("mci_debug_merge_tickets", C.c_int, [_VP, c_int32_p, C.c_int32, c_int32_p]),
     ("mci_debug_plant_wrong_decision", C.c_int, [_VP, C.c_int32]),
     ("mci_debug_persist_spin_ticks", C.c_int, [_VP, C.c_uint64]),
     ("mci_debug_override", C.c_int, [C.c_char_p, C.c_int64, C.c_int32]),
diff --git a/mcintegration.jl_amd/csrc/mci_debug.h b/mcintegration.jl_amd/csrc/mci_debug.h
--- a/mcintegration.jl_amd/csrc/mci_debug.h
+++ b/mcintegration.jl_amd/csrc/mci_debug.h
@@ -6,6 +6,7 @@
 #endif
 int mci_debug_persist_words(mci_problem *prob, unsigned long long *out, int32_t n);
 int mci_debug_walk_counts(mci_problem *prob, int64_t *out);
+int mci_debug_merge_tickets(mci_problem *prob, int32_t *out, int32_t n, int32_t *got);
 int mci_debug_plant_wrong_decision(mci_problem *prob, int32_t on);
 int mci_debug_persist_spin_ticks(mci_problem *prob, unsigned long long ticks);
 int mci_debug_override(const char *key, int64_t value, int32_t on);
diff --git a/mcintegration.jl_amd/csrc/mci_host_integrate.h b/mcintegration.jl_amd/csrc/mci_host_integrate.h
--- a/mcintegration.jl_amd/csrc/mci_host_integrate.h
+++ b/mcintegration.jl_amd/csrc/mci_host_integrate.h
@@ -221,6 +221,7 @@
     p->persist_done += (unsigned long long)ia->niter;
     p->launch.time_this_launch = false;
     p->merge_pending = false;
+    p->merge_stage1_rows = 0;
     p->merge = m;
     p->merge.part_cols = p->d_part_cols + (size_t)((ia->niter - 1) & 1) * (size_t)nrows * s.ncols;
     p->launch.last_samples = nblocks * nevalperblock;
diff --git a/mcintegration.jl_amd/csrc/mci_host_iteration.h b/mcintegration.jl_amd/csrc/mci_host_iteration.h
--- a/mcintegration.jl_amd/csrc/mci_host_iteration.h
+++ b/mcintegration.jl_amd/csrc/mci_host_iteration.h
@@ -600,9 +600,14 @@
     p->launch.last_nblocks = (int)nblocks;
     if (solver != MCI_VEGAS) p->launch.last_nchain = nchain;
     const int nb256 = (s.nbin + 255) / 256;
-    if (hist_lds && s.nbin > 0 && !atomic_flush)
+    p->merge_stage1_rows = 0;
+    if (hist_lds && s.nbin > 0 && !atomic_flush) {
+        const bool fuse = s.ntile == 1 && !p->in_self_check && !(g_over.two_launch_merge.on && g_over.two_launch_merge.v);
+        if (fuse) p->merge_stage1_rows = hist_rows;
+        else
         hipLaunchKernelGGL(mci::k_hist_stage1, dim3(nb256, mci_problem::kGroups), dim3(256), 0, st, p->d_part_hist, (int)hist_rows, s.nbin,
                            (int)mci_problem::kGroups, p->d_stage1);
+    }
     HIPCHK(hipGetLastError());
     mci::MergeArgs &m = p->merge;
     m.part_cols = p->d_part_cols;
@@ -641,12 +646,32 @@
     return MCI_OK;
 }
 
+static mci::Stage1Args stage1_args(mci_problem *p, int64_t rows) {
+    mci::Stage1Args f{};
+    f.part_hist = p->d_part_hist;
+    f.rows = (int)rows;
+    f.tickets = p->d_tickets;
+#ifdef MCI_FINISH_PHASES
+    (void)hipMemsetAsync(p->d_phases, 0, 64 * sizeof(unsigned long long), p->ctx->stream);
+    f.phases = p->d_phases;
+#endif
+    return f;
+}
+
 static int flush_merge(mci_problem *p) {
     if (!p->merge_pending) return MCI_OK;
     p->merge_pending = false;
     HIPCHK(hipSetDevice(p->ctx->device));
-    const int nb256 = (p->shape.nbin + 255) / 256;
-    hipLaunchKernelGGL(mci::k_finalize, dim3(nb256 + 1 + (2 * p->npa + 3) / 4), dim3(256), 0, p->ctx->stream, p->merge);
+    const int64_t rows = p->merge_stage1_rows;
+    p->merge_stage1_rows = 0;
+    if (rows > 0) {
+        const int nsl = (p->shape.nbin + mci::kFinalizeSlice - 1) / mci::kFinalizeSlice;
+        hipLaunchKernelGGL(mci::k_finalize_fused, dim3(nsl * mci_problem::kGroups + 1 + (2 * p->npa + 3) / 4), dim3(256), 0, p->ctx->stream,
+                           p->merge, stage1_args(p, rows));
+    } else {
+        const int nb256 = (p->shape.nbin + 255) / 256;
+        hipLaunchKernelGGL(mci::k_finalize, dim3(nb256 + 1 + (2 * p->npa + 3) / 4), dim3(256), 0, p->ctx->stream, p->merge);
+    }
     HIPCHK(hipGetLastError());
     return MCI_OK;
 }
@@ -747,11 +772,21 @@
     if (sm > 64 * 1024 && !p->train_lds_raised) {
         HIPCHK(hipFuncSetAttribute((const void *)mci::k_train, hipFuncAttributeMaxDynamicSharedMemorySize, (int)kTrainLdsMax));
         HIPCHK(hipFuncSetAttribute((const void *)mci::k_finish, hipFuncAttributeMaxDynamicSharedMemorySize, (int)kTrainLdsMax));
+        HIPCHK(hipFuncSetAttribute((const void *)mci::k_finish_fused, hipFuncAttributeMaxDynamicSharedMemorySize, (int)kTrainLdsMax));
         p->train_lds_raised = true;
     }
     if (p->merge_pending) {
         p->merge_pending = false;
-        hipLaunchKernelGGL(mci::k_finish, dim3(s.nleaf + 1 + (2 * p->npa + 3) / 4), dim3(tt), sm, p->ctx->stream, p->merge, a);
+        const int64_t rows = p->merge_stage1_rows;
+        p->merge_stage1_rows = 0;
+        if (rows > 0) {
+            const int nsl = (maxn + (int)tt / 4 - 1) / ((int)tt / 4);
+            hipLaunchKernelGGL(mci::k_finish_fused, dim3(s.nleaf * mci_problem::kGroups * nsl + 1 + (2 * p->npa + 3) / 4), dim3(tt), sm,
+                               p->ctx->stream, p->merge, a, stage1_args(p, rows));
+        } else {
+            hipLaunchKernelGGL(mci::k_finish, dim3(s.nleaf + 1 + (2 * p->npa + 3) / 4), dim3(tt), sm, p->ctx->stream, p->merge, a,
+                               stage1_args(p, 0));
+        }
     } else {
         hipLaunchKernelGGL(mci::k_train, dim3(s.nleaf + 1), dim3(tt), sm, p->ctx->stream, a);
     }
diff --git a/mcintegration.jl_amd/csrc/mci_host_jit.h b/mcintegration.jl_amd/csrc/mci_host_jit.h
--- a/mcintegration.jl_amd/csrc/mci_host_jit.h
+++ b/mcintegration.jl_amd/csrc/mci_host_jit.h
@@ -573,6 +573,26 @@
     return MCI_OK;
 }
 
+int mci_debug_merge_tickets(mci_problem *p, int32_t *out, int32_t n, int32_t *got) {
+    if (!p || !out || !got || !p->d_tickets) return fail(MCI_ERR_INVALID, "NULL argument");
+    HIPCHK(hipStreamSynchronize(p->ctx->stream));
+    const int k = n - 1 < p->n_tickets ? n - 1 : p->n_tickets;
+    if (k < 0) return fail(MCI_ERR_INVALID, "n must be at least 1");
+    HIPCHK(hipMemcpy(out, p->d_tickets, (size_t)k * sizeof(int), hipMemcpyDeviceToHost));
+    out[k] = p->merge_pending && p->merge_stage1_rows > 0 ? 1 : 0;
+    *got = p->n_tickets;
+    return MCI_OK;
+}
+
+#ifdef MCI_FINISH_PHASES
+int mci_debug_finish_phases(mci_problem *p, unsigned long long *out, int32_t n) {
+    if (!p || !out || !p->d_phases) return fail(MCI_ERR_INVALID, "NULL argument");
+    HIPCHK(hipStreamSynchronize(p->ctx->stream));
+    HIPCHK(hipMemcpy(out, p->d_phases, (size_t)(n < 64 ? n : 64) * sizeof(unsigned long long), hipMemcpyDeviceToHost));
+    return MCI_OK;
+}
+#endif
+
 int mci_debug_walk_counts(mci_problem *p, int64_t *out) {
     if (!p || !out || !p->d_status) return fail(MCI_ERR_INVALID, "NULL argument");
     int h[2] = {0, 0};
diff --git a/mcintegration.jl_amd/csrc/mci_host_problem.h b/mcintegration.jl_amd/csrc/mci_host_problem.h
--- a/mcintegration.jl_amd/csrc/mci_host_problem.h
+++ b/mcintegration.jl_amd/csrc/mci_host_problem.h
@@ -330,6 +330,15 @@
         HIPCHK(hipMalloc((void **)&p->d_ghist, 3 * (size_t)(s.nbin ? s.nbin : 1) * sizeof(double)));
         HIPCHK(hipMemset(p->d_ghist, 0, 3 * (size_t)(s.nbin ? s.nbin : 1) * sizeof(double)));
         HIPCHK(hipMalloc((void **)&p->d_stage1, (size_t)mci_problem::kGroups * (s.nbin ? s.nbin : 1) * sizeof(double)));
+        p->n_tickets = (s.nbin + mci::kFinalizeSlice - 1) / mci::kFinalizeSlice;
+        if (p->n_tickets < s.nleaf) p->n_tickets = s.nleaf;
+        if (p->n_tickets < 1) p->n_tickets = 1;
+        HIPCHK(hipMalloc((void **)&p->d_tickets, (size_t)p->n_tickets * sizeof(int)));
+        HIPCHK(hipMemset(p->d_tickets, 0, (size_t)p->n_tickets * sizeof(int)));
+#ifdef MCI_FINISH_PHASES
+        HIPCHK(hipMalloc((void **)&p->d_phases, 64 * sizeof(unsigned long long)));
+        HIPCHK(hipMemset(p->d_phases, 0, 64 * sizeof(unsigned long long)));
+#endif
         HIPCHK(hipMalloc((void **)&p->d_status, 4 * sizeof(int)));
         HIPCHK(hipMemset(p->d_status, 0, 4 * sizeof(int)));
         std::vector<mci::LeafDev> ld;
@@ -351,7 +360,7 @@
         for (void *q : {(void *)p->d_edges, (void *)p->d_dacc, (void *)p->d_ddist, (void *)p->d_reweight, (void *)p->d_ud,
                         (void *)p->d_part_cols, (void *)p->d_part_hist, (void *)p->d_ghist, (void *)p->d_stage1,
                         (void *)p->d_packed, (void *)p->d_scratch, (void *)p->d_iterlog, (void *)p->d_dump,
-                        (void *)p->d_status, (void *)p->d_leaves})
+                        (void *)p->d_status, (void *)p->d_tickets, (void *)p->d_leaves})
             if (q) (void)hipFree(q);
         for (int k = 0; k < mci_problem::kSlots; ++k)
             if (p->module[k]) (void)hipModuleUnload(p->module[k]);
@@ -359,6 +368,9 @@
         if (p->strat.module) (void)hipModuleUnload(p->strat.module);
         strat_free_buffers(p);
         if (p->d_persist) (void)hipFree(p->d_persist);
+#ifdef MCI_FINISH_PHASES
+        if (p->d_phases) (void)hipFree(p->d_phases);
+#endif
     }
     persist_job_drop(p);
     if (!p->ctx->offline) {
diff --git a/mcintegration.jl_amd/csrc/mci_host_strat.h b/mcintegration.jl_amd/csrc/mci_host_strat.h
--- a/mcintegration.jl_amd/csrc/mci_host_strat.h
+++ b/mcintegration.jl_amd/csrc/mci_host_strat.h
@@ -390,6 +390,7 @@
     m.block_means = nullptr;
     m.hold = nullptr;
     p->merge_pending = true;
+    p->merge_stage1_rows = 0;
     p->launch.last_samples = N;
     p->launch.last_wg = (int)nwg;
     p->launch.last_threads = T;
diff --git a/mcintegration.jl_amd/csrc/mci_host_types.h b/mcintegration.jl_amd/csrc/mci_host_types.h
--- a/mcintegration.jl_amd/csrc/mci_host_types.h
+++ b/mcintegration.jl_amd/csrc/mci_host_types.h
@@ -80,6 +80,11 @@
     double *d_part_cols = nullptr, *d_part_hist = nullptr, *d_ghist = nullptr, *d_stage1 = nullptr, *d_packed = nullptr;
     double *d_scratch = nullptr, *d_iterlog = nullptr, *d_dump = nullptr;
     int *d_status = nullptr;
+    int *d_tickets = nullptr;
+    int n_tickets = 0;
+#ifdef MCI_FINISH_PHASES
+    unsigned long long *d_phases = nullptr;
+#endif
     mci::LeafDev *d_leaves = nullptr;
     int64_t cap_wg = 0, cap_blocks = 0, cap_iter = 0, cap_dump = 0;
     static const int kSlots = 7;
@@ -116,6 +121,7 @@
     hipFunction_t f_tiles[2] = {nullptr, nullptr};
     mci::MergeArgs merge{};
     bool merge_pending = false;
+    int64_t merge_stage1_rows = 0;
     bool has_fermik = false;
     mci_host_integrand_fn host_fn = nullptr;
     mci_host_integrand_idx_fn host_idx_fn = nullptr;
@@ -265,7 +271,8 @@
 
 namespace {
 struct Override { bool on = false; int64_t v = 0; };
-struct Overrides { Override table_mode, hist_tile_bins, no_split_all, l1_phase, train_walk, hist_copies, fresh_floors, fresh_burnin_pct, spec_self_check, split_chunk; } g_over;
+struct Overrides { Override table_mode, hist_tile_bins, no_split_all, l1_phase, train_walk, hist_copies, fresh_floors, fresh_burnin_pct, spec_self_check, split_chunk,
+                   two_launch_merge; } g_over;
 Override *override_slot(const char *key) {
     if (!key) return nullptr;
     if (!strcmp(key, "table_mode")) return &g_over.table_mode;
@@ -278,6 +285,7 @@
     if (!strcmp(key, "fresh_burnin_pct")) return &g_over.fresh_burnin_pct;
     if (!strcmp(key, "spec_self_check")) return &g_over.spec_self_check;
     if (!strcmp(key, "split_chunk")) return &g_over.split_chunk;
+    if (!strcmp(key, "two_launch_merge")) return &g_over.two_launch_merge;
     return nullptr;
 }
 }
@@ -391,6 +399,7 @@
     p->persist_arrive = p->persist_done = 0;
     p->persist_failed = true;
     p->merge_pending = false;
+    p->merge_stage1_rows = 0;
     return MCI_OK;
 }
 
diff --git a/mcintegration.jl_amd/csrc/mci_static_kernels.h b/mcintegration.jl_amd/csrc/mci_static_kernels.h
--- a/mcintegration.jl_amd/csrc/mci_static_kernels.h
+++ b/mcintegration.jl_amd/csrc/mci_static_kernels.h
@@ -32,6 +32,79 @@
     part_cols[(size_t)b * wg_per_block * ncols + o] += obs[i];
 }
 
+struct Stage1Args {
+    const double *part_hist;
+    int rows;
+    int *tickets;
+    unsigned long long *phases;
+};
+enum { kFinalizeSlice = 64 };
+
+#ifdef MCI_FINISH_PHASES
+#define MCI_PH(k) if (ph && threadIdx.x == 0) { ph[2 * (k)] = clock64(); ph[2 * (k) + 1] = wall_clock64(); }
+#else
+#define MCI_PH(k)
+#endif
+
+__device__ inline bool stage1_slice(const Stage1Args &f, const MergeArgs &m, int g, int bin0, int nb, int *ctr, int needed, int *last) {
+    const int tid = threadIdx.x, q = tid & 3, b = tid >> 2, bin = bin0 + b;
+    const int per = (f.rows + m.ngroup - 1) / m.ngroup;
+    const int w0 = g * per, w1 = min(f.rows, w0 + per);
+    const int nfull = w1 > w0 ? (w1 - w0) >> 2 : 0;
+    double s = 0.0;
+    if (b < nb) {
+        const double *__restrict__ col = f.part_hist + (size_t)(w0 + q) * m.nbin + bin;
+        const size_t step = (size_t)4 * m.nbin;
+        int k = 0;
+        for (; k + 8 <= nfull; k += 8) {
+            double v[8];
+#pragma unroll
+            for (int u = 0; u < 8; ++u) v[u] = col[(size_t)(k + u) * step];
+#pragma unroll
+            for (int u = 0; u < 8; ++u) s += v[u];
+        }
+        for (; k < nfull; ++k) s += col[(size_t)k * step];
+        if (q == 0)
+            for (int w = w0 + 4 * nfull; w < w1; ++w) s += f.part_hist[(size_t)w * m.nbin + bin];
+    }
+    s += __shfl_xor(s, 1, 64);
+    s += __shfl_xor(s, 2, 64);
+    if (b < nb && q == 0) const_cast<double *>(m.stage1)[(size_t)g * m.nbin + bin] = s;
+    __builtin_amdgcn_s_waitcnt(0x0F70);
+    __syncthreads();
+    if (tid == 0) {
+        __builtin_amdgcn_fence(__ATOMIC_RELEASE, "agent");
+        const int t = __hip_atomic_fetch_add(ctr, 1, __ATOMIC_RELAXED, __HIP_MEMORY_SCOPE_AGENT);
+        *last = t == needed - 1;
+        if (*last) {
+            *ctr = 0;
+            __builtin_amdgcn_fence(__ATOMIC_ACQUIRE, "agent");
+        }
+    }
+    __syncthreads();
+    return *last != 0;
+}
+
+__device__ inline void finish_leaf(const MergeArgs &m, const TrainArgs &a, int leaf, double *sm, double *ps, int &bad, double &ssum,
+                                   unsigned long long *ph) {
+    const int tid = threadIdx.x, T = blockDim.x;
+    const LeafDev L = a.leaves[leaf];
+    double *hl = sm + train_lds_doubles(a.maxn);
+    double *hp = a.packed + a.nstat + L.boff;
+    const bool train = a.do_train && L.adapt;
+    if (train) train_stage_grid(L, sm, a.edges);
+    for (int i = tid; i < L.nbin; i += T) {
+        const double v = merge_hist_bin(m, L.boff + i);
+        hl[i] = v;
+        hp[i] = v;
+    }
+    __syncthreads();
+    MCI_PH(3)
+    if (!train) return;
+    train_leaf(L, hl, hp, sm, ps, bad, ssum, a.edges, a.dacc, a.ddist, a.serial_walk, a.status, true, ph ? ph + 2 * 4 : nullptr, false,
+               a.spare ? hl : nullptr);
+}
+
 __global__ void __launch_bounds__(256) k_finalize(MergeArgs m) {
     const int nhb = (m.nbin + 255) / 256;
     const int hoff = 2 * m.nobs + 2 + m.ni + 1;
@@ -42,6 +115,24 @@
     }
     if ((int)blockIdx.x > nhb) {
         merge_pa(m, (int)blockIdx.x - nhb - 1);
+        return;
+    }
+    merge_stats(m);
+}
+
+__global__ void __launch_bounds__(256) k_finalize_fused(MergeArgs m, Stage1Args f) {
+    __shared__ int last;
+    const int nsl = (m.nbin + kFinalizeSlice - 1) / kFinalizeSlice, nst = nsl * m.ngroup;
+    const int hoff = 2 * m.nobs + 2 + m.ni + 1;
+    if ((int)blockIdx.x < nst) {
+        const int sl = (int)blockIdx.x / m.ngroup, g = (int)blockIdx.x % m.ngroup, bin0 = sl * kFinalizeSlice;
+        if (!stage1_slice(f, m, g, bin0, min(kFinalizeSlice, m.nbin - bin0), f.tickets + sl, m.ngroup, &last)) return;
+        const int bin = bin0 + (int)threadIdx.x;
+        if ((int)threadIdx.x < kFinalizeSlice && bin < m.nbin) m.packed[hoff + bin] = merge_hist_bin(m, bin);
+        return;
+    }
+    if ((int)blockIdx.x > nst) {
+        merge_pa(m, (int)blockIdx.x - nst - 1);
         return;
     }
     merge_stats(m);
@@ -174,36 +265,71 @@
     train_leaf(L, h, h, sm, ps, bad, ssum, a.edges, a.dacc, a.ddist, a.serial_walk, a.status, false, nullptr, false, a.spare ? sm + train_lds_doubles(a.maxn) : nullptr);
 }
 
-__global__ void __launch_bounds__(512) k_finish(MergeArgs m, TrainArgs a) {
+__global__ void __launch_bounds__(512) k_finish(MergeArgs m, TrainArgs a, Stage1Args f) {
     extern __shared__ __attribute__((aligned(16))) double sm[];
     __shared__ double ps[256];
     __shared__ int bad;
     __shared__ double ssum;
-    const int tid = threadIdx.x, T = blockDim.x;
+    unsigned long long *ph = f.phases;
     if ((int)blockIdx.x == a.nleaf) {
+        MCI_PH(20)
         merge_stats(m);
         __syncthreads();
+        MCI_PH(21)
         iteration_bookkeeping(a);
+        MCI_PH(22)
         return;
     }
     if ((int)blockIdx.x > a.nleaf) {
         merge_pa(m, (int)blockIdx.x - a.nleaf - 1);
         return;
     }
-    const LeafDev L = a.leaves[blockIdx.x];
-    double *hl = sm + train_lds_doubles(a.maxn);
-    double *hp = a.packed + a.nstat + L.boff;
-    const bool train = a.do_train && L.adapt;
-    if (train) train_stage_grid(L, sm, a.edges);
-    for (int i = tid; i < L.nbin; i += T) {
-        const double v = merge_hist_bin(m, L.boff + i);
-        hl[i] = v;
-        hp[i] = v;
-    }
-    __syncthreads();
-    if (!train) return;
-    train_leaf(L, hl, hp, sm, ps, bad, ssum, a.edges, a.dacc, a.ddist, a.serial_walk, a.status, true, nullptr, false, a.spare ? hl : nullptr);
-}
+    if (blockIdx.x != 0) ph = nullptr;
+    MCI_PH(0)
+    finish_leaf(m, a, (int)blockIdx.x, sm, ps, bad, ssum, ph);
+}
+
+__global__ void __launch_bounds__(512) k_finish_fused(MergeArgs m, TrainArgs a, Stage1Args f) {
+    extern __shared__ __attribute__((aligned(16))) double sm[];
+    __shared__ double ps[256];
+    __shared__ int bad;
+    __shared__ double ssum;
+    __shared__ int last;
+    unsigned long long *ph = f.phases;
+    const int bpw = (int)blockDim.x >> 2, nsl = (a.maxn + bpw - 1) / bpw, per_leaf = m.ngroup * nsl, nst = a.nleaf * per_leaf;
+    if ((int)blockIdx.x == nst) {
+        MCI_PH(20)
+        merge_stats(m);
+        __syncthreads();
+        MCI_PH(21)
+        iteration_bookkeeping(a);
+        MCI_PH(22)
+        return;
+    }
+    if ((int)blockIdx.x > nst) {
+        merge_pa(m, (int)blockIdx.x - nst - 1);
+        return;
+    }
+    const int leaf = (int)blockIdx.x / per_leaf, r = (int)blockIdx.x % per_leaf, g = r / nsl, sl = r % nsl;
+    const LeafDev L = a.leaves[leaf];
+    const int lsl = (L.nbin + bpw - 1) / bpw;
+    if (sl >= lsl) return;
+    if (blockIdx.x == 0) {
+        MCI_PH(23)
+    }
+#ifdef MCI_FINISH_PHASES
+    const unsigned long long e0 = wall_clock64();
+#endif
+    const bool done = stage1_slice(f, m, g, L.boff + sl * bpw, min(bpw, L.nbin - sl * bpw), f.tickets + leaf, m.ngroup * lsl, &last);
+    if (!done) return;
+    if (leaf != 0) ph = nullptr;
+#ifdef MCI_FINISH_PHASES
+    if (ph && threadIdx.x == 0) ph[2 * 1 + 1] = e0;
+#endif
+    MCI_PH(2)
+    finish_leaf(m, a, leaf, sm, ps, bad, ssum, ph);
+}
+#undef MCI_PH
 
 struct StratAllocArgs {
     const double *d;
diff --git a/mcintegration.jl_amd/csrc/mci_train.h b/mcintegration.jl_amd/csrc/mci_train.h
--- a/mcintegration.jl_amd/csrc/mci_train.h
+++ b/mcintegration.jl_amd/csrc/mci_train.h
@@ -321,6 +321,8 @@
                                   double *spare = nullptr) {
 #ifdef MCI_PERSIST_TRACE
 #define MCI_TT(k) if (tt && threadIdx.x == 0) tt[k] = wall_clock64();
+#elif defined(MCI_FINISH_PHASES)
+#define MCI_TT(k) if (tt && threadIdx.x == 0) { tt[2 * (k)] = clock64(); tt[2 * (k) + 1] = wall_clock64(); }
 #else
 #define MCI_TT(k)
     (void)tt;
@@ -484,6 +486,7 @@
         }
 #ifndef MCI_TRAIN_SCAN_ONLY
         const double f_ninc = sum_julia(d, N) / (double)N;
+        MCI_TT(8)
         if (!(f_ninc > 0.0 && isfinite(f_ninc))) {
             if (tid == 0) atomicOr(status, ST_RESCALE_NONFINITE);
             return;
@@ -533,6 +536,7 @@
             }
             for (int k = nslot + tid; k < nslot + kWalkPad; k += T) es[k] = 0.0;
             __syncthreads();
+            MCI_TT(9)
         }
         int cnt;
         for (;;) {
@@ -565,6 +569,7 @@
                 }
             }
             __syncthreads();
+            MCI_TT(given ? 10 : 13)
             if (given) {
                 for (int t = tid; t * 16 < nslot; t += T) {
                     double ev[16];
@@ -574,6 +579,7 @@
                     walk_slots16<true>(acc_f, ev, rs + t * 16);
                 }
                 __syncthreads();
+                MCI_TT(11)
             }
             cnt = 0;
             int wrong = 0, sl = sbase;
@@ -590,6 +596,7 @@
             if (!given) break;
             if (wrong) atomicOr(flag, 1);
             __syncthreads();
+            MCI_TT(12)
             if (*flag == 0) break;
             given = false;
         }
@@ -623,6 +630,7 @@
                 g[0] = sg[0];
                 g[N] = sg[N];
             }
+            MCI_TT(14)
         }
 #endif
     }
@@ -662,6 +670,7 @@
     __syncthreads();
     if (hclear)
         for (int i = tid; i < N; i += T) hclear[i] = 1.0e-10;
+    MCI_TT(15)
 #undef MCI_TT
 }
 
diff --git a/mcintegration.jl_amd/engine.py b/mcintegration.jl_amd/engine.py
--- a/mcintegration.jl_amd/engine.py
+++ b/mcintegration.jl_amd/engine.py
@@ -546,6 +546,12 @@
         check(lib().mci_debug_walk_counts(self.p, out))
         return int(out[0]), int(out[1])
 
+    def merge_tickets(self):
+        out, got = (C.c_int32 * 4097)(), C.c_int32()
+        check(lib().mci_debug_merge_tickets(self.p, out, 4097, C.byref(got)))
+        k = min(int(got.value), 4096)
+        return [int(v) for v in out[:k]], bool(out[k])
+
     def split_chunks(self):
         n, b = C.c_int64(), C.c_int64()
         check(lib().mci_debug_split_chunks(self.p, C.byref(n), C.byref(b)))
```
